# allenai/OLMoASR

Hardware: AMD Instinct MI355X
Metric: audio-seconds/sec/node (train step) (higher is better)
Workload: dtype bf16

## Files before the change

### include/oasr.h

```cpp
#ifndef OASR_H
#define OASR_H
#include <stddef.h>
#include <stdint.h>
#ifdef __cplusplus
extern "C" {
#endif

#define OASR_OK 0
#define OASR_EINVAL (-1)
#define OASR_EHIP (-2)
#define OASR_ESTATE (-3)
#define OASR_ERETRY (-4)

typedef struct oasr_ctx oasr_ctx;

typedef struct oasr_dims {
  int n_mels, n_audio_ctx, n_audio_state, n_audio_head, n_audio_layer;
  int n_vocab, n_text_ctx, n_text_state, n_text_head, n_text_layer;
} oasr_dims;

const char* oasr_last_error(void);
#define OASR_ABI_VERSION 216
int oasr_version(void);

// ... 64 lines not shown
  int32_t B;
  int32_t S;
  int32_t span_forward;
  int32_t accumulate_loss;
  float loss_scale, inv_accum;
} oasr_train_step_args;
size_t oasr_sizeof_train_step_args(void);
int oasr_train_step(oasr_ctx*, const oasr_train_step_args*, void* workspace, size_t workspace_bytes, void* stream);

int oasr_train_fwd(oasr_ctx*, const float* mel, const int64_t* tokens, const int32_t* text_len, int B, int S, float* logits_out,
                   void* workspace, size_t workspace_bytes, void* stream);
int oasr_train_bwd(oasr_ctx*, const int64_t* tokens, const int32_t* text_len, const float* dlogits, int B, int S, void** seg_events,
                   void* workspace, size_t workspace_bytes, void* stream);
int oasr_zero_grad(oasr_ctx*, void* stream);

int oasr_train_encode(oasr_ctx*, const float* mel, int B, void* xa_out, void* workspace, size_t workspace_bytes, void* stream);
int oasr_train_encode_bwd(oasr_ctx*, const void* dxa, int B, float* dmel_out, void* workspace, size_t workspace_bytes, void* stream);
int oasr_train_decode(oasr_ctx*, const int64_t* tokens, const void* xa, const int32_t* text_len, int B, int S, float* logits_out,
                      void* workspace, size_t workspace_bytes, void* stream);
int oasr_train_decode_bwd(oasr_ctx*, const int64_t* tokens, const int32_t* text_len, const float* dlogits, int B, int S, void* dxa_out,
                          void* workspace, size_t workspace_bytes, void* stream);

int oasr_set_trainable(oasr_ctx*, const uint8_t* mask, int n_params);

int oasr_optim_step(oasr_ctx*, float inv_loss_scale, float max_grad_norm, float lr, float beta1, float beta2, float eps,
                    float weight_decay, int64_t step, float* stats_out, void* scratch, void* stream);

int oasr_grad_sumsq_range(oasr_ctx*, int64_t off, int64_t numel, float* stats_out, void* scratch, void* stream);
int oasr_optim_step_range(oasr_ctx*, int64_t off, int64_t numel, float* exp_avg_shard, float* exp_avg_sq_shard, const float* stats,
                          float inv_loss_scale, float max_grad_norm, float lr, float beta1, float beta2, float eps, float weight_decay,
                          int64_t step, void* stream);

typedef struct oasr_operand {
  const void* ptr; int64_t ld; int rpb; int64_t bstride; int lead; int kvalid; int trail_from;
} oasr_operand;
typedef struct oasr_gemm_args {
  oasr_operand A, B; int M, N, K; int ta, tb; float alpha;
  const float* bias; int act; const float* pos; int pos_period;
  const void* dgelu_u; int64_t ldu; const void* resid; int64_t ldr;
  void* out; void* out_pre; int64_t ldc; float* out_f32; int64_t ldc32; float beta; float* colsum; int atomic; int split_k;
  int dgelu_deriv;
} oasr_gemm_args;
int oasr_gemm(const oasr_gemm_args*, void* stream);
int oasr_layernorm_fwd(const void* x, const float* gamma, const float* beta, void* y, float* mean, float* rstd, int64_t rows, int d, void* stream);
int oasr_layernorm_bwd(const void* dy, const void* x, const float* gamma, const float* mean, const float* rstd, const void* dres,
                       void* dx, float* dgamma, float* dbeta, int64_t rows, int d, void* stream);
typedef struct oasr_attn_args {
  const void *q, *k, *v; int64_t ldq, ldk, ldv, bsq, bsk, bsv; void* o; int64_t ldo, bso; float* lse; void* o_lo; const int32_t* kv_len;
  int B, H, Tq, Tk, causal; const void* d_o; float* delta; void *dq, *dk, *dv;
  float *dq_colsum, *dv_colsum;
  float* colsum_scratch;
  int32_t* qtile_flags;
  const int32_t *q_rows, *k_rows, *q_span;
} oasr_attn_args;
#define OASR_ROWTAB 16
size_t oasr_sizeof_attn_args(void);
int oasr_attention_fwd(const oasr_attn_args*, void* stream);
int oasr_attention_bwd(const oasr_attn_args*, void* stream);
int oasr_attention_scores(const oasr_attn_args*, int dtype, float* scores, void* stream);
#define OASR_ALIGN_MAX_LAYERS 32
typedef struct oasr_align_args {
  const float* qk[OASR_ALIGN_MAX_LAYERS];
  uint32_t head_mask[OASR_ALIGN_MAX_LAYERS];
  int32_t n_layers, H, n_tok, Tk, n_frames, medfilt_width;
  float qk_scale;
  int32_t reserved;
  float* out;
  int64_t ldo;
} oasr_align_args;
size_t oasr_sizeof_align_args(void);
size_t oasr_alignment_workspace_bytes(int n_selected_heads, int n_tok, int n_frames);
int oasr_alignment_matrix(const oasr_align_args*, void* workspace, size_t workspace_bytes, void* stream);
size_t oasr_dtw_workspace_bytes(int N, int M);
int oasr_dtw(const float* cost, int64_t ld, int N, int M, int negate, int32_t* text_indices, int32_t* time_indices, int32_t* path_len,
             void* workspace, size_t workspace_bytes, void* stream);
#define OASR_SPECAUG_MAX_MASKS 8
typedef struct oasr_specaug {
  int32_t freq_masks, freq_width, time_masks, time_width;
  float fill;
} oasr_specaug;
size_t oasr_sizeof_specaug(void);
int oasr_spec_augment(float* mel, int B, int n_mels, int T, const oasr_specaug* policy, uint64_t seed, uint64_t first_clip, void* stream);
int oasr_spec_augment_plan(const oasr_specaug* policy, uint64_t seed, uint64_t clip, int n_mels, int T, int32_t* freq_iv, int32_t* time_iv);
#define OASR_EDIT_MAX_LEN 1023
typedef struct oasr_edit_args {
  const int32_t *hyp, *ref, *hyp_len, *ref_len;
  int32_t* out;
  int64_t ld_hyp, ld_ref;
  int32_t B, Lh, Lr, reserved;
} oasr_edit_args;
size_t oasr_sizeof_edit_args(void);
int oasr_edit_counts(const oasr_edit_args*, void* stream);
int oasr_edit_counts_host(const oasr_edit_args*);
int oasr_cross_entropy(void* logits_bf16, int64_t ld, int V, const int64_t* targets, int64_t rows, int64_t ignore, float gscale,
                       int32_t* n_valid_dev, float* row_loss, float* loss_out, int write_grad, void* stream);
int oasr_cast_f32_bf16(const float* src, void* dst, int64_t n, void* stream);
int oasr_lora_merge_op(const float* w0, const float* A, const float* B, int rows, int cols, int rank, float scale, int out_dtype, void* out,
                       void* stream);
size_t oasr_lora_grad_scratch_bytes(int rows, int cols, int rank);
int oasr_lora_grad_op(const float* dW, const float* A, const float* B, int rows, int cols, int rank, float scale, float* dA, float* dB,
                      void* scratch, void* stream);
int oasr_pick_tokens(const float* logits, int64_t ld, int V, int64_t rows, const float* mask, const float* mask2, int64_t* tok,
                     float* logprob, void* stream);
int oasr_pick_tokens_ts(const float* logits, int64_t ld, int V, int64_t rows, const float* mask, const float* mask2,
                        const int64_t* history, int64_t history_ld, int n_history, int timestamp_begin, int eot, int no_timestamps,
                        int max_initial_index, int64_t* tok, float* logprob, void* stream);
// ... 12 lines not shown
```

### include/oasr_testing.h

```cpp
#ifndef OASR_TESTING_H
#define OASR_TESTING_H
#include "oasr.h"
#ifdef __cplusplus
extern "C" {
#endif

int oasr_profile_gemm(int enable);
int oasr_gemm_set_variant(int v);
int oasr_decode_set_ln_fold(int mode);
int oasr_span_set_side_streams(int mode);
int oasr_span_side_streams(void);
int oasr_xcd_plan_debug(int d, int H, int Te, int M, int L, int team, int wg, int* out, int max_blocks);
int oasr_wide_supports_debug(int d, int H, int Te, int S_max, int L, int M, int nwg);
int oasr_wide_plan_debug(int d, int nwg, int N, int K, int wg, int wave, int* out, int max_units);
int oasr_xcd_offsets_ok_debug(const int64_t* layer0, long long lstride, long long cache_lstride, int d, int Te, int L, int M);
int oasr_attention_set_pingpong(int on);
int oasr_gemm_set_stagger(int sleeps, int phases);
int oasr_gemm_force_general(int on);
int oasr_test_gemm(const oasr_gemm_args* a, float* colsum_scratch, int atomic_on_pp, int raster_gm, int stagger, int stagger_phases, void* stream);
int oasr_profile_gemm_records(char* buf, int cap);
int oasr_profile_gemm_collect(double* ms4, double* flops4, int64_t* count4, char* by_symbol , int cap);
int oasr_probe_lds_oob(const void* src_u16 , void* dst_u16 , void* stream);
int oasr_probe_tr16(const void* src_bf16 , void* dst_bf16 , void* stream);
int oasr_test_span_tables(const int32_t* span_host, int B, int S, const int64_t* targets, int32_t* rows_out, int32_t* span_out,
                          int64_t* targets_rows_out, int64_t* active_rows_out, void* stream);

int oasr_test_embedding_fwd(const int64_t* tok, const float* E, const float* pos, void* x, int dtype, int B, int S, int d, int64_t n_embed,
                            const int32_t* rows, void* stream);
int oasr_test_embedding_bwd(const int64_t* tok, const void* dx, int dtype, float* dE, float* dpos, int B, int S, int d, int64_t pad_id,
                            int64_t n_embed, const int32_t* rows, const int32_t* span, void* stream);
int oasr_test_colsum(const void* x, int dtype, int64_t ld, int64_t M, int ncols, float* out, void* stream);
int oasr_test_conv2_col2im_dgelu(const void* dA, const void* u1, void* dpre1, int dtype, int B, int T1, int d, void* stream);
int oasr_test_conv1_col2im_mel(const void* dcol, int dtype, float* dmel, int B, int T1, int n_mels, void* stream);
int oasr_test_mel_to_time_major(const float* mel, void* out, int dtype, int B, int n_mels, int T, const float* clip_max, void* stream);
int oasr_test_pack_conv_weight(const float* w, void* dst, int dtype, int co, int ci, int ldk, void* stream);
int oasr_test_unpack_conv_grad(const float* g, float* dw, int co, int ci, int ldk, void* stream);
int oasr_test_pack_embedding(const float* e, void* dst, int rows, int rows_pad, int d, void* stream);
int oasr_test_dgelu_mul(const void* dy, const void* u, void* out, int dtype, int64_t n, void* stream);
int oasr_test_dlogits_from_f32(const float* src, int V, int64_t rows, int64_t ld, void* dst, int dtype, void* stream);
int oasr_test_logits_to_f32(const void* logits, int dtype, int64_t ld, int64_t rows, int V, float* out, void* stream);
int oasr_test_layernorm_bwd(const void* dy, const void* x, const float* gamma, const float* mean, const float* rstd, const void* dres, void* dx,
                            float* dgamma, float* dbeta, float* dsum, int dtype, int64_t rows, int d, void* stream);

int oasr_test_dtw_host(const float* cost, int64_t ld, int N, int M, int negate, int32_t* text_indices, int32_t* time_indices, int32_t* path_len,
                       void* workspace);

int oasr_test_argmax_rows(const void* logits, int dtype, int64_t ld, int V, int64_t n_rows, const int32_t* rows, const int32_t* span, int B, int S,
                          int32_t* pred_out, void* stream);

#ifdef __cplusplus
}
#endif
#endif
```

### olmoasr_amd/_native.py

```python
import ctypes as C
import os

import torch

_HERE = os.path.dirname(os.path.abspath(__file__))
LIB_PATH = os.environ.get("OASR_LIB") or os.path.join(_HERE, "liboasr.so")
_lib = None


class NativeError(RuntimeError):
    pass


class Dims(C.Structure):
    _fields_ = [(n, C.c_int) for n in ("n_mels", "n_audio_ctx", "n_audio_state", "n_audio_head", "n_audio_layer",
                                       "n_vocab", "n_text_ctx", "n_text_state", "n_text_head", "n_text_layer")]


class Operand(C.Structure):
    _fields_ = [("ptr", C.c_void_p), ("ld", C.c_int64), ("rpb", C.c_int), ("bstride", C.c_int64), ("lead", C.c_int),
                ("kvalid", C.c_int), ("trail_from", C.c_int)]


class GemmArgs(C.Structure):
    _fields_ = [("A", Operand), ("B", Operand), ("M", C.c_int), ("N", C.c_int), ("K", C.c_int), ("ta", C.c_int),
                ("tb", C.c_int), ("alpha", C.c_float), ("bias", C.c_void_p), ("act", C.c_int), ("pos", C.c_void_p),
                ("pos_period", C.c_int), ("dgelu_u", C.c_void_p), ("ldu", C.c_int64), ("resid", C.c_void_p),
                ("ldr", C.c_int64), ("out", C.c_void_p), ("out_pre", C.c_void_p), ("ldc", C.c_int64),
                ("out_f32", C.c_void_p), ("ldc32", C.c_int64), ("beta", C.c_float), ("colsum", C.c_void_p), ("atomic", C.c_int),
                ("split_k", C.c_int), ("dgelu_deriv", C.c_int)]


class AttnArgs(C.Structure):
    _fields_ = [("q", C.c_void_p), ("k", C.c_void_p), ("v", C.c_void_p), ("ldq", C.c_int64), ("ldk", C.c_int64),
                ("ldv", C.c_int64), ("bsq", C.c_int64), ("bsk", C.c_int64), ("bsv", C.c_int64), ("o", C.c_void_p),
                ("ldo", C.c_int64), ("bso", C.c_int64), ("lse", C.c_void_p), ("o_lo", C.c_void_p), ("kv_len", C.c_void_p), ("B", C.c_int),
                ("H", C.c_int), ("Tq", C.c_int), ("Tk", C.c_int), ("causal", C.c_int), ("d_o", C.c_void_p),
                ("delta", C.c_void_p), ("dq", C.c_void_p), ("dk", C.c_void_p), ("dv", C.c_void_p), ("dq_colsum", C.c_void_p),
                ("dv_colsum", C.c_void_p), ("colsum_scratch", C.c_void_p), ("qtile_flags", C.c_void_p),
                ("q_rows", C.c_void_p), ("k_rows", C.c_void_p), ("q_span", C.c_void_p)]


class AlignArgs(C.Structure):
    MAX_LAYERS = 32
    _fields_ = [("qk", C.c_void_p * 32), ("head_mask", C.c_uint32 * 32), ("n_layers", C.c_int32), ("H", C.c_int32), ("n_tok", C.c_int32),
                ("Tk", C.c_int32), ("n_frames", C.c_int32), ("medfilt_width", C.c_int32), ("qk_scale", C.c_float), ("reserved", C.c_int32),
                ("out", C.c_void_p), ("ldo", C.c_int64)]


class SpecAug(C.Structure):
    MAX_MASKS = 8
    _fields_ = [("freq_masks", C.c_int32), ("freq_width", C.c_int32), ("time_masks", C.c_int32), ("time_width", C.c_int32), ("fill", C.c_float)]


class EditArgs(C.Structure):
    MAX_LEN = 1023
    _fields_ = [("hyp", C.c_void_p), ("ref", C.c_void_p), ("hyp_len", C.c_void_p), ("ref_len", C.c_void_p), ("out", C.c_void_p),
                ("ld_hyp", C.c_int64), ("ld_ref", C.c_int64), ("B", C.c_int32), ("Lh", C.c_int32), ("Lr", C.c_int32), ("reserved", C.c_int32)]


class TrainStepArgs(C.Structure):
    _fields_ = [(n, C.c_void_p) for n in ("mel", "xa", "tokens", "targets", "text_len", "span_host", "mel_clip_max", "loss_out", "logits_out",
                                          "pred_out", "seg_events")] + \
               [(n, C.c_int32) for n in ("B", "S", "span_forward", "accumulate_loss")] + [("loss_scale", C.c_float), ("inv_accum", C.c_float)]


DTW_MAX_N, DTW_MAX_M = 448, 1500
ABI_VERSION = 216
KV_TAIL_BYTES = 327680
MODE_INFER, MODE_TRAIN, MODE_TRAIN_ENC, MODE_TRAIN_DEC = 0, 1, 2, 3
ROWTAB = 16
LORA_MAX_RANK = 64


def _declare(lib):
    vp, i32, i64, f32, sz = C.c_void_p, C.c_int, C.c_int64, C.c_float, C.c_size_t
    sig = {
        "oasr_last_error": (C.c_char_p, []),
        "oasr_version": (i32, []),
        "oasr_log_mel_workspace_bytes": (sz, [i32]),
        "oasr_log_mel": (i32, [vp, i32, i32, i32, vp, vp, vp]),
        "oasr_mel_filterbank": (i32, [vp]),
        "oasr_create": (vp, [C.POINTER(Dims)]),
        "oasr_create_ex": (vp, [C.POINTER(Dims), i32]),
        "oasr_create_ex2": (vp, [C.POINTER(Dims), i32, i32]),
        "oasr_compute_dtype": (i32, [vp]),
        "oasr_create_ex3": (vp, [C.POINTER(Dims), i32, i32, vp, i32, i32, f32]),
        "oasr_lora_count": (i32, [vp]),
        "oasr_lora_merge": (i32, [vp, vp]),
        "oasr_lora_merge_op": (i32, [vp, vp, vp, i32, i32, i32, f32, i32, vp, vp]),
        "oasr_lora_grad_scratch_bytes": (sz, [i32, i32, i32]),
        "oasr_lora_grad_op": (i32, [vp, vp, vp, i32, i32, i32, f32, vp, vp, vp, vp]),
        "oasr_encode": (i32, [vp, vp, i32, vp, vp, sz, vp]),
        "oasr_kv_cache_bytes": (sz, [vp, i32]),
        "oasr_decode_step_workspace_bytes": (sz, [vp, i32]),
        "oasr_decode_begin": (i32, [vp, vp, i32, vp, vp]),
        "oasr_decode_step": (i32, [vp, vp, i32, i32, vp, vp, vp, sz, vp]),
        "oasr_decode_check": (i32, [vp, i32, vp, vp]),
        "oasr_decode_logits": (i32, [vp, vp, vp, vp, i32, i32, i32, vp, vp, sz, vp]),
        "oasr_destroy": (None, [vp]),
        "oasr_param_count": (i32, [vp]),
        "oasr_param_info": (i32, [vp, i32, C.c_char_p, i32, C.POINTER(i64), C.POINTER(i64), C.POINTER(i32), C.POINTER(i64)]),
        "oasr_param_numel": (i64, [vp]),
        "oasr_segment_count": (i32, [vp]),
        "oasr_segment_info": (i32, [vp, i32, C.POINTER(i64), C.POINTER(i64)]),
        "oasr_bind": (i32, [vp, vp, vp, vp, vp, vp]),
        "oasr_shadow_bytes": (sz, [vp]),
        "oasr_bind_shadow": (i32, [vp, vp]),
        "oasr_refresh_shadow": (i32, [vp, vp]),
        "oasr_workspace_bytes": (sz, [vp, i32, i32, i32]),
        "oasr_forward": (i32, [vp, vp, vp, vp, i32, i32, vp, vp, vp, sz, vp]),
        "oasr_sizeof_train_step_args": (sz, []),
        "oasr_train_step": (i32, [vp, C.POINTER(TrainStepArgs), vp, sz, vp]),
        "oasr_log_mel_raw": (i32, [vp, i32, i32, i32, vp, vp, vp, vp]),
        "oasr_sizeof_attn_args": (sz, []),
        "oasr_test_span_tables": (i32, [vp, i32, i32, vp, vp, vp, vp, vp, vp]),
        "oasr_test_embedding_fwd": (i32, [vp, vp, vp, vp, i32, i32, i32, i32, i64, vp, vp]),
        "oasr_test_embedding_bwd": (i32, [vp, vp, i32, vp, vp, i32, i32, i32, i64, i64, vp, vp, vp]),
        "oasr_test_colsum": (i32, [vp, i32, i64, i64, i32, vp, vp]),
        "oasr_test_conv2_col2im_dgelu": (i32, [vp, vp, vp, i32, i32, i32, i32, vp]),
        "oasr_test_conv1_col2im_mel": (i32, [vp, i32, vp, i32, i32, i32, vp]),
        "oasr_test_mel_to_time_major": (i32, [vp, vp, i32, i32, i32, i32, vp, vp]),
        "oasr_test_pack_conv_weight": (i32, [vp, vp, i32, i32, i32, i32, vp]),
        "oasr_test_unpack_conv_grad": (i32, [vp, vp, i32, i32, i32, vp]),
        "oasr_test_pack_embedding": (i32, [vp, vp, i32, i32, i32, vp]),
        "oasr_test_dgelu_mul": (i32, [vp, vp, vp, i32, i64, vp]),
        "oasr_test_dlogits_from_f32": (i32, [vp, i32, i64, i64, vp, i32, vp]),
        "oasr_test_logits_to_f32": (i32, [vp, i32, i64, i64, i32, vp, vp]),
        "oasr_test_layernorm_bwd": (i32, [vp, vp, vp, vp, vp, vp, vp, vp, vp, vp, i32, i64, i32, vp]),
        "oasr_train_fwd": (i32, [vp, vp, vp, vp, i32, i32, vp, vp, sz, vp]),
        "oasr_train_bwd": (i32, [vp, vp, vp, vp, i32, i32, vp, vp, sz, vp]),
        "oasr_zero_grad": (i32, [vp, vp]),
        "oasr_train_encode": (i32, [vp, vp, i32, vp, vp, sz, vp]),
        "oasr_train_encode_bwd": (i32, [vp, vp, i32, vp, vp, sz, vp]),
        "oasr_train_decode": (i32, [vp, vp, vp, vp, i32, i32, vp, vp, sz, vp]),
        "oasr_train_decode_bwd": (i32, [vp, vp, vp, vp, i32, i32, vp, vp, sz, vp]),
        "oasr_set_trainable": (i32, [vp, vp, i32]),
        "oasr_optim_step": (i32, [vp, f32, f32, f32, f32, f32, f32, f32, i64, vp, vp, vp]),
        "oasr_grad_sumsq_range": (i32, [vp, i64, i64, vp, vp, vp]),
        "oasr_optim_step_range": (i32, [vp, i64, i64, vp, vp, vp, f32, f32, f32, f32, f32, f32, f32, i64, vp]),
        "oasr_gemm": (i32, [C.POINTER(GemmArgs), vp]),
        "oasr_test_gemm": (i32, [C.POINTER(GemmArgs), vp, i32, i32, i32, i32, vp]),
        "oasr_profile_gemm_records": (i32, [C.c_char_p, i32]),
        "oasr_layernorm_fwd": (i32, [vp, vp, vp, vp, vp, vp, i64, i32, vp]),
        "oasr_layernorm_bwd": (i32, [vp, vp, vp, vp, vp, vp, vp, vp, vp, i64, i32, vp]),
        "oasr_attention_fwd": (i32, [C.POINTER(AttnArgs), vp]),
        "oasr_attention_bwd": (i32, [C.POINTER(AttnArgs), vp]),
        "oasr_attention_scores": (i32, [C.POINTER(AttnArgs), i32, vp, vp]),
        "oasr_sizeof_align_args": (sz, []),
        "oasr_alignment_workspace_bytes": (sz, [i32, i32, i32]),
        "oasr_alignment_matrix": (i32, [C.POINTER(AlignArgs), vp, sz, vp]),
        "oasr_dtw_workspace_bytes": (sz, [i32, i32]),
        "oasr_dtw": (i32, [vp, i64, i32, i32, i32, vp, vp, vp, vp, sz, vp]),
        "oasr_test_dtw_host": (i32, [vp, i64, i32, i32, i32, vp, vp, vp, vp]),
        "oasr_sizeof_specaug": (sz, []),
        "oasr_spec_augment": (i32, [vp, i32, i32, i32, C.POINTER(SpecAug), C.c_uint64, C.c_uint64, vp]),
        "oasr_spec_augment_plan": (i32, [C.POINTER(SpecAug), C.c_uint64, C.c_uint64, i32, i32, vp, vp]),
        "oasr_sizeof_edit_args": (sz, []),
        "oasr_edit_counts": (i32, [C.POINTER(EditArgs), vp]),
        "oasr_edit_counts_host": (i32, [C.POINTER(EditArgs)]),
        "oasr_test_argmax_rows": (i32, [vp, i32, i64, i32, i64, vp, vp, i32, i32, vp, vp]),
        "oasr_cross_entropy": (i32, [vp, i64, i32, vp, i64, i64, f32, vp, vp, vp, i32, vp]),
        "oasr_cast_f32_bf16": (i32, [vp, vp, i64, vp]),
        "oasr_pick_tokens": (i32, [vp, i64, i32, i64, vp, vp, vp, vp, vp]),
        "oasr_pick_tokens_ts": (i32, [vp, i64, i32, i64, vp, vp, vp, i64, i32, i32, i32, i32, i32, vp, vp, vp]),
        "oasr_topk_tokens": (i32, [vp, i64, i32, i64, vp, vp, vp, i64, i32, i32, i32, i32, i32, i32, vp, vp, vp]),
        "oasr_sample_tokens": (i32, [vp, i64, i32, i64, vp, vp, vp, i64, i32, i32, i32, i32, i32, f32, vp, vp, vp, vp]),
        "oasr_probe_tr16": (i32, [vp, vp, vp]),
        "oasr_probe_lds_oob": (i32, [vp, vp, vp]),
        "oasr_profile_gemm": (i32, [i32]),
        "oasr_gemm_force_general": (i32, [i32]),
        "oasr_gemm_set_stagger": (i32, [i32, i32]),
        "oasr_gemm_set_variant": (i32, [i32]),
        "oasr_decode_set_ln_fold": (i32, [i32]),
        "oasr_span_set_side_streams": (i32, [i32]),
        "oasr_span_side_streams": (i32, []),
        "oasr_xcd_plan_debug": (i32, [i32, i32, i32, i32, i32, i32, i32, vp, i32]),
        "oasr_xcd_offsets_ok_debug": (i32, [vp, C.c_longlong, C.c_longlong, i32, i32, i32, i32]),
        "oasr_wide_supports_debug": (i32, [i32, i32, i32, i32, i32, i32, i32]),
        "oasr_wide_plan_debug": (i32, [i32, i32, i32, i32, i32, i32, vp, i32]),
        "oasr_attention_set_pingpong": (i32, [i32]),
        "oasr_profile_gemm_collect": (i32, [vp, vp, vp, C.c_char_p, i32]),
    }
    for name, (res, args) in sig.items():
        fn = getattr(lib, name)
        fn.restype = res
        fn.argtypes = args
    return list(sig)


EXPORTS = None


def lib():
    global _lib, EXPORTS
    if _lib is None:
        if not os.path.isfile(LIB_PATH):
            raise NativeError(f"{LIB_PATH} not found: run `python -c 'import __graft_entry__ as g; g.build()'` "
                              "(hipcc --offload-arch=gfx950).  There is no CPU/PyTorch fallback for this path.")
        try:
            _lib = C.CDLL(LIB_PATH)
        except OSError as e:
            raise NativeError(f"cannot load {LIB_PATH}: {e}") from e
        handle, _lib = _lib, None
        vfn = getattr(handle, "oasr_version", None)
        ver = int(vfn()) if vfn is not None else None
        sfn = getattr(handle, "oasr_sizeof_attn_args", None)
        size = int(sfn()) if sfn is not None else None
        if ver != ABI_VERSION or size != C.sizeof(AttnArgs):
            raise NativeError(f"{LIB_PATH}: ABI version {ver} / oasr_attn_args of {size} bytes, this binding is written for version "
                              f"{ABI_VERSION} / {C.sizeof(AttnArgs)} bytes -- rebuild (__graft_entry__.build())")
        try:
            exports = _declare(handle)
        except AttributeError as e:
            raise NativeError(f"{LIB_PATH} (ABI {ver}) lacks an entry point this binding declares: {e} -- rebuild (__graft_entry__.build())") from e
        if int(handle.oasr_sizeof_align_args()) != C.sizeof(AlignArgs):
            raise NativeError(f"{LIB_PATH}: oasr_align_args of {int(handle.oasr_sizeof_align_args())} bytes, this binding passes "
                              f"{C.sizeof(AlignArgs)} -- rebuild (__graft_entry__.build())")
        if int(handle.oasr_sizeof_specaug()) != C.sizeof(SpecAug):
            raise NativeError(f"{LIB_PATH}: oasr_specaug of {int(handle.oasr_sizeof_specaug())} bytes, this binding passes "
                              f"{C.sizeof(SpecAug)} -- rebuild (__graft_entry__.build())")
        if int(handle.oasr_sizeof_edit_args()) != C.sizeof(EditArgs):
            raise NativeError(f"{LIB_PATH}: oasr_edit_args of {int(handle.oasr_sizeof_edit_args())} bytes, this binding passes "
                              f"{C.sizeof(EditArgs)} -- rebuild (__graft_entry__.build())")
        if int(handle.oasr_sizeof_train_step_args()) != C.sizeof(TrainStepArgs):
            raise NativeError(f"{LIB_PATH}: oasr_train_step_args of {int(handle.oasr_sizeof_train_step_args())} bytes, this binding passes "
                              f"{C.sizeof(TrainStepArgs)} -- rebuild (__graft_entry__.build())")
        _lib, EXPORTS = handle, exports
    return _lib


def enable_testing_hooks():
    os.environ["OASR_TESTING_HOOKS"] = "1"

# ... 24 lines not shown
```

### olmoasr_amd/csrc/api.hip

```cpp
#include <stdarg.h>

#include "../../include/oasr.h"
#include "kernels.h"

static thread_local char g_err[512] = "";

void oasr_set_error(const char* fmt, ...) {
  va_list ap;
  va_start(ap, fmt);
  vsnprintf(g_err, sizeof(g_err), fmt, ap);
  va_end(ap);
}

extern "C" const char* oasr_last_error(void) { return g_err; }
extern "C" int oasr_version(void) { return OASR_ABI_VERSION; }
extern "C" size_t oasr_sizeof_attn_args(void) { return sizeof(oasr_attn_args); }

static OperandView to_view(const oasr_operand& o) {
  return OperandView{(const bf16_t*)o.ptr, (long)o.ld, o.rpb, (long)o.bstride, o.lead, o.kvalid, o.trail_from};
}

static int to_gemm(const oasr_gemm_args* a, GemmArgs& g) {
  OASR_REQUIRE(a, "oasr_gemm: null args");
  g = gemm_defaults();
// ... 13 lines not shown
  g.ldu = a->ldu;
  g.resid = (const bf16_t*)a->resid;
  g.ldr = a->ldr;
  g.out = (bf16_t*)a->out;
  g.out_pre = (bf16_t*)a->out_pre;
  g.ldc = a->ldc;
  g.out_f32 = a->out_f32;
  g.ldc32 = a->ldc32;
  g.beta = a->beta;
  g.colsum = a->colsum;
  g.atomic = a->atomic;
  g.split_k = a->split_k < 1 ? 1 : a->split_k;
  g.dgelu_deriv = a->dgelu_deriv;
  OASR_REQUIRE(a->act >= 0 && a->act <= 2, "oasr_gemm: act must be 0 (none), 1 (GELU) or 2 (GELU, out_pre = GELU')");
  return OASR_OK;
}

extern "C" int oasr_gemm(const oasr_gemm_args* a, void* stream) {
  GemmArgs g;
  const int rc = to_gemm(a, g);
  return rc ? rc : launch_gemm(g, (hipStream_t)stream);
}

extern "C" int oasr_test_gemm(const oasr_gemm_args* a, float* colsum_scratch, int atomic_on_pp, int raster_gm, int stagger, int stagger_phases,
                              void* stream) {
  GemmArgs g;
  const int rc = to_gemm(a, g);
  if (rc) return rc;
  g.colsum_scratch = colsum_scratch;
  g.atomic_on_pp = atomic_on_pp;
  g.raster_gm = raster_gm;
  g.stagger = stagger;
  g.stagger_phases = stagger_phases;
  return launch_gemm(g, (hipStream_t)stream);
}

extern "C" int oasr_profile_gemm(int enable) {
  gemm_profile_enable(enable);
  return OASR_OK;
}
extern "C" int oasr_gemm_set_variant(int dma_in_mma) {
  OASR_HOOK_GATE("oasr_gemm_set_variant");
  gemm_set_variant(dma_in_mma);
  return OASR_OK;
}
extern "C" int oasr_gemm_set_stagger(int sleeps, int phases) {
  OASR_HOOK_GATE("oasr_gemm_set_stagger");
  gemm_set_stagger(sleeps, phases);
  return OASR_OK;
}
extern "C" int oasr_attention_set_pingpong(int on) {
  OASR_HOOK_GATE("oasr_attention_set_pingpong");
  attention_set_pingpong(on);
  return OASR_OK;
}
extern "C" int oasr_gemm_force_general(int on) {
  OASR_HOOK_GATE("oasr_gemm_force_general");
  gemm_force_general(on);
  return OASR_OK;
}
extern "C" int oasr_profile_gemm_records(char* buf, int cap) {
  const int n = gemm_profile_records(buf, cap);
  OASR_REQUIRE(n >= 0, "oasr_profile_gemm_records: %d bytes do not hold the launch records", cap);
  return n;
}
extern "C" int oasr_profile_gemm_collect(double* ms4, double* flops4, int64_t* count4, char* by_symbol, int cap) {
  OASR_REQUIRE(ms4 && flops4 && count4, "profile_collect: null");
  long c[4];
  int rc = gemm_profile_collect(ms4, flops4, c, by_symbol, cap);
  for (int i = 0; i < 4; ++i) count4[i] = c[i];
  return rc;
}

extern "C" int oasr_layernorm_fwd(const void* x, const float* gamma, const float* beta, void* y, float* mean, float* rstd, int64_t rows,
                                  int d, void* stream) {
  return launch_layernorm_fwd((const bf16_t*)x, gamma, beta, (bf16_t*)y, mean, rstd, rows, d, (hipStream_t)stream);
}
extern "C" int oasr_layernorm_bwd(const void* dy, const void* x, const float* gamma, const float* mean, const float* rstd,
                                  const void* dres, void* dx, float* dgamma, float* dbeta, int64_t rows, int d, void* stream) {
  return launch_layernorm_bwd((const bf16_t*)dy, (const bf16_t*)x, gamma, mean, rstd, (const bf16_t*)dres, (bf16_t*)dx, dgamma, dbeta,
                              nullptr, rows, d, (hipStream_t)stream);
}

static AttnArgs to_attn(const oasr_attn_args* a) {
  AttnArgs r;
  memset(&r, 0, sizeof(r));
  r.q = (const bf16_t*)a->q;
  r.k = (const bf16_t*)a->k;
  r.v = (const bf16_t*)a->v;
  r.ldq = a->ldq;
  r.ldk = a->ldk;
  r.ldv = a->ldv;
  r.bsq = a->bsq;
  r.bsk = a->bsk;
  r.bsv = a->bsv;
  r.o = (bf16_t*)a->o;
  r.ldo = a->ldo;
  r.bso = a->bso;
  r.lse = a->lse;
  r.o_lo = (bf16_t*)a->o_lo;
  r.kv_len = a->kv_len;
  r.B = a->B;
  r.H = a->H;
  r.Tq = a->Tq;
  r.Tk = a->Tk;
  r.causal = a->causal;
  r.d_o = (const bf16_t*)a->d_o;
  r.delta = a->delta;
  r.dq = (bf16_t*)a->dq;
  r.dk = (bf16_t*)a->dk;
  r.dv = (bf16_t*)a->dv;
  r.dq_colsum = a->dq_colsum;
  r.dv_colsum = a->dv_colsum;
  r.colsum_scratch = a->colsum_scratch;
  r.qtile_flags = a->qtile_flags;
  r.q_rows = a->q_rows;
  r.k_rows = a->k_rows;
  r.q_span = a->q_span;
  return r;
}
extern "C" int oasr_attention_fwd(const oasr_attn_args* a, void* stream) {
  OASR_REQUIRE(a, "oasr_attention_fwd: null args");
  return launch_attention_fwd(to_attn(a), (hipStream_t)stream);
}
extern "C" int oasr_attention_bwd(const oasr_attn_args* a, void* stream) {
  OASR_REQUIRE(a, "oasr_attention_bwd: null args");
  return launch_attention_bwd(to_attn(a), (hipStream_t)stream);
}
extern "C" int oasr_attention_scores(const oasr_attn_args* a, int dtype, float* scores, void* stream) {
  OASR_REQUIRE(a && scores, "oasr_attention_scores: null args");
  OASR_REQUIRE(dtype == OASR_DTYPE_BF16 || dtype == OASR_DTYPE_F32, "oasr_attention_scores: dtype %d (0 = bf16 operands, 1 = fp32 operands)", dtype);
  if (dtype == OASR_DTYPE_BF16) return launch_attention_scores(to_attn(a), scores, (hipStream_t)stream);
  AttnArgsF f;
  memset(&f, 0, sizeof(f));
  f.q = (const float*)a->q, f.k = (const float*)a->k;
  f.ldq = a->ldq, f.ldk = a->ldk, f.bsq = a->bsq, f.bsk = a->bsk;
  f.kv_len = a->kv_len;
  f.B = a->B, f.H = a->H, f.Tq = a->Tq, f.Tk = a->Tk, f.causal = a->causal;
  f.q_rows = a->q_rows, f.k_rows = a->k_rows;
  return launch_attention_scores(f, scores, (hipStream_t)stream);
}

extern "C" size_t oasr_sizeof_align_args(void) { return sizeof(oasr_align_args); }
extern "C" int oasr_alignment_matrix(const oasr_align_args* a, void* workspace, size_t workspace_bytes, void* stream) {
  return launch_alignment_matrix(a, workspace, workspace_bytes, (hipStream_t)stream);
}
extern "C" int oasr_dtw(const float* cost, int64_t ld, int N, int M, int negate, int32_t* text_indices, int32_t* time_indices, int32_t* path_len,
                        void* workspace, size_t workspace_bytes, void* stream) {
  return launch_dtw(cost, (long)ld, N, M, negate, text_indices, time_indices, path_len, workspace, workspace_bytes, (hipStream_t)stream);
}

extern "C" size_t oasr_sizeof_specaug(void) { return sizeof(oasr_specaug); }
extern "C" int oasr_spec_augment(float* mel, int B, int n_mels, int T, const oasr_specaug* policy, uint64_t seed, uint64_t first_clip,
                                 void* stream) {
  return launch_spec_augment(mel, B, n_mels, T, policy, seed, first_clip, (hipStream_t)stream);
}

extern "C" int oasr_edit_counts(const oasr_edit_args* a, void* stream) { return launch_edit_counts(a, (hipStream_t)stream); }

extern "C" int oasr_test_span_tables(const int32_t* span_host, int B, int S, const int64_t* targets, int32_t* rows_out, int32_t* span_out,
                                     int64_t* targets_rows_out, int64_t* active_rows_out, void* stream) {
  OASR_REQUIRE(active_rows_out, "oasr_test_span_tables: null");
  long act = 0;
  const int rc = launch_build_span_tables(span_host, B, S, targets, 51864, rows_out, span_out, targets_rows_out, &act, (hipStream_t)stream);
  *active_rows_out = act;
  return rc;
}

#define OASR_TEST_DTYPE(name) \
  OASR_REQUIRE(dtype == OASR_DTYPE_BF16 || dtype == OASR_DTYPE_F32, name ": dtype %d (0 = bf16, 1 = fp32 activations)", dtype)

extern "C" int oasr_test_embedding_fwd(const int64_t* tok, const float* E, const float* pos, void* x, int dtype, int B, int S, int d,
                                       int64_t n_embed, const int32_t* rows, void* stream) {
  OASR_TEST_DTYPE("oasr_test_embedding_fwd");
  if (dtype == OASR_DTYPE_BF16) return launch_embedding_fwd(tok, E, pos, (bf16_t*)x, B, S, d, (long)n_embed, (hipStream_t)stream, rows);
  return launch_embedding_fwd(tok, E, pos, (float*)x, B, S, d, (long)n_embed, (hipStream_t)stream, rows);
}
extern "C" int oasr_test_embedding_bwd(const int64_t* tok, const void* dx, int dtype, float* dE, float* dpos, int B, int S, int d, int64_t pad_id,
                                       int64_t n_embed, const int32_t* rows, const int32_t* span, void* stream) {
  OASR_TEST_DTYPE("oasr_test_embedding_bwd");
  OASR_REQUIRE(!span || rows, "oasr_test_embedding_bwd: span comes with a chunk-row table");
  if (dtype == OASR_DTYPE_BF16)
    return launch_embedding_bwd(tok, (const bf16_t*)dx, dE, dpos, B, S, d, (long)pad_id, (long)n_embed, (hipStream_t)stream, rows, span);
  return launch_embedding_bwd(tok, (const float*)dx, dE, dpos, B, S, d, (long)pad_id, (long)n_embed, (hipStream_t)stream, rows, span);
}
extern "C" int oasr_test_colsum(const void* x, int dtype, int64_t ld, int64_t M, int ncols, float* out, void* stream) {
  OASR_TEST_DTYPE("oasr_test_colsum");
  if (dtype == OASR_DTYPE_BF16) return launch_colsum_accum((const bf16_t*)x, (long)ld, (long)M, ncols, out, (hipStream_t)stream);
  return launch_colsum_accum((const float*)x, (long)ld, (long)M, ncols, out, (hipStream_t)stream);
}
extern "C" int oasr_test_conv2_col2im_dgelu(const void* dA, const void* u1, void* dpre1, int dtype, int B, int T1, int d, void* stream) {
  OASR_TEST_DTYPE("oasr_test_conv2_col2im_dgelu");
  OASR_REQUIRE(B > 0 && T1 > 0 && d > 0, "oasr_test_conv2_col2im_dgelu: bad shape (B=%d T1=%d d=%d)", B, T1, d);
  if (dtype == OASR_DTYPE_BF16) return launch_conv2_col2im_dgelu((const bf16_t*)dA, (const bf16_t*)u1, (bf16_t*)dpre1, B, T1, d, (hipStream_t)stream);
  return launch_conv2_col2im_dgelu((const float*)dA, (const float*)u1, (float*)dpre1, B, T1, d, (hipStream_t)stream);
}
extern "C" int oasr_test_conv1_col2im_mel(const void* dcol, int dtype, float* dmel, int B, int T1, int n_mels, void* stream) {
  OASR_TEST_DTYPE("oasr_test_conv1_col2im_mel");
  if (dtype == OASR_DTYPE_BF16) return launch_conv1_col2im_mel((const bf16_t*)dcol, dmel, B, T1, n_mels, (hipStream_t)stream);
  return launch_conv1_col2im_mel((const float*)dcol, dmel, B, T1, n_mels, (hipStream_t)stream);
}
extern "C" int oasr_test_mel_to_time_major(const float* mel, void* out, int dtype, int B, int n_mels, int T, const float* clip_max, void* stream) {
  OASR_TEST_DTYPE("oasr_test_mel_to_time_major");
  OASR_REQUIRE(B > 0 && n_mels > 0 && T > 0, "oasr_test_mel_to_time_major: bad shape (B=%d n_mels=%d T=%d)", B, n_mels, T);
  if (dtype == OASR_DTYPE_BF16) return launch_mel_to_time_major(mel, (bf16_t*)out, B, n_mels, T, (hipStream_t)stream, clip_max);
  return launch_mel_to_time_major(mel, (float*)out, B, n_mels, T, (hipStream_t)stream, clip_max);
}
extern "C" int oasr_test_pack_conv_weight(const float* w, void* dst, int dtype, int co, int ci, int ldk, void* stream) {
  OASR_TEST_DTYPE("oasr_test_pack_conv_weight");
  OASR_REQUIRE(co > 0 && ci > 0, "oasr_test_pack_conv_weight: bad shape (co=%d ci=%d)", co, ci);
  if (dtype == OASR_DTYPE_BF16) return launch_pack_conv_weight(w, (bf16_t*)dst, co, ci, ldk, (hipStream_t)stream);
  return launch_pack_conv_weight(w, (float*)dst, co, ci, ldk, (hipStream_t)stream);
}
extern "C" int oasr_test_unpack_conv_grad(const float* g, float* dw, int co, int ci, int ldk, void* stream) {
  OASR_REQUIRE(co > 0 && ci > 0, "oasr_test_unpack_conv_grad: bad shape (co=%d ci=%d)", co, ci);
  return launch_unpack_conv_grad(g, dw, co, ci, ldk, (hipStream_t)stream);
}
extern "C" int oasr_test_pack_embedding(const float* e, void* dst, int rows, int rows_pad, int d, void* stream) {
  OASR_REQUIRE(rows > 0 && d > 0, "oasr_test_pack_embedding: bad shape (rows=%d d=%d)", rows, d);
  return launch_pack_embedding(e, (bf16_t*)dst, rows, rows_pad, d, (hipStream_t)stream);
}
// ... 109 lines not shown
```

### olmoasr_amd/csrc/attention.hip

```cpp
#include "decode_shared.h"

namespace {

constexpr float LOG2E = 1.4426950408889634f;
constexpr float LN2 = 0.6931471805599453f;
constexpr float SCALE = 0.125f;
constexpr float NEG = -1.0e30f;
constexpr int TILE = 64 * 64 * 2;

typedef __attribute__((address_space(3))) s16x4_t* lds_s16x4_ptr;

__device__ __forceinline__ int tile_addr(int row, int c16) {
  const int x = (row >> 1) & 7;
  return row * 128 + ((c16 ^ x ^ ((x & 1) << 2)) << 4);
}

struct TileSrc {
  __amdgpu_buffer_rsrc_t rs;
  unsigned voff[2];
  unsigned row_bytes;
};
__device__ __forceinline__ TileSrc tile_src(const bf16_t* base, long ld, int rmax, int tid) {
  TileSrc t;
  t.rs = __builtin_amdgcn_make_buffer_rsrc(const_cast<bf16_t*>(base), 0, (int)(((long)(rmax - 1) * ld + 64) * 2), 0x00020000);
// ... 47 lines not shown
  }
  return v;
}

__device__ __forceinline__ void store_rows_bf16(char* stg, const f32x16_t (&T)[2], float scale, bf16_t* gbase, long ld, int rows_valid,
                                                int lane, float* wave_sums = nullptr) {
  const int row = lane & 31, hh = lane >> 5;
#pragma unroll
  for (int dt = 0; dt < 2; ++dt)
#pragma unroll
    for (int g4 = 0; g4 < 4; ++g4) {
      u32x2_t o;
      o[0] = pack_bf2(T[dt][4 * g4] * scale, T[dt][4 * g4 + 1] * scale);
      o[1] = pack_bf2(T[dt][4 * g4 + 2] * scale, T[dt][4 * g4 + 3] * scale);
      *(u32x2_t*)(stg + row * 128 + (((dt * 4 + g4) ^ (row & 7)) << 4) + hh * 8) = o;
    }
  __builtin_amdgcn_wave_barrier();
  float cs[8];
#pragma unroll
  for (int e = 0; e < 8; ++e) cs[e] = 0.f;
#pragma unroll
  for (int i = 0; i < 4; ++i) {
    const int r2 = i * 8 + (lane >> 3), ch = lane & 7;
    const u32x4_t v = *(const u32x4_t*)(stg + r2 * 128 + ((ch ^ (r2 & 7)) << 4));
    if (r2 < rows_valid) {
      *(u32x4_t*)(gbase + (long)r2 * ld + ch * 8) = v;
#pragma unroll
      for (int e = 0; e < 4; ++e) {
        cs[2 * e] += bf_lo(v[e]);
        cs[2 * e + 1] += bf_hi(v[e]);
      }
    }
  }
  if (wave_sums) {
#pragma unroll
    for (int e = 0; e < 8; ++e) {
      float t = cs[e];
      t += __shfl_xor(t, 8, 64);
      t += __shfl_xor(t, 16, 64);
      t += __shfl_xor(t, 32, 64);
      cs[e] = t;
    }
    if (lane < 8) {
#pragma unroll
      for (int e = 0; e < 8; ++e) wave_sums[lane * 8 + e] = cs[e];
    }
  }
  __builtin_amdgcn_wave_barrier();
}

#define MFMA(a, b, c) __builtin_amdgcn_mfma_f32_32x32x16_bf16((a), (b), (c), 0, 0, 0)

__device__ __forceinline__ int chunk_row(const int32_t* rows, int b, int t) { return rows[b * OASR_ROWTAB + (t >> 6)] + (t & 63); }

typedef float f32x2_t __attribute__((ext_vector_type(2)));
__device__ __forceinline__ f32x2_t pk_fma(f32x2_t a, f32x2_t b, f32x2_t c) { return __builtin_elementwise_fma(a, b, c); }
__device__ __forceinline__ f32x2_t pk_exp2(f32x2_t a) {
  f32x2_t r;
  r[0] = __builtin_amdgcn_exp2f(a[0]);
  r[1] = __builtin_amdgcn_exp2f(a[1]);
  return r;
}
constexpr float RESCALE_THR = 8.0f;

#define ATTN_FENCE() __builtin_amdgcn_sched_barrier(0)
constexpr int PNS = 4;
constexpr int PSTG = 2 * TILE;

__device__ __forceinline__ void glds16_asm(const u32x4_t rs, unsigned lds_addr, unsigned voff) {
  asm volatile("s_mov_b32 m0, %0\n\ts_nop 0\n\tbuffer_load_dwordx4 %1, %2, 0 offen lds" ::"s"(lds_addr), "v"(voff), "s"(rs) : "memory");
}
struct PipeSrc1 {
  u32x4_t rs;
  unsigned voff;
  unsigned tile_bytes;
};
__device__ __forceinline__ PipeSrc1 pipe_src1(const bf16_t* base, long ld, int rmax, int wave, int lane) {
  PipeSrc1 t;
  const unsigned long addr = (unsigned long)base;
  t.rs[0] = (unsigned)addr;
  t.rs[1] = (unsigned)(addr >> 32) & 0xffffu;
  t.rs[2] = (unsigned)(((long)(rmax - 1) * ld + 64) * 2);
  t.rs[3] = 0x00020000u;
  t.tile_bytes = (unsigned)(64 * ld * 2);
  const int row = wave * 8 + (lane >> 3);
  const int x = (row >> 1) & 7;
  const int c = (lane & 7) ^ x ^ ((x & 1) << 2);
  t.voff = (unsigned)(row * ld * 2 + c * 16);
  return t;
}
#define ATTN_BARRIER()                          \
  do {                                          \
    ATTN_FENCE();                               \
    asm volatile("s_barrier" ::: "memory");     \
    ATTN_FENCE();                               \
  } while (0)


template <bool CAUSAL, bool ROWS>
__global__ __launch_bounds__(256, 3) void attn_fwd_kernel(AttnArgs a) {
  __shared__ __attribute__((aligned(1024))) char smem[3 * 2 * TILE];
  const int tid = threadIdx.x, lane = tid & 63, wave = tid >> 6, hh = lane >> 5;
  const int nqb = (a.Tq + 127) >> 7;
  const int bid = xcd_remap(blockIdx.x, gridDim.x);
  const int bh = bid / nqb;
  const int b = bh / a.H, h = bh - b * a.H;
  const int q0 = (bid - bh * nqb) * 128;
  const int myq = q0 + wave * 32 + (lane & 31);
  const int myq_c = myq < a.Tq ? myq : a.Tq - 1;
  const bool krows = ROWS && a.k_rows != nullptr;
  const int q_lim = (ROWS && a.q_span) ? min(a.q_span[b], a.Tq) : a.Tq;
  if (ROWS && q0 >= q_lim) return;
  const bool w_act = !ROWS || q0 + wave * 32 < q_lim;

  const bf16_t* qp = ROWS ? a.q + (long)chunk_row(a.q_rows, b, myq_c) * a.ldq + h * 64 : a.q + (long)b * a.bsq + (long)myq_c * a.ldq + h * 64;
  bf16x8_t qf[4];
#pragma unroll
  for (int ds = 0; ds < 4; ++ds) qf[ds] = ld_frag_global(qp + ds * 16 + hh * 8);

  int kv_len = a.kv_len ? a.kv_len[b] : a.Tk;
  kv_len = kv_len < a.Tk ? kv_len : a.Tk;
  int kv_end = kv_len;
  if (CAUSAL) kv_end = kv_end < q0 + 128 ? kv_end : q0 + 128;
  const int ntiles = kv_end > 0 ? (kv_end + 63) >> 6 : 1;

  auto krow0 = [&](int t) { return krows ? __builtin_amdgcn_readfirstlane(a.k_rows[b * OASR_ROWTAB + t]) : t * 64; };
  const PipeSrc1 ksrc = krows ? pipe_src1(a.k + h * 64, a.ldk, a.B * a.Tk, wave, lane) : pipe_src1(a.k + (long)b * a.bsk + h * 64, a.ldk, a.Tk, wave, lane);
  const PipeSrc1 vsrc = krows ? pipe_src1(a.v + h * 64, a.ldv, a.B * a.Tk, wave, lane) : pipe_src1(a.v + (long)b * a.bsv + h * 64, a.ldv, a.Tk, wave, lane);
  const unsigned smem_a = (unsigned)(size_t)smem;
  const int wave_u = __builtin_amdgcn_readfirstlane(wave);
  const unsigned krb = (unsigned)(a.ldk * 2), vrb = (unsigned)(a.ldv * 2);
  auto dma_tile = [&](int t2, int stage) {
    unsigned ko = 0x7fffff00u, vo = 0x7fffff00u;
    if (t2 < ntiles) {
      const unsigned r0 = (unsigned)krow0(t2);
      ko = ksrc.voff + r0 * krb;
      vo = vsrc.voff + r0 * vrb;
    }
    const unsigned dst = smem_a + stage * 2 * TILE + wave_u * 1024;
    glds16_asm(ksrc.rs, dst, ko);
    glds16_asm(ksrc.rs, dst + 4096, ko + 32 * krb);
    glds16_asm(vsrc.rs, dst + TILE, vo);
    glds16_asm(vsrc.rs, dst + TILE + 4096, vo + 32 * vrb);
  };

  f32x16_t oT[2];
#pragma unroll
  for (int i = 0; i < 2; ++i)
#pragma unroll
    for (int r = 0; r < 16; ++r) oT[i][r] = 0.f;
  float m_run = NEG;
  f32x2_t l_run2 = {0.f, 0.f};

  asm volatile("" ::"v"(qf[0]), "v"(qf[1]), "v"(qf[2]), "v"(qf[3]));
  asm volatile("s_waitcnt vmcnt(0)" ::: "memory");
  dma_tile(0, 0);
  dma_tile(1, 1);
  int stg = 0;
  asm volatile("s_waitcnt vmcnt(4)" ::: "memory");
  ATTN_BARRIER();
// ... 65 lines not shown
          ps0 += p0;
          ps1 += p1;
        }
      l_run2[0] += ps0;
      l_run2[1] += ps1;
    }
    asm volatile("s_waitcnt vmcnt(0)" ::: "memory");
    ATTN_BARRIER();
    dma_tile(t + 2, stg == 2 ? 0 : stg + 1);
    if (t + 1 < ntiles) {
#pragma unroll
      for (int ds = 0; ds < 4; ++ds) kf0[ds] = frag_rows(smem + stg * 2 * TILE, 0, ds, lane);
    }
#pragma unroll
    for (int kt = 0; kt < 2; ++kt)
#pragma unroll
      for (int u = 0; u < 2; ++u) {
        const bf16x8_t pf = pack_half(sT[kt], u);
#pragma unroll
        for (int dt = 0; dt < 2; ++dt) oT[dt] = MFMA(frag_cols(vb, kt * 32 + 16 * u, dt * 32, lane), pf, oT[dt]);
      }
  }
  asm volatile("s_waitcnt vmcnt(0)" ::: "memory");
  __syncthreads();

  const float l_run = l_run2[0] + l_run2[1];
  const float l_tot = l_run + __shfl_xor(l_run, 32, 64);
  const float inv = l_tot > 0.f ? 1.0f / l_tot : 0.f;
  {
    char* stg = smem + wave * 4096;
    const int rows_valid = w_act ? a.Tq - (q0 + wave * 32) : 0;
    const long row0 = ROWS ? (long)chunk_row(a.q_rows, b, q0 + wave * 32) * a.ldo + h * 64 : (long)b * a.bso + (long)(q0 + wave * 32) * a.ldo + h * 64;
    store_rows_bf16(stg, oT, inv, a.o + row0, a.ldo, rows_valid, lane);
    if (a.o_lo) {
#pragma unroll
      for (int dt = 0; dt < 2; ++dt)
#pragma unroll
        for (int r = 0; r < 16; ++r) {
          const float v = oT[dt][r] * inv;
          oT[dt][r] = v - bf_round(v);
        }
      store_rows_bf16(stg, oT, 1.0f, a.o_lo + row0, a.ldo, rows_valid, lane);
    }
    if (myq < a.Tq && hh == 0 && a.lse && w_act) a.lse[((long)b * a.H + h) * a.Tq + myq] = (m_run + __builtin_amdgcn_logf(l_tot)) * LN2;
  }
}

template <bool CAUSAL, bool ROWS>
__global__ __launch_bounds__(256, 2) void attn_bwd_dq_kernel(AttnArgs a) {
  __shared__ __attribute__((aligned(16))) char smem[4 * TILE];
  const int tid = threadIdx.x, lane = tid & 63, wave = tid >> 6, hh = lane >> 5;
  const int nqb = (a.Tq + 127) >> 7;
  const int bid = xcd_remap(blockIdx.x, gridDim.x);
  const int bh = bid / nqb;
  const int b = bh / a.H, h = bh - b * a.H;
  const int q0 = (bid - bh * nqb) * 128;
  const int myq = q0 + wave * 32 + (lane & 31);
  const bool krows = ROWS && a.k_rows != nullptr;
  const int q_lim = (ROWS && a.q_span) ? min(a.q_span[b], a.Tq) : a.Tq;
  if (ROWS && q0 >= q_lim) {
    if (a.dq_colsum && tid < 64) a.colsum_scratch[((long)(b * nqb + (bid - bh * nqb)) * a.H + h) * 64 + tid] = 0.f;
    return;
  }
  const bool w_act = !ROWS || q0 + wave * 32 < q_lim;
  const int myq_c = !w_act ? q0 + (lane & 31) : (myq < a.Tq ? myq : a.Tq - 1);

  const long qrow = ROWS ? (long)chunk_row(a.q_rows, b, myq_c) : 0;
  const bf16_t* qp = ROWS ? a.q + qrow * a.ldq + h * 64 : a.q + (long)b * a.bsq + (long)myq_c * a.ldq + h * 64;
  const long orow_off = ROWS ? qrow * a.ldo + h * 64 : (long)b * a.bso + (long)myq_c * a.ldo + h * 64;
  const bf16_t* dop = a.d_o + orow_off;
  const bf16_t* op = a.o + orow_off;
  const bf16_t* olop = a.o_lo ? a.o_lo + orow_off : nullptr;
  bf16x8_t qf[4], dof[4];
  float dpart = 0.f;
#pragma unroll
  for (int ds = 0; ds < 4; ++ds) {
    qf[ds] = ld_frag_global(qp + ds * 16 + hh * 8);
    u32x4_t d4 = *(const u32x4_t*)(dop + ds * 16 + hh * 8);
    if (ROWS && !w_act) d4 = u32x4_t{0u, 0u, 0u, 0u};
    dof[ds] = __builtin_bit_cast(bf16x8_t, d4);
    const u32x4_t o4 = *(const u32x4_t*)(op + ds * 16 + hh * 8);
    if (olop) {
      const u32x4_t r4 = *(const u32x4_t*)(olop + ds * 16 + hh * 8);
#pragma unroll
      for (int i = 0; i < 4; ++i)
        dpart += bf_lo(d4[i]) * (bf_lo(o4[i]) + bf_lo(r4[i])) + bf_hi(d4[i]) * (bf_hi(o4[i]) + bf_hi(r4[i]));
    } else {
#pragma unroll
      for (int i = 0; i < 4; ++i) dpart += bf_lo(d4[i]) * bf_lo(o4[i]) + bf_hi(d4[i]) * bf_hi(o4[i]);
    }
  }
  const float delta = dpart + __shfl_xor(dpart, 32, 64);
  const long stat_idx = ((long)b * a.H + h) * a.Tq + myq_c;
  if (hh == 0 && myq < a.Tq && w_act) a.delta[stat_idx] = delta;
  const float lse2 = a.lse[stat_idx] * LOG2E;

  int kv_len = a.kv_len ? a.kv_len[b] : a.Tk;
  kv_len = kv_len < a.Tk ? kv_len : a.Tk;
  int kv_end = kv_len;
  if (CAUSAL) kv_end = kv_end < q0 + 128 ? kv_end : q0 + 128;
  int ntiles = kv_end > 0 ? (kv_end + 63) >> 6 : 1;
  if (a.qtile_flags) {
    __shared__ int nzs[4];
    bool nz = false;
#pragma unroll
    for (int ds = 0; ds < 4; ++ds) {
      const u32x4_t d4 = __builtin_bit_cast(u32x4_t, dof[ds]);
      nz = nz || ((d4[0] | d4[1] | d4[2] | d4[3]) & 0x7fff7fffu) != 0u;
    }
    const bool wnz = __any(nz);
    if (lane == 0) nzs[wave] = wnz ? 1 : 0;
    __syncthreads();
    const int t0nz = nzs[0] | nzs[1], t1nz = nzs[2] | nzs[3];
    if (tid == 0) {
// ... 34 lines not shown
      f32x16_t sT, dpT;
#pragma unroll
      for (int r = 0; r < 16; ++r) {
        sT[r] = 0.f;
        dpT[r] = 0.f;
      }
#pragma unroll
      for (int ds = 0; ds < 4; ++ds) {
        sT = MFMA(frag_rows(kb, kt * 32, ds, lane), qf[ds], sT);
        dpT = MFMA(frag_rows(vb, kt * 32, ds, lane), dof[ds], dpT);
      }
      const bool full = (t * 64 + kt * 32 + 32 <= kv_len) && (!CAUSAL || (t * 64 + kt * 32 + 31 <= q0 + wave * 32));
      if (full) {
        const f32x2_t c2 = {SCALE * LOG2E, SCALE * LOG2E}, nl2 = {-lse2, -lse2}, nd2 = {-delta, -delta};
#pragma unroll
        for (int r = 0; r < 16; r += 2) {
          const f32x2_t s2 = {sT[r], sT[r + 1]}, dp2 = {dpT[r], dpT[r + 1]};
          const f32x2_t ds2 = pk_exp2(pk_fma(s2, c2, nl2)) * (dp2 + nd2);
          sT[r] = ds2[0];
          sT[r + 1] = ds2[1];
        }
      } else {
#pragma unroll
        for (int r = 0; r < 16; ++r) {
          const int key = t * 64 + kt * 32 + acc_row(r, hh);
          const bool ok = (key < kv_len) && (!CAUSAL || key <= myq);
          const float p = ok ? __builtin_amdgcn_exp2f(fmaf(sT[r], SCALE * LOG2E, -lse2)) : 0.f;
          sT[r] = p * (dpT[r] - delta);
        }
      }
#pragma unroll
      for (int u = 0; u < 2; ++u) {
        const bf16x8_t dsf = pack_half(sT, u);
#pragma unroll
        for (int dt = 0; dt < 2; ++dt) dqT[dt] = MFMA(frag_cols(kb, kt * 32 + 16 * u, dt * 32, lane), dsf, dqT[dt]);
      }
    }
    if (more) {
      char* nb = smem + ((t + 1) & 1) * 2 * TILE;
      tile_commit(nb, tid, rk);
      tile_commit(nb + TILE, tid, rv);
    }
    __syncthreads();
  }
  float* wsum = (float*)(smem + 16384);
  {
    const long drow0 = ROWS ? (long)chunk_row(a.q_rows, b, q0 + wave * 32) * a.ldq + h * 64 : (long)b * a.bsq + (long)(q0 + wave * 32) * a.ldq + h * 64;
    store_rows_bf16(smem + wave * 4096, dqT, SCALE, a.dq + drow0, a.ldq, w_act ? a.Tq - (q0 + wave * 32) : 0, lane,
                    a.dq_colsum ? wsum + wave * 64 : nullptr);
  }
  if (a.dq_colsum) {
    __syncthreads();
    if (tid < 64)
      a.colsum_scratch[((long)(b * nqb + (bid - bh * nqb)) * a.H + h) * 64 + tid] =
          (wsum[tid] + wsum[64 + tid]) + (wsum[128 + tid] + wsum[192 + tid]);
  }
}

template <bool ROWS>
__global__ __launch_bounds__(512, 1) void attn_bwd_dq_pp_kernel(AttnArgs a) {
  __shared__ __attribute__((aligned(1024))) char smem[PNS * PSTG];
  const int tid = threadIdx.x, lane = tid & 63, wave = __builtin_amdgcn_readfirstlane(tid >> 6), hh = lane >> 5;
  const int grp = wave >> 2;
  const unsigned smem_a = (unsigned)(size_t)smem;
  const int nqb = (a.Tq + 255) >> 8;
  const int bid = xcd_remap(blockIdx.x, gridDim.x);
  const int bh = bid / nqb;
  const int b = bh / a.H, h = bh - b * a.H;
  const int q0 = (bid - bh * nqb) * 256;
  const int myq = q0 + wave * 32 + (lane & 31);
  const int q_lim = (ROWS && a.q_span) ? min(a.q_span[b], a.Tq) : a.Tq;
  if (ROWS && q0 >= q_lim) {
    if (a.dq_colsum && tid < 128) {
      const int nqb128 = (a.Tq + 127) >> 7, blk128 = (bid - bh * nqb) * 2 + (tid >> 6);
      if (blk128 < nqb128) a.colsum_scratch[((long)(b * nqb128 + blk128) * a.H + h) * 64 + (tid & 63)] = 0.f;
    }
    return;
  }
  const bool w_act = !ROWS || q0 + wave * 32 < q_lim;
  const int myq_c = !w_act ? q0 + (lane & 31) : (myq < a.Tq ? myq : a.Tq - 1);

  const long qrow = ROWS ? (long)chunk_row(a.q_rows, b, myq_c) : 0;
  const bf16_t* qp = ROWS ? a.q + qrow * a.ldq + h * 64 : a.q + (long)b * a.bsq + (long)myq_c * a.ldq + h * 64;
  const long orow_off = ROWS ? qrow * a.ldo + h * 64 : (long)b * a.bso + (long)myq_c * a.ldo + h * 64;
  const bf16_t* dop = a.d_o + orow_off;
  const bf16_t* op = a.o + orow_off;
  const bf16_t* olop = a.o_lo ? a.o_lo + orow_off : nullptr;
  bf16x8_t qf[4], dof[4];
  float dpart = 0.f;
#pragma unroll
  for (int ds = 0; ds < 4; ++ds) {
    qf[ds] = ld_frag_global(qp + ds * 16 + hh * 8);
    u32x4_t d4 = *(const u32x4_t*)(dop + ds * 16 + hh * 8);
    if (ROWS && !w_act) d4 = u32x4_t{0u, 0u, 0u, 0u};
    dof[ds] = __builtin_bit_cast(bf16x8_t, d4);
    const u32x4_t o4 = *(const u32x4_t*)(op + ds * 16 + hh * 8);
    if (olop) {
      const u32x4_t r4 = *(const u32x4_t*)(olop + ds * 16 + hh * 8);
#pragma unroll
      for (int i = 0; i < 4; ++i)
        dpart += bf_lo(d4[i]) * (bf_lo(o4[i]) + bf_lo(r4[i])) + bf_hi(d4[i]) * (bf_hi(o4[i]) + bf_hi(r4[i]));
    } else {
#pragma unroll
      for (int i = 0; i < 4; ++i) dpart += bf_lo(d4[i]) * bf_lo(o4[i]) + bf_hi(d4[i]) * bf_hi(o4[i]);
    }
  }
  const float delta = dpart + __shfl_xor(dpart, 32, 64);
  const long stat_idx = ((long)b * a.H + h) * a.Tq + myq_c;
  if (hh == 0 && myq < a.Tq && w_act) a.delta[stat_idx] = delta;
  const float lse2 = a.lse[stat_idx] * LOG2E;
  asm volatile("" ::"v"(lse2), "v"(delta), "v"(qf[3]), "v"(dof[3]));
  asm volatile("s_waitcnt vmcnt(0)" ::: "memory");
  bool blk_nz = true;
  if (a.qtile_flags) {
    int* nzs = (int*)smem;
    bool nz = false;
#pragma unroll
    for (int ds = 0; ds < 4; ++ds) {
      const u32x4_t d4 = __builtin_bit_cast(u32x4_t, dof[ds]);
      nz = nz || ((d4[0] | d4[1] | d4[2] | d4[3]) & 0x7fff7fffu) != 0u;
    }
    const bool wnz = __any(nz);
    if (lane == 0) nzs[wave] = wnz ? 1 : 0;
    __syncthreads();
    if (tid < 4) {
      const int ntq = (a.Tq + 63) >> 6, tq = (q0 >> 6) + tid;
      if (tq < ntq) a.qtile_flags[((long)b * a.H + h) * ntq + tq] = nzs[2 * tid] | nzs[2 * tid + 1];
// ... 128 lines not shown
    S[0] = MFMA(Ak[ds], qf[ds], S[0]);
    dP[0] = MFMA(Av[ds], dof[ds], dP[0]);
  }
  ATTN_FENCE();
  load_seg(0, 0, 0);
#pragma unroll
  for (int u = 0; u < 2; ++u) {
    w[1][u] = u32x4_t{0u, 0u, 0u, 0u};
#pragma unroll
    for (int dt = 0; dt < 2; ++dt) {
      kc[u][dt][0] = s16x4_t{0, 0, 0, 0};
      kc[u][dt][1] = s16x4_t{0, 0, 0, 0};
    }
  }
  ATTN_BARRIER();
  if (grp == 1) ATTN_BARRIER();

  for (int g = 0; g < ngroups; ++g) {
#pragma unroll
    for (int st = 0; st < PNS; ++st) {
      const int t = g * PNS + st;
      if (w_act) compute_seg(0);
      ATTN_BARRIER();
      load_seg(t, st, 1);
      ATTN_BARRIER();
      if (w_act) compute_seg(1);
      ATTN_BARRIER();
      load_seg(t + 1, (st + 1) & 3, 0);
      ATTN_BARRIER();
    }
  }
#pragma unroll
  for (int u = 0; u < 2; ++u)
#pragma unroll
    for (int dt = 0; dt < 2; ++dt) {
      const s16x8_t kv8 = __builtin_shufflevector(kc[u][dt][0], kc[u][dt][1], 0, 1, 2, 3, 4, 5, 6, 7);
      dqT[dt] = MFMA(__builtin_bit_cast(bf16x8_t, kv8), __builtin_bit_cast(bf16x8_t, w[1][u]), dqT[dt]);
    }
  if (grp == 0) ATTN_BARRIER();
  asm volatile("s_waitcnt vmcnt(0)" ::: "memory");
  }
  __syncthreads();
  float* wsum = (float*)(smem + 32768);
  {
    const long drow0 = ROWS ? (long)chunk_row(a.q_rows, b, q0 + wave * 32) * a.ldq + h * 64 : (long)b * a.bsq + (long)(q0 + wave * 32) * a.ldq + h * 64;
    store_rows_bf16(smem + wave * 4096, dqT, SCALE, a.dq + drow0, a.ldq, w_act ? a.Tq - (q0 + wave * 32) : 0, lane,
                    a.dq_colsum ? wsum + wave * 64 : nullptr);
  }
  if (a.dq_colsum) {
    __syncthreads();
    if (tid < 128) {
      const int half = tid >> 6, c = tid & 63;
      const int nqb128 = (a.Tq + 127) >> 7;
      const int blk128 = (bid - bh * nqb) * 2 + half;
      if (blk128 < nqb128)
        a.colsum_scratch[((long)(b * nqb128 + blk128) * a.H + h) * 64 + c] =
            (wsum[half * 256 + c] + wsum[half * 256 + 64 + c]) + (wsum[half * 256 + 128 + c] + wsum[half * 256 + 192 + c]);
    }
  }
}

__device__ __forceinline__ int last_nonzero_qtile(const int32_t* flags, int n, int lane) {
  int last = -1;
  for (int i = lane; i < n; i += 64)
    if (flags[i] != 0) last = i;
  return __builtin_amdgcn_readfirstlane(wave_max_i(last));
}

template <bool CAUSAL, bool ROWS>
__global__ __launch_bounds__(256, 2) void attn_bwd_dkdv_kernel(AttnArgs a) {
  constexpr int STAGE = 2 * TILE + 512;
  __shared__ __attribute__((aligned(16))) char smem[2 * STAGE];
  const int tid = threadIdx.x, lane = tid & 63, wave = tid >> 6, hh = lane >> 5;
  const int nkb = (a.Tk + 127) >> 7;
  const int bid = xcd_remap(blockIdx.x, gridDim.x);
  const int bh = bid / nkb;
  const int b = bh / a.H, h = bh - b * a.H;
  const int k0 = (bid - bh * nkb) * 128;
  const int mykey = k0 + wave * 32 + (lane & 31);
  const bool krows = ROWS && a.k_rows != nullptr;
  const int q_lim = (ROWS && a.q_span) ? min(a.q_span[b], a.Tq) : a.Tq;
  const long dv_scratch_off0 = (long)a.B * ((a.Tq + 127) >> 7) * a.H * 64;
  if (krows && a.q_span && k0 >= q_lim) {
    if (a.dv_colsum && tid < 64) a.colsum_scratch[dv_scratch_off0 + ((long)(b * nkb + (bid - bh * nkb)) * a.H + h) * 64 + tid] = 0.f;
    return;
  }
  const bool w_store = !(krows && a.q_span) || k0 + wave * 32 < q_lim;
  const int mykey_c = !w_store ? k0 + (lane & 31) : (mykey < a.Tk ? mykey : a.Tk - 1);

  int kv_len = a.kv_len ? a.kv_len[b] : a.Tk;
  kv_len = kv_len < a.Tk ? kv_len : a.Tk;

  const bf16_t* kp = krows ? a.k + (long)chunk_row(a.k_rows, b, mykey_c) * a.ldk + h * 64 : a.k + (long)b * a.bsk + (long)mykey_c * a.ldk + h * 64;
  const bf16_t* vp = krows ? a.v + (long)chunk_row(a.k_rows, b, mykey_c) * a.ldv + h * 64 : a.v + (long)b * a.bsv + (long)mykey_c * a.ldv + h * 64;
  bf16x8_t kf[4], vf[4];
#pragma unroll
  for (int ds = 0; ds < 4; ++ds) {
    kf[ds] = ld_frag_global(kp + ds * 16 + hh * 8);
    vf[ds] = ld_frag_global(vp + ds * 16 + hh * 8);
  }
  f32x16_t dkT[2], dvT[2];
#pragma unroll
  for (int i = 0; i < 2; ++i)
#pragma unroll
    for (int r = 0; r < 16; ++r) {
      dkT[i][r] = 0.f;
      dvT[i][r] = 0.f;
    }

  const TileSrc qsrc = ROWS ? tile_src(a.q + h * 64, a.ldq, a.B * a.Tq, tid) : tile_src(a.q + (long)b * a.bsq + h * 64, a.ldq, a.Tq, tid);
  const TileSrc dosrc = ROWS ? tile_src(a.d_o + h * 64, a.ldo, a.B * a.Tq, tid) : tile_src(a.d_o + (long)b * a.bso + h * 64, a.ldo, a.Tq, tid);
  const float* lse_b = a.lse + ((long)b * a.H + h) * a.Tq;
  const float* delta_b = a.delta + ((long)b * a.H + h) * a.Tq;

  int nqt = (a.Tq + 63) >> 6;
  if (a.qtile_flags) nqt = last_nonzero_qtile(a.qtile_flags + ((long)b * a.H + h) * nqt, nqt, lane) + 1;
  if (ROWS && (q_lim >> 6) < nqt) nqt = q_lim >> 6;
  const int t_begin = (CAUSAL && k0 < kv_len) ? (k0 >> 6) : 0;
  const bool any = k0 < kv_len && t_begin < nqt;

  u32x4_t rq[2], rd[2];
  float rstat = 0.f;
  auto issue = [&](int t) {
    const int qr0 = ROWS ? __builtin_amdgcn_readfirstlane(a.q_rows[b * OASR_ROWTAB + t]) : t * 64;
    tile_issue(qsrc, qr0, rq);
    tile_issue(dosrc, qr0, rd);
    if (tid < 128) {
      int qi = t * 64 + (tid & 63);
      qi = qi < a.Tq ? qi : a.Tq - 1;
      rstat = tid < 64 ? lse_b[qi] * LOG2E : delta_b[qi];
    }
  };
  auto commit = [&](char* st) {
    tile_commit(st, tid, rq);
    tile_commit(st + TILE, tid, rd);
    if (tid < 128) ((float*)(st + 2 * TILE))[tid] = rstat;
  };
  const long dv_scratch_off = dv_scratch_off0;
  if (!any) {
    if (a.dv_colsum && tid < 64) a.colsum_scratch[dv_scratch_off + ((long)(b * nkb + (bid - bh * nkb)) * a.H + h) * 64 + tid] = 0.f;
    if (mykey < a.Tk && w_store) {
      bf16_t* dkp0 = krows ? a.dk + (long)chunk_row(a.k_rows, b, mykey) * a.ldk + h * 64 : a.dk + (long)b * a.bsk + (long)mykey * a.ldk + h * 64;
      bf16_t* dvp0 = krows ? a.dv + (long)chunk_row(a.k_rows, b, mykey) * a.ldv + h * 64 : a.dv + (long)b * a.bsv + (long)mykey * a.ldv + h * 64;
      const u32x4_t z = {0u, 0u, 0u, 0u};
#pragma unroll
      for (int i = 0; i < 4; ++i) {
        *(u32x4_t*)(dkp0 + hh * 32 + i * 8) = z;
        *(u32x4_t*)(dvp0 + hh * 32 + i * 8) = z;
      }
    }
    return;
  }
  issue(t_begin);
  commit(smem);
  __syncthreads();
  for (int t = t_begin; t < nqt; ++t) {
    const int cur = (t - t_begin) & 1;
    const char* st = smem + cur * STAGE;
    const char* qb = st;
    const char* dob = st + TILE;
    const float* stat = (const float*)(st + 2 * TILE);
    const bool more = t + 1 < nqt;
    if (more) issue(t + 1);
#pragma unroll
    for (int qt = 0; qt < 2; ++qt) {
      f32x16_t s, dp;
#pragma unroll
      for (int r = 0; r < 16; ++r) {
        s[r] = 0.f;
        dp[r] = 0.f;
      }
#pragma unroll
      for (int ds = 0; ds < 4; ++ds) {
        s = MFMA(frag_rows(qb, qt * 32, ds, lane), kf[ds], s);
        dp = MFMA(frag_rows(dob, qt * 32, ds, lane), vf[ds], dp);
      }
      const int key_hi = k0 + wave * 32 + 31;
      const bool full = (t * 64 + qt * 32 + 32 <= a.Tq) && (key_hi < kv_len) && (!CAUSAL || key_hi <= t * 64 + qt * 32);
      if (full) {
        const f32x2_t c2 = {SCALE * LOG2E, SCALE * LOG2E};
#pragma unroll
        for (int g4 = 0; g4 < 4; ++g4) {
          const int ql = qt * 32 + 8 * g4 + 4 * hh;
          const f32x4_t l4 = *(const f32x4_t*)(stat + ql);
          const f32x4_t d4 = *(const f32x4_t*)(stat + 64 + ql);
#pragma unroll
          for (int i = 0; i < 4; i += 2) {
            const int r = 4 * g4 + i;
            const f32x2_t s2 = {s[r], s[r + 1]}, dp2 = {dp[r], dp[r + 1]}, nl2 = {-l4[i], -l4[i + 1]}, nd2 = {-d4[i], -d4[i + 1]};
            const f32x2_t p2 = pk_exp2(pk_fma(s2, c2, nl2));
            const f32x2_t ds2 = p2 * (dp2 + nd2);
            s[r] = p2[0];
            s[r + 1] = p2[1];
            dp[r] = ds2[0];
            dp[r + 1] = ds2[1];
          }
        }
      } else {
#pragma unroll
        for (int g4 = 0; g4 < 4; ++g4) {
          const int ql = qt * 32 + 8 * g4 + 4 * hh;
          const f32x4_t l4 = *(const f32x4_t*)(stat + ql);
          const f32x4_t d4 = *(const f32x4_t*)(stat + 64 + ql);
#pragma unroll
          for (int i = 0; i < 4; ++i) {
            const int r = 4 * g4 + i;
            const int qg = t * 64 + ql + i;
            const bool ok = (qg < a.Tq) && (mykey < kv_len) && (!CAUSAL || mykey <= qg);
            const float p = ok ? __builtin_amdgcn_exp2f(fmaf(s[r], SCALE * LOG2E, -l4[i])) : 0.f;
            s[r] = p;
            dp[r] = p * (dp[r] - d4[i]);
          }
        }
      }
#pragma unroll
      for (int u = 0; u < 2; ++u) {
        const bf16x8_t pf = pack_half(s, u);
        const bf16x8_t dsf = pack_half(dp, u);
#pragma unroll
        for (int dt = 0; dt < 2; ++dt) {
          dvT[dt] = MFMA(frag_cols(dob, qt * 32 + 16 * u, dt * 32, lane), pf, dvT[dt]);
          dkT[dt] = MFMA(frag_cols(qb, qt * 32 + 16 * u, dt * 32, lane), dsf, dkT[dt]);
        }
      }
    }
    if (more) commit(smem + (cur ^ 1) * STAGE);
    __syncthreads();
  }
  {
    char* stg = smem + wave * 4096;
    const int rows_valid = w_store ? a.Tk - (k0 + wave * 32) : 0;
    const long krow0 = krows ? (long)chunk_row(a.k_rows, b, k0 + wave * 32) : 0;
    store_rows_bf16(stg, dkT, SCALE, krows ? a.dk + krow0 * a.ldk + h * 64 : a.dk + (long)b * a.bsk + (long)(k0 + wave * 32) * a.ldk + h * 64,
                    a.ldk, rows_valid, lane);
    float* wsum = (float*)(smem + 16384);
    store_rows_bf16(stg, dvT, 1.0f, krows ? a.dv + krow0 * a.ldv + h * 64 : a.dv + (long)b * a.bsv + (long)(k0 + wave * 32) * a.ldv + h * 64,
                    a.ldv, rows_valid, lane, a.dv_colsum ? wsum + wave * 64 : nullptr);
    if (a.dv_colsum) {
      __syncthreads();
      if (tid < 64)
        a.colsum_scratch[dv_scratch_off + ((long)(b * nkb + (bid - bh * nkb)) * a.H + h) * 64 + tid] =
            (wsum[tid] + wsum[64 + tid]) + (wsum[128 + tid] + wsum[192 + tid]);
    }
  }
}

constexpr int KSTAT = 2048;
constexpr int KLDS = KSTAT + PNS * PSTG;

__device__ __forceinline__ void glds4_asm(const u32x4_t rs, unsigned lds_addr, unsigned voff) {
  asm volatile("s_mov_b32 m0, %0\n\ts_nop 0\n\tbuffer_load_dword %1, %2, 0 offen lds" ::"s"(lds_addr), "v"(voff), "s"(rs) : "memory");
}

template <bool ROWS>
__global__ __launch_bounds__(512, 1) void attn_bwd_dkdv_pp_kernel(AttnArgs a) {
  extern __shared__ __attribute__((aligned(1024))) char smem[];
  const int tid = threadIdx.x, lane = tid & 63, wave = __builtin_amdgcn_readfirstlane(tid >> 6), hh = lane >> 5;
  const int grp = wave >> 2;
  const unsigned smem_a = (unsigned)(size_t)smem;
  const int nkb = (a.Tk + 255) >> 8;
  const int bid = xcd_remap(blockIdx.x, gridDim.x);
  const int bh = bid / nkb;
  const int b = bh / a.H, h = bh - b * a.H;
  const int k0 = (bid - bh * nkb) * 256;
  const int mykey = k0 + wave * 32 + (lane & 31);
  const int mykey_c = mykey < a.Tk ? mykey : a.Tk - 1;

  const bf16_t* kp = a.k + (long)b * a.bsk + (long)mykey_c * a.ldk + h * 64;
  const bf16_t* vp = a.v + (long)b * a.bsv + (long)mykey_c * a.ldv + h * 64;
  bf16x8_t kf[4], vf[4];
#pragma unroll
  for (int ds = 0; ds < 4; ++ds) {
    const u32x4_t k4 = *(const u32x4_t*)(kp + ds * 16 + hh * 8);
    const u32x4_t v4 = *(const u32x4_t*)(vp + ds * 16 + hh * 8);
    u32x4_t kn, vn;
#pragma unroll
    for (int i = 0; i < 4; ++i) {
      kn[i] = pack_bf2(bf_lo(k4[i]) * -0.125f, bf_hi(k4[i]) * -0.125f);
      vn[i] = v4[i] ^ 0x80008000u;
    }
    kf[ds] = __builtin_bit_cast(bf16x8_t, kn);
    vf[ds] = __builtin_bit_cast(bf16x8_t, vn);
  }
  asm volatile("" ::"v"(kf[3]), "v"(vf[3]));
  asm volatile("s_waitcnt vmcnt(0)" ::: "memory");

  int ntiles = (a.Tq + 63) >> 6;
  if (a.qtile_flags) ntiles = last_nonzero_qtile(a.qtile_flags + ((long)b * a.H + h) * ntiles, ntiles, lane) + 1;
  if (ROWS && a.q_span) ntiles = min(ntiles, min(a.q_span[b], a.Tq) >> 6);
  const int ngroups = (ntiles + PNS - 1) / PNS;
  const PipeSrc1 qsrc = ROWS ? pipe_src1(a.q + h * 64, a.ldq, a.B * a.Tq, wave, lane) : pipe_src1(a.q + (long)b * a.bsq + h * 64, a.ldq, a.Tq, wave, lane);
  const PipeSrc1 dosrc = ROWS ? pipe_src1(a.d_o + h * 64, a.ldo, a.B * a.Tq, wave, lane) : pipe_src1(a.d_o + (long)b * a.bso + h * 64, a.ldo, a.Tq, wave, lane);
  int qrow[8];
  if (ROWS) {
// ... 232 lines not shown
        const int t = t0 + 32 * u;
        k4[u] = *(const u32x4_t*)(kp + (long)(k0 + (t < n ? t : n - 1)) * a.ldk);
      }
#pragma unroll
      for (int u = 0; u < 8; ++u) {
        const int t = t0 + 32 * u;
        const float s2 = dec::score8(qv, k4[u]);
        if (t < n) {
          if (l8 == 0) sc[t] = s2;
          mx = fmaxf(mx, s2);
        }
      }
    }
    mx = wave_max(mx);
    if (lane == 0) wmax[wave] = mx;
    __syncthreads();
    const float m = fmaxf(fmaxf(wmax[0], wmax[1]), fmaxf(wmax[2], wmax[3]));
    float l = 0.f, o[8];
#pragma unroll
    for (int j = 0; j < 8; ++j) o[j] = 0.f;
    for (int t0 = grp; t0 < n; t0 += 32 * 8) {
      u32x4_t v4[8];
#pragma unroll
      for (int u = 0; u < 8; ++u) {
        const int t = t0 + 32 * u;
        v4[u] = *(const u32x4_t*)(vp + (long)(k0 + (t < n ? t : n - 1)) * a.ldv);
      }
#pragma unroll
      for (int u = 0; u < 8; ++u) {
        const int t = t0 + 32 * u;
        dec::accum_pv(t < n ? __builtin_amdgcn_exp2f(sc[t] - m) : 0.f, v4[u], l, o);
      }
    }
#pragma unroll
    for (int j = 0; j < 8; ++j) red[grp][l8 * 8 + j] = o[j];
    if (l8 == 0) lsum[grp] = l;
    __syncthreads();
    if (tid < 64) {
      dec::reduce_groups(red, lsum, tid, o_s[sg], l_s[sg]);
      m_s[sg] = m;
    }
    __syncthreads();
  }
  if (tid < 64) {
    float m, lt;
    const float val = dec::merge_segments(m_s, l_s, o_s, ns, m, lt);
    const float nb = __shfl_xor(val, 1, 64);
    if ((tid & 1) == 0) *(uint32_t*)(a.o + (long)b * a.bso + h * 64 + tid) = pack_bf2(val, nb);
    if (tid == 0 && a.lse) a.lse[(long)b * a.H + h] = lt > 0.f ? (m + __builtin_amdgcn_logf(lt)) * LN2 : NEG;
  }
}

int g_attn_pingpong = 1;

int check_args(const AttnArgs& a, bool bwd) {
  OASR_REQUIRE(a.q && a.k && a.v && a.o, "attention: null pointer");
  OASR_REQUIRE(a.B > 0 && a.H > 0 && a.Tq > 0 && a.Tk > 0, "attention: bad shape");
  OASR_REQUIRE((a.ldq % 8) == 0 && (a.ldk % 8) == 0 && (a.ldv % 8) == 0 && (a.ldo % 8) == 0, "attention: strides must be multiples of 8");
  OASR_REQUIRE(!a.causal || a.Tq == a.Tk, "attention: causal needs Tq == Tk");
  if (bwd) OASR_REQUIRE(a.d_o && a.lse && a.delta && a.dq && a.dk && a.dv, "attention_bwd: null pointer");
  if (bwd) OASR_REQUIRE((!a.dq_colsum && !a.dv_colsum) || a.colsum_scratch, "attention_bwd: fused bias gradients need colsum_scratch");
  OASR_REQUIRE(!a.k_rows || a.q_rows, "attention: k_rows needs q_rows");
  OASR_REQUIRE(!a.q_span || a.q_rows, "attention: q_span needs q_rows");
  OASR_REQUIRE(!a.q_rows || ((a.Tq % 64) == 0 && a.Tq <= 64 * OASR_ROWTAB), "attention: chunked query rows need Tq %% 64 == 0 and Tq <= %d", 64 * OASR_ROWTAB);
  OASR_REQUIRE(!a.k_rows || ((a.Tk % 64) == 0 && a.Tk <= 64 * OASR_ROWTAB), "attention: chunked key rows need Tk %% 64 == 0 and Tk <= %d", 64 * OASR_ROWTAB);
  return OASR_OK;
}

}

void attention_set_pingpong(int on) { g_attn_pingpong = on; }

int launch_attention_fwd(const AttnArgs& a, hipStream_t s) {
  int rc = check_args(a, false);
  if (rc) return rc;
  if (a.Tq == 1 && a.Tk <= 1536 && !a.o_lo && !a.q_rows) {
    hipLaunchKernelGGL(attn_decode_kernel, dim3(a.B * a.H), dim3(256), 0, s, a);
    OASR_LAUNCH_CHECK();
    return OASR_OK;
  }
  dim3 grid(cdiv(a.Tq, 128) * a.B * a.H);
  if (a.q_rows) {
    if (a.causal)
      hipLaunchKernelGGL((attn_fwd_kernel<true, true>), grid, dim3(256), 0, s, a);
    else
      hipLaunchKernelGGL((attn_fwd_kernel<false, true>), grid, dim3(256), 0, s, a);
  } else if (a.causal) {
    hipLaunchKernelGGL((attn_fwd_kernel<true, false>), grid, dim3(256), 0, s, a);
  } else {
    hipLaunchKernelGGL((attn_fwd_kernel<false, false>), grid, dim3(256), 0, s, a);
  }
  OASR_LAUNCH_CHECK();
  return OASR_OK;
}

int launch_attention_bwd(const AttnArgs& a, hipStream_t s) {
  int rc = check_args(a, true);
  if (rc) return rc;
  dim3 gq(cdiv(a.Tq, 128) * a.B * a.H), gk(cdiv(a.Tk, 128) * a.B * a.H);
  const bool rows = a.q_rows != nullptr;
  if (a.causal) {
    if (rows) {
      hipLaunchKernelGGL((attn_bwd_dq_kernel<true, true>), gq, dim3(256), 0, s, a);
      hipLaunchKernelGGL((attn_bwd_dkdv_kernel<true, true>), gk, dim3(256), 0, s, a);
    } else {
      hipLaunchKernelGGL((attn_bwd_dq_kernel<true, false>), gq, dim3(256), 0, s, a);
      hipLaunchKernelGGL((attn_bwd_dkdv_kernel<true, false>), gk, dim3(256), 0, s, a);
    }
  } else {
    const bool pp = !a.kv_len && g_attn_pingpong && (!rows || (!a.k_rows && a.Tq <= 512));
    if (pp) {
      if (rows) hipLaunchKernelGGL(attn_bwd_dq_pp_kernel<true>, dim3(cdiv(a.Tq, 256) * a.B * a.H), dim3(512), 0, s, a);
      else hipLaunchKernelGGL(attn_bwd_dq_pp_kernel<false>, dim3(cdiv(a.Tq, 256) * a.B * a.H), dim3(512), 0, s, a);
      static LdsAttrOnce attr_rows, attr_plain;
      rc = rows ? ensure_dynamic_lds(attr_rows, (const void*)attn_bwd_dkdv_pp_kernel<true>, KLDS)
                : ensure_dynamic_lds(attr_plain, (const void*)attn_bwd_dkdv_pp_kernel<false>, KLDS);
      if (rc) return rc;
      if (rows) hipLaunchKernelGGL(attn_bwd_dkdv_pp_kernel<true>, dim3(cdiv(a.Tk, 256) * a.B * a.H), dim3(512), KLDS, s, a);
      else hipLaunchKernelGGL(attn_bwd_dkdv_pp_kernel<false>, dim3(cdiv(a.Tk, 256) * a.B * a.H), dim3(512), KLDS, s, a);
    } else if (rows) {
      hipLaunchKernelGGL((attn_bwd_dq_kernel<false, true>), gq, dim3(256), 0, s, a);
      hipLaunchKernelGGL((attn_bwd_dkdv_kernel<false, true>), gk, dim3(256), 0, s, a);
    } else {
      hipLaunchKernelGGL((attn_bwd_dq_kernel<false, false>), gq, dim3(256), 0, s, a);
      hipLaunchKernelGGL((attn_bwd_dkdv_kernel<false, false>), gk, dim3(256), 0, s, a);
    }
  }
  OASR_LAUNCH_CHECK();
  const int d = a.H * 64;
  const long rq = (long)a.B * cdiv(a.Tq, 128), rk = (long)a.B * cdiv(a.Tk, 128);
  if (a.dq_colsum) {
    int rc2 = launch_colsum_accum(a.colsum_scratch, d, rq, d, a.dq_colsum, s);
    if (rc2) return rc2;
  }
  if (a.dv_colsum) {
    int rc2 = launch_colsum_accum(a.colsum_scratch + rq * d, d, rk, d, a.dv_colsum, s);
    if (rc2) return rc2;
  }
  return OASR_OK;
}
```

### olmoasr_amd/csrc/elementwise.hip

```cpp
#include "kernels.h"

namespace {

inline unsigned grid_for(long work_items, int per_block = 256, int cap = 2048) {
  long b = (work_items + per_block - 1) / per_block;
  if (b < 1) b = 1;
  if (b > cap) b = cap;
  return (unsigned)b;
}

__global__ __launch_bounds__(256) void cast_kernel(const float* __restrict__ src, bf16_t* __restrict__ dst, long n) {
  const long n8 = n >> 3;
  for (long i = blockIdx.x * 256L + threadIdx.x; i < n8; i += (long)gridDim.x * 256) {
    const f32x4_t a = ((const f32x4_t*)src)[2 * i], b = ((const f32x4_t*)src)[2 * i + 1];
    u32x4_t o;
    o[0] = pack_bf2(a[0], a[1]);
    o[1] = pack_bf2(a[2], a[3]);
    o[2] = pack_bf2(b[0], b[1]);
    o[3] = pack_bf2(b[2], b[3]);
    ((u32x4_t*)dst)[i] = o;
  }
  if (blockIdx.x == 0)
    for (long i = (n8 << 3) + threadIdx.x; i < n; i += 256) dst[i] = f2bf_dev(src[i]);
}
// ... 214 lines not shown
  hipLaunchKernelGGL(cast_kernel, dim3(grid_for(n / 8 + 1)), dim3(256), 0, s, src, dst, n);
  OASR_LAUNCH_CHECK();
  return OASR_OK;
}
int launch_pack_conv_weight(const float* w, bf16_t* dst, int co, int ci, int ldk, hipStream_t s) {
  OASR_REQUIRE(w && dst && ldk >= 3 * ci, "pack_conv_weight: bad args");
  hipLaunchKernelGGL(pack_conv_kernel, dim3(grid_for((long)co * ldk)), dim3(256), 0, s, w, dst, co, ci, ldk);
  OASR_LAUNCH_CHECK();
  return OASR_OK;
}
int launch_unpack_conv_grad(const float* g, float* dw, int co, int ci, int ldk, hipStream_t s) {
  OASR_REQUIRE(g && dw && ldk >= 3 * ci, "unpack_conv_grad: bad args");
  hipLaunchKernelGGL(unpack_conv_grad_kernel, dim3(grid_for((long)co * ci * 3)), dim3(256), 0, s, g, dw, co, ci, ldk);
  OASR_LAUNCH_CHECK();
  return OASR_OK;
}
int launch_pack_embedding(const float* e, bf16_t* dst, int rows, int rows_pad, int d, hipStream_t s) {
  OASR_REQUIRE(e && dst && rows_pad >= rows && d % 8 == 0, "pack_embedding: bad args");
  hipLaunchKernelGGL(pack_embedding_kernel, dim3(grid_for((long)rows_pad * d / 8)), dim3(256), 0, s, e, dst, (long)rows * d,
                     (long)rows_pad * d);
  OASR_LAUNCH_CHECK();
  return OASR_OK;
}
int launch_mel_to_time_major(const float* mel, bf16_t* out, int B, int n_mels, int T, hipStream_t s, const float* clip_max) {
  OASR_REQUIRE(mel && out && n_mels <= 128, "mel_to_time_major: bad args");
  hipLaunchKernelGGL(mel_tm_kernel, dim3(cdiv(T, 32), B), dim3(256), 0, s, mel, out, n_mels, T, clip_max);
  OASR_LAUNCH_CHECK();
  return OASR_OK;
}
int launch_embedding_fwd(const int64_t* tok, const float* E, const float* pos, bf16_t* x, int B, int S, int d, long n_embed,
                         hipStream_t s, const int32_t* rows_tab) {
  OASR_REQUIRE(tok && E && pos && x && d % 8 == 0, "embedding_fwd: bad args");
  OASR_REQUIRE(!rows_tab || (S % 64 == 0 && S <= 64 * OASR_ROWTAB), "embedding_fwd: chunk rows need S %% 64 == 0");
  const long rows = (long)B * S;
  hipLaunchKernelGGL(embedding_fwd_kernel, dim3(grid_for(rows * (d / 8))), dim3(256), 0, s, tok, E, pos, x, S, d, rows, n_embed, rows_tab);
  OASR_LAUNCH_CHECK();
  return OASR_OK;
}
int launch_embedding_bwd(const int64_t* tok, const bf16_t* dx, float* dE, float* dpos, int B, int S, int d, long pad_id, long n_embed,
                         hipStream_t s, const int32_t* rows_tab, const int32_t* span) {
  OASR_REQUIRE(tok && dx && (dE || dpos), "embedding_bwd: bad args");
  OASR_REQUIRE(!rows_tab || (S % 64 == 0 && S <= 64 * OASR_ROWTAB), "embedding_bwd: chunk rows need S %% 64 == 0");
  hipLaunchKernelGGL(embedding_bwd_kernel, dim3(S), dim3(256), 0, s, tok, dx, dE, dpos, B, S, d, pad_id, n_embed, rows_tab, span);
  OASR_LAUNCH_CHECK();
  return OASR_OK;
}

namespace {
struct SpanArg {
  uint16_t span[512];
};
__global__ __launch_bounds__(1024) void build_span_tables_kernel(SpanArg sp, int B, int S, const int64_t* __restrict__ targets, long ignore,
                                                                 int32_t* __restrict__ rows, int32_t* __restrict__ span_dev,
                                                                 int64_t* __restrict__ targets_phys) {
  __shared__ int cnt_act[OASR_ROWTAB + 1];
  __shared__ int rows_s[512 * OASR_ROWTAB];
  const int nch = S >> 6, tid = threadIdx.x;
  if (tid <= OASR_ROWTAB) cnt_act[tid] = 0;
  __syncthreads();
  if (tid < nch) {
    int n = 0;
    for (int b = 0; b < B; ++b) n += (64 * tid < (int)sp.span[b]) ? 1 : 0;
    for (int c = tid + 1; c <= nch; ++c) atomicAdd(&cnt_act[c], n);
  }
  __syncthreads();
  const int total_act = cnt_act[nch];
  for (int i = tid; i < B * OASR_ROWTAB; i += 1024) {
    const int b = i / OASR_ROWTAB, c = i - b * OASR_ROWTAB;
    int row = 0x3fffffff;
    if (c < nch) {
      const bool act = 64 * c < (int)sp.span[b];
      int before = 0;
      for (int bb = 0; bb < b; ++bb) before += ((64 * c < (int)sp.span[bb]) == act) ? 1 : 0;
      const int blk_before = act ? cnt_act[c] : c * B - cnt_act[c];
      row = 64 * ((act ? 0 : total_act) + blk_before + before);
    }
    rows[i] = row;
    rows_s[i] = row;
  }
  for (int b = tid; b < B; b += 1024) span_dev[b] = ((int)sp.span[b] + 63) & ~63;
  __syncthreads();
  for (long i = tid; i < (long)B * S; i += 1024) {
    const int b = (int)(i / S), s = (int)(i - (long)b * S);
    if (s < (((int)sp.span[b] + 63) & ~63)) targets_phys[(long)rows_s[b * OASR_ROWTAB + (s >> 6)] + (s & 63)] = targets[i];
  }
  (void)ignore;
}
}
int launch_build_span_tables(const int32_t* span_host, int B, int S, const int64_t* targets, long ignore, int32_t* rows, int32_t* span_dev,
                             int64_t* targets_phys, long* active_rows, hipStream_t s) {
  OASR_REQUIRE(span_host && targets && rows && span_dev && targets_phys && active_rows, "build_span_tables: null pointer");
  OASR_REQUIRE(B > 0 && B <= 512 && S > 0 && S % 64 == 0 && S <= 64 * OASR_ROWTAB, "build_span_tables: need B <= 512, S %% 64 == 0, S <= %d (B=%d S=%d)",
               64 * OASR_ROWTAB, B, S);
  SpanArg sp;
  long act = 0;
  for (int b = 0; b < B; ++b) {
    OASR_REQUIRE(span_host[b] >= 0 && span_host[b] <= S, "build_span_tables: span[%d] = %d outside [0, %d]", b, span_host[b], S);
    sp.span[b] = (uint16_t)span_host[b];
    act += (span_host[b] + 63) / 64 * 64;
  }
  for (int b = B; b < 512; ++b) sp.span[b] = 0;
  *active_rows = act;
  hipLaunchKernelGGL(build_span_tables_kernel, dim3(1), dim3(1024), 0, s, sp, B, S, targets, ignore, rows, span_dev, targets_phys);
  OASR_LAUNCH_CHECK();
  return OASR_OK;
}
int launch_colsum_accum(const bf16_t* x, long ld, long M, int ncols, float* out, hipStream_t s) {
  OASR_REQUIRE(x && out && ncols > 0 && ncols % 8 == 0 && ld % 8 == 0, "colsum: bad args");
  if (M <= 0) return OASR_OK;
  const int gx = cdiv(ncols, 512);
  long gy = 2048 / gx;
  if (gy < 1) gy = 1;
  if (gy > (M + 3) / 4) gy = (M + 3) / 4;
  hipLaunchKernelGGL(colsum_kernel, dim3(gx, (unsigned)gy), dim3(256), 0, s, x, ld, M, ncols, out);
  OASR_LAUNCH_CHECK();
  return OASR_OK;
}
int launch_conv2_col2im_dgelu(const bf16_t* dA, const bf16_t* u1, bf16_t* dpre1, int B, int T1, int d, hipStream_t s) {
  OASR_REQUIRE(dA && u1 && dpre1 && d % 8 == 0 && T1 % 2 == 0, "col2im: bad args");
  const long total8 = (long)B * T1 * (d / 8);
  hipLaunchKernelGGL(col2im_dgelu_kernel, dim3(grid_for(total8)), dim3(256), 0, s, dA, u1, dpre1, T1, d, total8);
  OASR_LAUNCH_CHECK();
  return OASR_OK;
}
int launch_axpy_f32(const float* src, float* dst, long n, float a, hipStream_t s) {
  if (n <= 0) return OASR_OK;
  hipLaunchKernelGGL(axpy_kernel, dim3(grid_for(n)), dim3(256), 0, s, src, dst, n, a);
  OASR_LAUNCH_CHECK();
  return OASR_OK;
}
int launch_dgelu_mul(const bf16_t* dy, const bf16_t* u, bf16_t* out, long n, hipStream_t s) {
  OASR_REQUIRE(dy && u && out && n % 8 == 0, "dgelu_mul: bad args");
  hipLaunchKernelGGL(dgelu_mul_kernel, dim3(grid_for(n / 8)), dim3(256), 0, s, dy, u, out, n / 8);
  OASR_LAUNCH_CHECK();
  return OASR_OK;
}
int launch_dlogits_from_f32(const float* src, int V, long rows, long ld, bf16_t* dst, hipStream_t s) {
  OASR_REQUIRE(src && dst && V <= ld, "dlogits_from_f32: bad args");
  const long total = rows * ld;
  hipLaunchKernelGGL(dlogits_from_f32_kernel, dim3(grid_for(total, 256, 4096)), dim3(256), 0, s, src, V, ld, dst, total);
  OASR_LAUNCH_CHECK();
  return OASR_OK;
}
int launch_logits_to_f32(const bf16_t* logits, long ld, long rows, int V, float* out, hipStream_t s) {
  const long total = rows * V;
  hipLaunchKernelGGL(logits_to_f32_kernel, dim3(grid_for(total, 256, 4096)), dim3(256), 0, s, logits, ld, V, out, total);
  OASR_LAUNCH_CHECK();
  return OASR_OK;
}
```

### olmoasr_amd/csrc/engine_run.h

```cpp
#pragma once
#include "engine_ctx.h"

namespace {

struct LaneScope {
  const int entry = gemm_profile_lane(-1);
  ~LaneScope() { gemm_profile_lane(entry); }
};

template <typename T>
struct Engine {
  typedef OperandViewT<T> View;
  typedef GemmArgsT<T> Gemm;
  typedef AttnArgsT<T> Attn;

struct AttnSave {
  T *ln, *qkv, *o;
  T* kv;
  float *mean, *rstd, *lse;
  T* o_lo;
};
struct BlockSave {
  T* x_in;
  AttnSave sa, ca;
  T *x_mid, *x_mid2, *ln2, *u, *hg, *x_out;
  float *mean2, *rstd2;
};

struct Plan {
  T *mel_tm, *u1, *h1, *u2, *x0, *xa;
  float *mean_p, *rstd_p;
  std::vector<BlockSave> enc, dec;
  T *dx0, *lnf, *logits;
  float *mean_f, *rstd_f, *row_loss;
  int32_t* n_valid;
  T *ga, *gb, *gc, *gln, *gqkv, *go, *gu, *gxa, *gkv, *gq, *gA2;
  float *delta, *tmp_w1p, *tmp_w2p, *cs_scratch, *gemm_cs_scratch;
  int32_t* qtile_flags;
  int32_t *rows, *span_dev;
  int64_t* targets_phys;
  float *lora_dw, *lora_part;
};

static void plan_attn(Arena& A, AttnSave& s, long M, long Mkv, int d, int B, int H, long Tq, bool cross, bool train) {
  s.ln = A.template act<T>(M * d);
  s.qkv = A.template act<T>(M * (cross ? d : 3 * d));
  s.kv = cross ? A.template act<T>(Mkv * 2 * d) : nullptr;
  s.o = A.template act<T>(M * d);
  s.mean = A.f32(M);
  s.rstd = A.f32(M);
  s.lse = A.f32((long)B * H * Tq);
  s.o_lo = train ? A.template act<T>(M * d) : nullptr;
}

static void make_plan(const oasr_ctx* c, Arena& A, Plan& p, int B, int S, bool train, int stage = STAGE_ALL) {
  const int d = c->d;
  const long Me = (long)B * c->Te, M1 = (long)B * c->T1, Md = (long)B * S;
  const bool enc = stage != STAGE_DEC, dec = stage != STAGE_ENC;
  p = Plan();
  if (enc) {
    p.mel_tm = A.template act<T>(M1 * c->dims.n_mels + 2 * 256) + 256;
    p.u1 = A.template act<T>(M1 * d);
    p.h1 = A.template act<T>(M1 * d + d) + d;
    p.u2 = A.template act<T>(Me * d);
    p.x0 = A.template act<T>(Me * d);
  }
  auto plan_block = [&](BlockSave& s, long M, long Tq, bool cross) {
    plan_attn(A, s.sa, M, 0, d, B, c->H, Tq, false, train);
    s.x_mid = A.template act<T>(M * d);
    if (cross) {
      plan_attn(A, s.ca, M, Me, d, B, c->H, Tq, true, train);
      s.x_mid2 = A.template act<T>(M * d);
    } else {
      s.x_mid2 = nullptr;
    }
    s.ln2 = A.template act<T>(M * d);
    s.u = A.template act<T>(M * 4 * d);
    s.hg = A.template act<T>(M * 4 * d);
    s.mean2 = A.f32(M);
    s.rstd2 = A.f32(M);
    s.x_out = A.template act<T>(M * d);
  };
  p.enc.resize(c->L_enc);
  p.dec.resize(c->L_dec);
  if (!enc) {
  } else if (train) {
    for (auto& s : p.enc) plan_block(s, Me, c->Te, false);
  } else {
    BlockSave s0, s1;
    plan_block(s0, Me, c->Te, false);
    s1 = s0;
    s1.x_out = A.template act<T>(Me * d);
    for (int i = 0; i < c->L_enc; ++i) p.enc[i] = (i & 1) ? s1 : s0;
  }
  p.xa = A.template act<T>(Me * d);
  if (enc) {
    p.mean_p = A.f32(Me);
    p.rstd_p = A.f32(Me);
  }
  if (dec) {
    p.dx0 = A.template act<T>(Md * d);
    if (train) {
      for (auto& s : p.dec) plan_block(s, Md, S, true);
    } else {
      BlockSave s0, s1;
      plan_block(s0, Md, S, true);
      s1 = s0;
      s1.x_out = A.template act<T>(Md * d);
      for (int i = 0; i < c->L_dec; ++i) p.dec[i] = (i & 1) ? s1 : s0;
    }
    p.lnf = A.template act<T>(Md * d);
    p.mean_f = A.f32(Md);
    p.rstd_f = A.f32(Md);
    p.logits = A.template act<T>(Md * c->Vp);
    p.row_loss = A.f32(Md);
    p.n_valid = (int32_t*)A.raw(256);
  }
  if (train) {
    if (dec) {
      p.rows = (int32_t*)A.raw((size_t)B * OASR_ROWTAB * 4);
      p.span_dev = (int32_t*)A.raw((size_t)B * 4);
      p.targets_phys = (int64_t*)A.raw((size_t)Md * 8);
    }
    const long Mmax = stage == STAGE_ENC ? Me : stage == STAGE_DEC ? Md : (Me > Md ? Me : Md);
    p.ga = A.template act<T>(Mmax * d);
    p.gb = A.template act<T>(Mmax * d);
    p.gc = A.template act<T>(Mmax * d);
    p.gln = A.template act<T>(Mmax * d);
    p.gqkv = A.template act<T>(Mmax * 3 * d);
    p.go = A.template act<T>(Mmax * d);
    p.gu = A.template act<T>(enc && M1 * d > Mmax * 4 * d ? M1 * d : Mmax * 4 * d);
    if (dec) {
      p.gxa = A.template act<T>(Me * d);
      p.gkv = A.template act<T>(Me * 2 * d);
      p.gq = A.template act<T>(Md * d);
    }
    if (enc)
      p.gA2 = A.template act<T>(stage == STAGE_ENC && M1 * 256 > Me * 3 * d ? M1 * 256 : Me * 3 * d);
    p.delta = A.f32((long)B * c->H * (stage == STAGE_DEC ? S : c->Te));
    p.cs_scratch = A.f32(stage == STAGE_DEC ? attn_colsum_scratch_floats(B, c->H, S, S > c->Te ? S : c->Te)
                                            : attn_colsum_scratch_floats(B, c->H, c->Te, c->Te));
    if (dec) p.qtile_flags = (int32_t*)A.f32((size_t)B * c->H * ((S + 63) / 64) + 16);
    p.gemm_cs_scratch = A.f32((size_t)2 * cdiv(Mmax, 256) * 4 * d + 64);
    if (enc) {
      p.tmp_w1p = A.f32((long)d * 256);
      p.tmp_w2p = A.f32((long)d * 3 * d);
    }
    if (!c->lora.empty()) {
      p.lora_dw = A.f32(c->lora_dw_floats);
      p.lora_part = A.f32(c->lora_part_floats);
    }
    if (enc)
      for (int i = 0; i < c->L_enc; ++i) p.enc[i].x_in = i ? p.enc[i - 1].x_out : p.x0;
    if (dec)
      for (int i = 0; i < c->L_dec; ++i) p.dec[i].x_in = i ? p.dec[i - 1].x_out : p.dx0;
  }
}

struct Runner {
  const oasr_ctx* c;
  hipStream_t st;
  int B, S;
  const int32_t* text_len;
  bool train = false;
  float* cs_scratch = nullptr;
  const int32_t* dec_rows = nullptr;
  const int32_t* dec_span = nullptr;
  long dec_rows_bwd = 0;
  long dec_rows_fwd = 0;
  const float* mel_clip_max = nullptr;
  float* lora_dw = nullptr;
  float* Gw(int64_t off) const {
    const int j = c->lora_at(off);
    return j >= 0 ? lora_dw + c->lora[j].dw : c->G(off);
  }

  int linear(const T* x, long M, int K, const T* W, int N, const float* bias, int act, const T* resid, T* out,
             T* out_pre) {
    Gemm g = gemm_defaults_t<T>();
    g.A = plain_view(x, K);
    g.B = plain_view(W, K);
    g.M = (int)M;
    g.N = N;
    g.K = K;
    g.bias = bias;
    g.act = act;
    g.resid = resid;
    g.ldr = N;
    g.out = out;
    g.out_pre = out_pre;
    g.ldc = N;
    return launch_gemm(g, st);
  }
  int dgrad(const T* dy, long M, int N, const T* W, int K, const T* dgelu_u, const T* resid, T* dx,
            float* colsum = nullptr, bool u_is_deriv = false) {
    Gemm g = gemm_defaults_t<T>();
    g.A = plain_view(dy, N);
    g.B = plain_view(W, K);
    g.tb = 1;
    g.M = (int)M;
    g.N = K;
    g.K = N;
    g.dgelu_u = dgelu_u;
    g.dgelu_deriv = u_is_deriv ? 1 : 0;
    g.ldu = K;
    g.resid = resid;
    g.ldr = K;
    g.out = dx;
    g.ldc = K;
    g.colsum = colsum;
    g.colsum_scratch = colsum ? cs_scratch : nullptr;
    return launch_gemm(g, st);
  }
  int wgrad(const T* dy, long ldy, long M, int N, const View& x, int K, float* dW, long ldw) {
    Gemm g = gemm_defaults_t<T>();
    g.A = plain_view(dy, ldy);
    g.ta = 1;
    g.B = x;
    g.tb = 1;
    g.M = N;
    g.N = K;
// ... 91 lines not shown
    return OASR_OK;
  }
  int wgrad_side(const T* dy, long ldy, long M, int N, const View& x, int K, float* dW, long ldw) {
    if (!(side_mode & 1)) return wgrad(dy, ldy, M, N, x, K, dW, ldw);
    RC(fork_to(c->side.stream));
    OnStream on(st, c->side.stream);
    side_pending = true;
    return wgrad(dy, ldy, M, N, x, K, dW, ldw);
  }
  int join_side() {
    if (!side_pending) return OASR_OK;
    side_pending = false;
    return join_from(c->side.stream);
  }
  int join_big() {
    if (!big_pending) return OASR_OK;
    big_pending = false;
    return join_from(c->side.big);
  }

  int attn_args(Attn& a, const AttnSave& s, bool cross, long Tq, long Tk, bool causal) {
    const int d = c->d;
    memset(&a, 0, sizeof(a));
    if (!cross) {
      a.q = s.qkv;
      a.k = s.qkv + d;
      a.v = s.qkv + 2 * d;
      a.ldq = a.ldk = a.ldv = 3 * d;
      a.bsq = a.bsk = a.bsv = Tq * 3 * d;
    } else {
      a.q = s.qkv;
      a.ldq = d;
      a.bsq = Tq * d;
      a.k = s.kv;
      a.v = s.kv + d;
      a.ldk = a.ldv = 2 * d;
      a.bsk = a.bsv = Tk * 2 * d;
    }
    a.o = s.o;
    a.ldo = d;
    a.bso = Tq * d;
    a.lse = s.lse;
    a.o_lo = s.o_lo;
    a.kv_len = causal ? text_len : nullptr;
    a.B = B;
    a.H = c->H;
    a.Tq = (int)Tq;
    a.Tk = (int)Tk;
    a.causal = causal ? 1 : 0;
    if (dec_rows && (causal || cross)) {
      a.q_rows = dec_rows;
      a.k_rows = cross ? nullptr : dec_rows;
      if (dec_rows_fwd) a.q_span = dec_span;
    }
    return OASR_OK;
  }

  int kv_proj(const BlockP& bp, BlockSave& s, const T* xa) {
    const int d = c->d;
    return linear(xa, (long)B * c->Te, d, c->template Wt<T>(bp.cattn.kw), 2 * d, c->aux(bp.cattn.fused_bias) + d, 0, nullptr, s.ca.kv, nullptr);
  }
  int block_fwd(const BlockP& bp, BlockSave& s, const T* x_in, long M, long Tq, const T* xa, bool causal, hipEvent_t kv_ready = nullptr) {
    const int d = c->d;
    s.x_in = const_cast<T*>(x_in);
    RC(launch_layernorm_fwd(x_in, c->P(bp.attn_ln_w), c->P(bp.attn_ln_b), s.sa.ln, s.sa.mean, s.sa.rstd, M, d, st));
    RC(linear(s.sa.ln, M, d, c->template Wt<T>(bp.attn.qw), 3 * d, c->aux(bp.attn.fused_bias), 0, nullptr, s.sa.qkv, nullptr));
    Attn a;
    attn_args(a, s.sa, false, Tq, Tq, causal);
    RC(launch_attention_fwd(a, st));
    RC(linear(s.sa.o, M, d, c->template Wt<T>(bp.attn.ow), d, c->P(bp.attn.ob), 0, x_in, s.x_mid, nullptr));
    const T* xm = s.x_mid;
    if (bp.cross) {
      RC(launch_layernorm_fwd(xm, c->P(bp.cln_w), c->P(bp.cln_b), s.ca.ln, s.ca.mean, s.ca.rstd, M, d, st));
      RC(linear(s.ca.ln, M, d, c->template Wt<T>(bp.cattn.qw), d, c->P(bp.cattn.qb), 0, nullptr, s.ca.qkv, nullptr));
      if (kv_ready)
        OASR_CHECK_HIP(hipStreamWaitEvent(st, kv_ready, 0));
      else
        RC(kv_proj(bp, s, xa));
      attn_args(a, s.ca, true, Tq, c->Te, false);
      RC(launch_attention_fwd(a, st));
      RC(linear(s.ca.o, M, d, c->template Wt<T>(bp.cattn.ow), d, c->P(bp.cattn.ob), 0, xm, s.x_mid2, nullptr));
      xm = s.x_mid2;
    }
    RC(launch_layernorm_fwd(xm, c->P(bp.mlp_ln_w), c->P(bp.mlp_ln_b), s.ln2, s.mean2, s.rstd2, M, d, st));
    RC(linear(s.ln2, M, d, c->template Wt<T>(bp.w1), 4 * d, c->P(bp.b1), train ? 2 : 1, nullptr, s.hg, train ? s.u : nullptr));
    RC(linear(s.hg, M, 4 * d, c->template Wt<T>(bp.w2), d, c->P(bp.b2), 0, xm, s.x_out, nullptr));
    return OASR_OK;
  }

  View conv1_view(const T* mel_tm) const {
    const int nm = c->dims.n_mels;
    return View{mel_tm, nm, c->T1, (long)c->T1 * nm, nm, 3 * nm, 2 * nm};
  }
  View conv2_view(const T* h1) const {
    const int d = c->d;
    return View{h1, 2L * d, c->Te, (long)c->T1 * d, d, 3 * d, 3 * d};
  }

  int encoder_fwd(Plan& p, const float* mel) {
    const int d = c->d;
    const long M1 = (long)B * c->T1, Me = (long)B * c->Te;
    RC(launch_mel_to_time_major(mel, p.mel_tm, B, c->dims.n_mels, c->T1, st, mel_clip_max));
    const int nm = c->dims.n_mels;
    OASR_CHECK_HIP(hipMemsetAsync(p.mel_tm - 256, 0, 256 * sizeof(T), st));
    OASR_CHECK_HIP(hipMemsetAsync(p.mel_tm + M1 * nm, 0, 256 * sizeof(T), st));
    OASR_CHECK_HIP(hipMemsetAsync(p.h1 - d, 0, (size_t)d * sizeof(T), st));
// ... 420 lines not shown
```

### olmoasr_amd/csrc/engine_step.hip

```cpp
#include "engine_run.h"

constexpr int SIDE_STREAMS_DEFAULT = 7;

template <typename T>
static size_t plan_bytes(const oasr_ctx* c, int B, int S, bool train, int stage) {
  return Step<T>(c, nullptr, 0, nullptr, B, S, nullptr, train, stage).A.cur;
}
extern "C" size_t oasr_workspace_bytes(const oasr_ctx* c, int B, int S, int mode) {
  if (!c || B <= 0 || S <= 0 || mode < OASR_MODE_INFER || mode > OASR_MODE_TRAIN_DEC) return 0;
  const bool train = mode != OASR_MODE_INFER;
  const int stage = mode == OASR_MODE_TRAIN_ENC ? STAGE_ENC : mode == OASR_MODE_TRAIN_DEC ? STAGE_DEC : STAGE_ALL;
  return OASR_BY_DTYPE(c, plan_bytes, c, B, S, train, stage) + 4096;
}

template <typename T>
static int oasr_forward_impl(oasr_ctx* c, const float* mel, const int64_t* tokens, const int32_t* text_len, int B, int S,
                            float* logits_out, void* xa_out, void* workspace, size_t workspace_bytes, void* stream) {
  RC(check_bound(c, false));
  OASR_REQUIRE(mel && tokens && workspace && B > 0 && S > 0 && S <= c->S_max, "oasr_forward: bad args (B=%d S=%d)", B, S);
  OASR_REQUIRE(workspace_bytes >= oasr_workspace_bytes(c, B, S, OASR_MODE_INFER), "oasr_forward: workspace too small");
  Step<T> s(c, workspace, workspace_bytes, stream, B, S, text_len, false);
  RC(s.r.encoder_fwd(s.p, mel));
  RC(s.r.decoder_fwd(s.p, tokens));
  if (xa_out) RC(copy_xa<T>(c, xa_out, s.p.xa, B, s.r.st));
// ... 45 lines not shown
    return e ? atoi(e) : -1;
  }();
  return env >= 0 ? (env & 15) : SIDE_STREAMS_DEFAULT;
}
extern "C" int oasr_span_side_streams(void) { return span_side_streams(); }
extern "C" int oasr_span_set_side_streams(int mode) {
  OASR_HOOK_GATE("oasr_span_set_side_streams");
  g_side_streams = mode < 0 ? -1 : (mode & 15);
  return OASR_OK;
}

static bool span_chunkable(const oasr_ctx* c, int B) { return (c->S_max % 64) == 0 && c->S_max <= 64 * OASR_ROWTAB && B <= 512; }

static int train_step_check(const oasr_ctx* c, const oasr_train_step_args* a, const void* workspace, size_t workspace_bytes) {
  RC(check_bound(c, true));
  OASR_REQUIRE(a, "oasr_train_step: null args");
  OASR_REQUIRE(!a->mel != !a->xa, "oasr_train_step: exactly one of mel and xa is required (mel: the whole step; xa: the decoder alone on given features)");
  OASR_REQUIRE(a->tokens && a->targets && a->text_len && a->loss_out && workspace,
               "oasr_train_step: bad args (tokens, targets, text_len, loss_out and workspace are required)");
  OASR_REQUIRE(a->B > 0 && a->S > 0 && a->S <= c->S_max, "oasr_train_step: B=%d must be positive and S=%d inside (0, n_text_ctx=%d]", a->B, a->S, c->S_max);
  if (a->span_host) {
    OASR_REQUIRE(a->S == c->S_max, "oasr_train_step: a span step covers the whole context (S = %d, n_text_ctx = %d)", a->S, c->S_max);
    OASR_REQUIRE(a->span_forward == OASR_SPAN_FORWARD_ALL || a->span_forward == OASR_SPAN_FORWARD_ACTIVE, "oasr_train_step: span_forward");
    OASR_REQUIRE(!a->logits_out, "oasr_train_step: logits_out belongs to the plain step (the span step keeps no fp32 logits)");
  } else {
    OASR_REQUIRE(!a->pred_out, "oasr_train_step: pred_out comes with span_host (the predictions cover the span's rows)");
    OASR_REQUIRE(!a->mel_clip_max, "oasr_train_step: mel_clip_max comes with span_host (the un-finalized log-mel is consumed by the span step only)");
  }
  OASR_REQUIRE(!a->xa || (!a->mel_clip_max && !a->logits_out), "oasr_train_step: mel_clip_max / logits_out do not apply to the step from a given xa");
  OASR_REQUIRE(!a->pred_out || span_chunkable(c, a->B),
               "pred_out needs the chunk-row table: n_text_ctx = %d must be a multiple of 64 (<= %d) and B = %d <= 512", c->S_max, 64 * OASR_ROWTAB, a->B);
  OASR_REQUIRE(workspace_bytes >= oasr_workspace_bytes(c, a->B, a->S, a->xa ? OASR_MODE_TRAIN_DEC : OASR_MODE_TRAIN), "oasr_train_step: workspace too small");
  if (a->xa && c->pr.enc_any) {
    oasr_set_error("oasr_train_step: an encoder tensor is trainable -- the step from a given xa has no encoder backward (freeze the "
                   "encoder, or pass mel)");
    return OASR_ESTATE;
  }
  return OASR_OK;
}

template <typename T>
static int train_step_impl(oasr_ctx* c, const oasr_train_step_args& a, bool chunked, void* workspace, size_t workspace_bytes, void* stream) {
  const int B = a.B, S = a.S;
  const long Md = (long)B * S;
  Step<T> s(c, workspace, workspace_bytes, stream, B, S, a.text_len, true, a.xa ? STAGE_DEC : STAGE_ALL);
  auto& p = s.p;
  auto& r = s.r;
  hipStream_t st = r.st;
  r.mel_clip_max = a.mel_clip_max;
  const int64_t* ce_targets = a.targets;
  long ce_rows = Md;
  if (chunked) {
    long R = 0;
    RC(launch_build_span_tables(a.span_host, B, S, a.targets, PAD_ID, p.rows, p.span_dev, p.targets_phys, &R, st));
    OASR_REQUIRE(R > 0, "oasr_train_step: no position of the micro-batch carries gradient (every span is 0)");
    r.dec_rows = p.rows;
    r.dec_span = p.span_dev;
    r.dec_rows_bwd = R;
    r.dec_rows_fwd = a.span_forward == OASR_SPAN_FORWARD_ACTIVE ? R : 0;
    if (const int mode = span_side_streams()) RC(r.side_begin(mode));
    ce_targets = p.targets_phys;
    ce_rows = R;
  }
  if (a.xa) RC(copy_xa<T>(c, p.xa, a.xa, B, st));
  else RC(r.encoder_fwd(p, a.mel));
  RC(r.decoder_fwd(p, a.tokens));
  if (a.logits_out) RC(launch_logits_to_f32(p.logits, c->Vp, Md, c->V, a.logits_out, st));
  if (a.pred_out) RC(launch_argmax_rows(p.logits, c->Vp, c->V, Md, p.rows, p.span_dev, B, S, a.pred_out, st));
  RC(launch_count_valid(a.targets, Md, PAD_ID, c->V, p.n_valid, st));
  RC(launch_cross_entropy(p.logits, c->Vp, c->V, ce_targets, ce_rows, PAD_ID, a.loss_scale * a.inv_accum, p.n_valid, p.row_loss, 1, st));
  RC(launch_loss_reduce(p.row_loss, ce_rows, p.n_valid, a.inv_accum, a.loss_out, a.accumulate_loss, st));
  return train_backward<T>(c, r, p, a.tokens, B, S, a.seg_events);
}
extern "C" size_t oasr_sizeof_train_step_args(void) { return sizeof(oasr_train_step_args); }
extern "C" int oasr_train_step(oasr_ctx* c, const oasr_train_step_args* a, void* workspace, size_t workspace_bytes, void* stream) {
  RC(train_step_check(c, a, workspace, workspace_bytes));
  return OASR_BY_DTYPE(c, train_step_impl, c, *a, a->span_host && span_chunkable(c, a->B), workspace, workspace_bytes, stream);
}

template <typename T>
static int oasr_train_fwd_impl(oasr_ctx* c, const float* mel, const int64_t* tokens, const int32_t* text_len, int B, int S,
                               float* logits_out, void* workspace, size_t workspace_bytes, void* stream) {
  Step<T> s(c, workspace, workspace_bytes, stream, B, S, text_len, true);
  RC(s.r.encoder_fwd(s.p, mel));
  RC(s.r.decoder_fwd(s.p, tokens));
  return launch_logits_to_f32(s.p.logits, c->Vp, (long)B * S, c->V, logits_out, s.r.st);
}
template <typename T>
static int oasr_train_bwd_impl(oasr_ctx* c, const int64_t* tokens, const int32_t* text_len, const float* dlogits, int B, int S, void** ev,
                               void* workspace, size_t workspace_bytes, void* stream) {
  Step<T> s(c, workspace, workspace_bytes, stream, B, S, text_len, true);
  RC(launch_dlogits_from_f32(dlogits, c->V, (long)B * S, c->Vp, s.p.logits, s.r.st));
  return train_backward<T>(c, s.r, s.p, tokens, B, S, ev);
}
extern "C" int oasr_train_fwd(oasr_ctx* c, const float* mel, const int64_t* tokens, const int32_t* text_len, int B, int S, float* logits_out,
                              void* workspace, size_t workspace_bytes, void* stream) {
  RC(check_bound(c, true));
  OASR_REQUIRE(S > 0 && S <= c->S_max, "oasr_train_fwd: S=%d outside (0, n_text_ctx=%d]", S, c->S_max);
  OASR_REQUIRE(mel && tokens && text_len && logits_out && workspace && B > 0, "oasr_train_fwd: bad args");
  OASR_REQUIRE(workspace_bytes >= oasr_workspace_bytes(c, B, S, OASR_MODE_TRAIN), "oasr_train_fwd: workspace too small");
  return OASR_BY_DTYPE(c, oasr_train_fwd_impl, c, mel, tokens, text_len, B, S, logits_out, workspace, workspace_bytes, stream);
}
extern "C" int oasr_train_bwd(oasr_ctx* c, const int64_t* tokens, const int32_t* text_len, const float* dlogits, int B, int S, void** ev,
                              void* workspace, size_t workspace_bytes, void* stream) {
  RC(check_bound(c, true));
  OASR_REQUIRE(S > 0 && S <= c->S_max, "oasr_train_bwd: S=%d outside (0, n_text_ctx=%d]", S, c->S_max);
  OASR_REQUIRE(tokens && text_len && dlogits && workspace && B > 0, "oasr_train_bwd: bad args");
  OASR_REQUIRE(workspace_bytes >= oasr_workspace_bytes(c, B, S, OASR_MODE_TRAIN), "oasr_train_bwd: workspace too small");
  return OASR_BY_DTYPE(c, oasr_train_bwd_impl, c, tokens, text_len, dlogits, B, S, ev, workspace, workspace_bytes, stream);
}
// ... 68 lines not shown
```

### olmoasr_amd/csrc/fp32ref.hip

```cpp
#include <math.h>

#include "kernels.h"

namespace {

inline unsigned grid_for(long work_items, int per_block = 256, int cap = 4096) {
  long b = (work_items + per_block - 1) / per_block;
  if (b < 1) b = 1;
  if (b > cap) b = cap;
  return (unsigned)b;
}

__device__ __forceinline__ float gelu_exact(float x) { return 0.5f * x * (1.0f + erff(x * 0.70710678118654752f)); }
__device__ __forceinline__ float dgelu_exact(float x) {
  const float z = x * 0.70710678118654752f;
  const float cdf = x < 0.f ? 0.5f * erfcf(-z) : 0.5f * (1.0f + erff(z));
  return cdf + x * expf(-0.5f * x * x) * 0.3989422804014327f;
}

__device__ __forceinline__ float view_elem(const OperandViewF& v, long i, long j) {
  if (v.rpb) {
    const long b = i / v.rpb, t = i - b * v.rpb;
    if (j >= v.kvalid || (t == 0 && j < v.lead) || (t == v.rpb - 1 && j >= v.trail_from)) return 0.f;
    return v.ptr[b * v.bstride + t * v.ld - v.lead + j];
// ... 456 lines not shown
  if (rows <= 0) return OASR_OK;
  hipLaunchKernelGGL(ln_fwd_f32_kernel, dim3((unsigned)((rows + 3) / 4)), dim3(256), 0, s, x, gamma, beta, y, mean, rstd, rows, d);
  OASR_LAUNCH_CHECK();
  return OASR_OK;
}
int launch_layernorm_bwd(const float* dy, const float* x, const float* gamma, const float* mean, const float* rstd, const float* dres,
                         float* dx, float* dgamma, float* dbeta, float* dsum, long rows, int d, hipStream_t s) {
  OASR_REQUIRE(dy && x && gamma && mean && rstd && dx && d > 0 && d <= 64 * LN_MAXC, "layernorm_bwd(f32): bad args");
  if (rows <= 0) return OASR_OK;
  long nb = (rows + 3) / 4;
  if (nb > 512) nb = 512;
  const dim3 g((unsigned)nb);
  switch ((dgamma ? 1 : 0) | (dbeta ? 2 : 0)) {
    case 3: hipLaunchKernelGGL(ln_bwd_f32_kernel<3>, g, dim3(256), 0, s, dy, x, gamma, mean, rstd, dres, dx, dgamma, dbeta, dsum, rows, d); break;
    case 2: hipLaunchKernelGGL(ln_bwd_f32_kernel<2>, g, dim3(256), 0, s, dy, x, gamma, mean, rstd, dres, dx, dgamma, dbeta, dsum, rows, d); break;
    case 1: hipLaunchKernelGGL(ln_bwd_f32_kernel<1>, g, dim3(256), 0, s, dy, x, gamma, mean, rstd, dres, dx, dgamma, dbeta, dsum, rows, d); break;
    default: hipLaunchKernelGGL(ln_bwd_f32_kernel<0>, g, dim3(256), 0, s, dy, x, gamma, mean, rstd, dres, dx, dgamma, dbeta, dsum, rows, d); break;
  }
  OASR_LAUNCH_CHECK();
  return OASR_OK;
}

int launch_pack_conv_weight(const float* w, float* dst, int co, int ci, int ldk, hipStream_t s) {
  OASR_REQUIRE(w && dst && ldk >= 3 * ci, "pack_conv_weight(f32): bad args");
  hipLaunchKernelGGL(pack_conv_f32_kernel, dim3(grid_for((long)co * ldk)), dim3(256), 0, s, w, dst, co, ci, ldk);
  OASR_LAUNCH_CHECK();
  return OASR_OK;
}
int launch_mel_to_time_major(const float* mel, float* out, int B, int n_mels, int T, hipStream_t s, const float* clip_max) {
  OASR_REQUIRE(mel && out, "mel_to_time_major(f32): bad args");
  const long total = (long)B * T * n_mels;
  hipLaunchKernelGGL(mel_tm_f32_kernel, dim3(grid_for(total)), dim3(256), 0, s, mel, out, n_mels, T, total, clip_max);
  OASR_LAUNCH_CHECK();
  return OASR_OK;
}
int launch_embedding_fwd(const int64_t* tok, const float* E, const float* pos, float* x, int B, int S, int d, long n_embed, hipStream_t s,
                         const int32_t* rows_tab) {
  OASR_REQUIRE(tok && E && pos && x, "embedding_fwd(f32): bad args");
  const long total = (long)B * S * d;
  hipLaunchKernelGGL(embedding_fwd_f32_kernel, dim3(grid_for(total)), dim3(256), 0, s, tok, E, pos, x, S, d, total, n_embed, rows_tab);
  OASR_LAUNCH_CHECK();
  return OASR_OK;
}
int launch_embedding_bwd(const int64_t* tok, const float* dx, float* dE, float* dpos, int B, int S, int d, long pad_id, long n_embed,
                         hipStream_t s, const int32_t* rows_tab, const int32_t* span) {
  OASR_REQUIRE(tok && dx && (dE || dpos), "embedding_bwd(f32): bad args");
  hipLaunchKernelGGL(embedding_bwd_f32_kernel, dim3(S), dim3(256), 0, s, tok, dx, dE, dpos, B, S, d, pad_id, n_embed, rows_tab, span);
  OASR_LAUNCH_CHECK();
  return OASR_OK;
}
int launch_colsum_accum(const float* x, long ld, long M, int ncols, float* out, hipStream_t s) {
  OASR_REQUIRE(x && out && ncols > 0, "colsum(f32): bad args");
  if (M <= 0) return OASR_OK;
  long gy = M < 256 ? M : 256;
  hipLaunchKernelGGL(colsum_f32_kernel, dim3(cdiv(ncols, 256), (unsigned)gy), dim3(256), 0, s, x, ld, M, ncols, out);
  OASR_LAUNCH_CHECK();
  return OASR_OK;
}
int launch_conv2_col2im_dgelu(const float* dA, const float* u1, float* dpre1, int B, int T1, int d, hipStream_t s) {
  OASR_REQUIRE(dA && u1 && dpre1 && T1 % 2 == 0, "col2im(f32): bad args");
  const long total = (long)B * T1 * d;
  hipLaunchKernelGGL(col2im_dgelu_f32_kernel, dim3(grid_for(total)), dim3(256), 0, s, dA, u1, dpre1, T1, d, total);
  OASR_LAUNCH_CHECK();
  return OASR_OK;
}
int launch_dgelu_mul(const float* dy, const float* u, float* out, long n, hipStream_t s) {
  OASR_REQUIRE(dy && u && out, "dgelu_mul(f32): bad args");
  hipLaunchKernelGGL(dgelu_mul_f32_kernel, dim3(grid_for(n)), dim3(256), 0, s, dy, u, out, n);
  OASR_LAUNCH_CHECK();
  return OASR_OK;
}
int launch_dlogits_from_f32(const float* src, int V, long rows, long ld, float* dst, hipStream_t s) {
  OASR_REQUIRE(src && dst && V <= ld, "dlogits_from_f32(f32): bad args");
  const long total = rows * ld;
  hipLaunchKernelGGL(dlogits_copy_f32_kernel, dim3(grid_for(total)), dim3(256), 0, s, src, V, ld, dst, total);
  OASR_LAUNCH_CHECK();
  return OASR_OK;
}
int launch_logits_to_f32(const float* logits, long ld, long rows, int V, float* out, hipStream_t s) {
  const long total = rows * V;
  hipLaunchKernelGGL(logits_copy_f32_kernel, dim3(grid_for(total)), dim3(256), 0, s, logits, ld, V, out, total);
  OASR_LAUNCH_CHECK();
  return OASR_OK;
}
int launch_cross_entropy(float* logits, long ld, int V, const int64_t* targets, long rows, long ignore, float gscale,
                         const int32_t* n_valid_dev, float* row_loss, int write_grad, hipStream_t s) {
  OASR_REQUIRE(logits && targets && n_valid_dev && row_loss && V <= ld, "cross_entropy(f32): bad args");
  if (rows <= 0) return OASR_OK;
  hipLaunchKernelGGL(ce_f32_kernel, dim3((unsigned)rows), dim3(256), 0, s, logits, ld, V, targets, ignore, gscale, n_valid_dev, row_loss,
                     write_grad);
  OASR_LAUNCH_CHECK();
  return OASR_OK;
}
```

### olmoasr_amd/csrc/kernels.h

```cpp
#pragma once
#include "common.h"

template <typename T>
struct OperandViewT {
  const T* ptr;
  long ld;
  int rpb;
  long bstride;
  int lead;
  int kvalid;
  int trail_from;
};
typedef OperandViewT<bf16_t> OperandView;
typedef OperandViewT<float> OperandViewF;
template <typename T>
static inline OperandViewT<T> plain_view(const T* p, long ld) {
  return OperandViewT<T>{p, ld, 0, 0, 0, 0, 0};
}

template <typename T>
struct GemmArgsT {
  OperandViewT<T> A, B;
  int M, N, K;
  int ta, tb;
// ... 22 lines not shown
  int vgrid;
  int epi_flags;
  float* colsum_scratch;
};
typedef GemmArgsT<bf16_t> GemmArgs;
typedef GemmArgsT<float> GemmArgsF;
int launch_gemm(const GemmArgs& a, hipStream_t stream);
int launch_gemm(const GemmArgsF& a, hipStream_t stream);
void gemm_profile_enable(int on);
int gemm_profile_lane(int lane);
void gemm_force_general(int on);
void gemm_set_variant(int dma_in_mma);
void gemm_set_stagger(int sleeps, int phases);
int gemm_profile_collect(double ms[4], double flops[4], long count[4], char* by_symbol, int cap);
int gemm_profile_records(char* buf, int cap);
template <typename T>
static inline GemmArgsT<T> gemm_defaults_t() {
  GemmArgsT<T> g;
  memset(&g, 0, sizeof(g));
  g.alpha = 1.0f;
  g.split_k = 1;
  return g;
}
static inline GemmArgs gemm_defaults() { return gemm_defaults_t<bf16_t>(); }

int launch_layernorm_fwd(const bf16_t* x, const float* gamma, const float* beta, bf16_t* y, float* mean, float* rstd,
                         long rows, int d, hipStream_t s);
int launch_layernorm_bwd(const bf16_t* dy, const bf16_t* x, const float* gamma, const float* mean, const float* rstd,
                         const bf16_t* dres, bf16_t* dx, float* dgamma, float* dbeta, float* dsum, long rows, int d, hipStream_t s);
int launch_layernorm_fwd(const float* x, const float* gamma, const float* beta, float* y, float* mean, float* rstd, long rows, int d,
                         hipStream_t s);
int launch_layernorm_bwd(const float* dy, const float* x, const float* gamma, const float* mean, const float* rstd, const float* dres,
                         float* dx, float* dgamma, float* dbeta, float* dsum, long rows, int d, hipStream_t s);

template <typename T>
struct AttnArgsT {
  const T *q, *k, *v;
  long ldq, ldk, ldv;
  long bsq, bsk, bsv;
  T* o;
  long ldo, bso;
  float* lse;
  T* o_lo;
  const int32_t* kv_len;
  int B, H, Tq, Tk, causal;
  const T* d_o;
  float* delta;
  T *dq, *dk, *dv;
  float *dq_colsum, *dv_colsum;
  float* colsum_scratch;
  int32_t* qtile_flags;
  const int32_t *q_rows, *k_rows;
  const int32_t* q_span;
};
#ifndef OASR_ROWTAB
#define OASR_ROWTAB 16
#endif
static inline size_t attn_colsum_scratch_floats(int B, int H, int Tq, int Tk) {
  return (size_t)B * ((size_t)(Tq + 127) / 128 + (size_t)(Tk + 127) / 128) * H * 64;
}
typedef AttnArgsT<bf16_t> AttnArgs;
typedef AttnArgsT<float> AttnArgsF;
int launch_attention_fwd(const AttnArgs& a, hipStream_t s);
int launch_attention_bwd(const AttnArgs& a, hipStream_t s);
int launch_attention_scores(const AttnArgs& a, float* out, hipStream_t s);
void attention_set_pingpong(int on);
int launch_attention_fwd(const AttnArgsF& a, hipStream_t s);
int launch_attention_bwd(const AttnArgsF& a, hipStream_t s);
int launch_attention_scores(const AttnArgsF& a, float* out, hipStream_t s);

int launch_decode_proj(const bf16_t* x, int M, int K, const bf16_t* W, int N, const float* ln_g, const float* ln_b, const float* bias,
                       int gelu, const bf16_t* resid, long ldr, bf16_t* out, long ldc, float* out_f32, long ldf, hipStream_t s);

struct DecodeXcdArgs {
  const bf16_t* wflat;
  const float* params;
  const float* aux;
  bf16_t* cache;
  long cache_lstride;
  bf16_t *x, *x2, *x3, *q, *o, *hg;
  float* part;
  unsigned* ctrl;
  int d, H, Te, S_max, L, M, pos;
  int flags;
  void* stamps;
  int team, stride;
  const bf16_t* w_logits = nullptr;
  const float *lnf_g = nullptr, *lnf_b = nullptr;
  float* logits_out = nullptr;
  int V = 0;
  const int64_t* layer_offsets;
  long lstride, astride;
};
int launch_decode_xcd(const DecodeXcdArgs& a, hipStream_t s);
bool decode_xcd_supports(int d, int H, int Te, int S_max, int L, int M);
bool decode_xcd_offsets_ok(const int64_t* layer0, long lstride, long cache_lstride, int d, int Te, int L, int M);
size_t decode_xcd_part_floats(int M, int H, int Te);
int launch_decode_wide(const DecodeXcdArgs& a, hipStream_t s);
bool decode_wide_supports(int d, int H, int Te, int S_max, int L, int M, int nwg);
size_t decode_wide_part_floats(int H);

int launch_cast_f32_bf16(const float* src, bf16_t* dst, long n, hipStream_t s);
int launch_pack_conv_weight(const float* w, bf16_t* dst, int co, int ci, int ldk, hipStream_t s);
int launch_unpack_conv_grad(const float* g, float* dw, int co, int ci, int ldk, hipStream_t s);
int launch_pack_embedding(const float* e, bf16_t* dst, int rows, int rows_pad, int d, hipStream_t s);
int launch_mel_to_time_major(const float* mel, bf16_t* out, int B, int n_mels, int T, hipStream_t s, const float* clip_max = nullptr);
int launch_embedding_fwd(const int64_t* tok, const float* E, const float* pos, bf16_t* x, int B, int S, int d, long n_embed,
                         hipStream_t s, const int32_t* rows = nullptr);
int launch_embedding_bwd(const int64_t* tok, const bf16_t* dx, float* dE, float* dpos, int B, int S, int d, long pad_id, long n_embed,
                         hipStream_t s, const int32_t* rows = nullptr, const int32_t* span = nullptr);
int launch_build_span_tables(const int32_t* span_host, int B, int S, const int64_t* targets, long ignore, int32_t* rows, int32_t* span_dev,
                             int64_t* targets_phys, long* active_rows, hipStream_t s);
int launch_colsum_accum(const bf16_t* x, long ld, long M, int ncols, float* out, hipStream_t s);
int launch_conv2_col2im_dgelu(const bf16_t* dA , const bf16_t* u1 , bf16_t* dpre1, int B, int T1,
                              int d, hipStream_t s);
int launch_conv1_col2im_mel(const bf16_t* dcol, float* dmel, int B, int T1, int n_mels, hipStream_t s);
int launch_conv1_col2im_mel(const float* dcol, float* dmel, int B, int T1, int n_mels, hipStream_t s);
int launch_axpy_f32(const float* src, float* dst, long n, float a, hipStream_t s);
int launch_pack_conv_weight(const float* w, float* dst, int co, int ci, int ldk, hipStream_t s);
int launch_mel_to_time_major(const float* mel, float* out, int B, int n_mels, int T, hipStream_t s, const float* clip_max = nullptr);
int launch_embedding_fwd(const int64_t* tok, const float* E, const float* pos, float* x, int B, int S, int d, long n_embed, hipStream_t s,
                         const int32_t* rows = nullptr);
int launch_embedding_bwd(const int64_t* tok, const float* dx, float* dE, float* dpos, int B, int S, int d, long pad_id, long n_embed,
                         hipStream_t s, const int32_t* rows = nullptr, const int32_t* span = nullptr);
int launch_colsum_accum(const float* x, long ld, long M, int ncols, float* out, hipStream_t s);
int launch_conv2_col2im_dgelu(const float* dA, const float* u1, float* dpre1, int B, int T1, int d, hipStream_t s);
int launch_dgelu_mul(const bf16_t* dy, const bf16_t* u, bf16_t* out, long n, hipStream_t s);
int launch_dgelu_mul(const float* dy, const float* u, float* out, long n, hipStream_t s);
int launch_logits_to_f32(const bf16_t* logits, long ld, long rows, int V, float* out, hipStream_t s);
int launch_logits_to_f32(const float* logits, long ld, long rows, int V, float* out, hipStream_t s);
int launch_dlogits_from_f32(const float* src, int V, long rows, long ld, bf16_t* dst, hipStream_t s);
int launch_dlogits_from_f32(const float* src, int V, long rows, long ld, float* dst, hipStream_t s);

int launch_count_valid(const int64_t* targets, long rows, long ignore, int V, int32_t* n_valid_dev, hipStream_t s);
int launch_cross_entropy(bf16_t* logits, long ld, int V, const int64_t* targets, long rows, long ignore, float gscale,
                         const int32_t* n_valid_dev, float* row_loss, int write_grad, hipStream_t s);
int launch_cross_entropy(float* logits, long ld, int V, const int64_t* targets, long rows, long ignore, float gscale,
                         const int32_t* n_valid_dev, float* row_loss, int write_grad, hipStream_t s);
int launch_loss_reduce(const float* row_loss, long rows, const int32_t* n_valid_dev, float mul, float* loss_out, int accumulate,
                       hipStream_t s);

int launch_pick_tokens(const float* logits, long ld, int V, long rows, const float* mask, const float* mask2, int64_t* tok, float* logprob,
                       hipStream_t s);
int launch_pick_tokens_ts(const float* logits, long ld, int V, long rows, const float* mask, const float* mask2, const int64_t* hist,
                          long hist_ld, int n_hist, int ts_begin, int eot, int no_ts, int max_initial_index, int64_t* tok, float* logprob,
                          hipStream_t s);

int launch_topk_tokens_ts(const float* logits, long ld, int V, long rows, const float* mask, const float* mask2, const int64_t* hist,
                          long hist_ld, int n_hist, int ts_begin, int eot, int no_ts, int max_initial_index, int K, int64_t* tok,
                          float* logprob, hipStream_t s);
int launch_sample_tokens_ts(const float* logits, long ld, int V, long rows, const float* mask, const float* mask2, const int64_t* hist,
                            long hist_ld, int n_hist, int ts_begin, int eot, int no_ts, int max_initial_index, float temperature,
                            const float* u, int64_t* tok, float* logprob, hipStream_t s);

struct oasr_align_args;
int launch_alignment_matrix(const oasr_align_args* a, void* workspace, size_t workspace_bytes, hipStream_t s);
int launch_dtw(const float* cost, long ld, int N, int M, int negate, int32_t* text_indices, int32_t* time_indices, int32_t* path_len,
               void* workspace, size_t workspace_bytes, hipStream_t s);

struct oasr_edit_args;
int launch_edit_counts(const oasr_edit_args* a, hipStream_t s);

int launch_argmax_rows(const bf16_t* logits, long ld, int V, long n_rows, const int32_t* rows, const int32_t* span, int B, int S, int32_t* pred,
                       hipStream_t s);
int launch_argmax_rows(const float* logits, long ld, int V, long n_rows, const int32_t* rows, const int32_t* span, int B, int S, int32_t* pred,
// ... 18 lines not shown
```

### olmoasr_amd/ops.py

```python
import ctypes as C

import torch

from . import _native as N

BF = torch.bfloat16


def _op(t, ld=None, rpb=0, bstride=0, lead=0, kvalid=0, trail_from=0):
    return N.Operand(t.data_ptr(), ld if ld is not None else t.stride(0), rpb, bstride, lead, kvalid, trail_from)


def gemm(A, B, M, N_, K, *, ta=False, tb=False, a_view=None, b_view=None, bias=None, act=0, pos=None, pos_period=0,
         dgelu_u=None, resid=None, out=None, out_pre=None, ldc=None, out_f32=None, beta=0.0, atomic=False, split_k=1,
         alpha=1.0, colsum=None, dgelu_deriv=False, ldc32=None, colsum_scratch=None, atomic_on_pp=None, raster_gm=None, stagger=None,
         stagger_phases=None):
    g = N.GemmArgs()
    g.A = a_view if a_view is not None else _op(A)
    g.B = b_view if b_view is not None else _op(B)
    g.M, g.N, g.K, g.ta, g.tb, g.alpha = M, N_, K, int(ta), int(tb), alpha
    g.bias = bias.data_ptr() if bias is not None else None
    g.act = act
    g.pos = pos.data_ptr() if pos is not None else None
    g.pos_period = pos_period
# ... 88 lines not shown
    a.kv_len = kv_len.data_ptr() if kv_len is not None else None
    a.B, a.H, a.Tq, a.Tk, a.causal = B, H, Tq, Tk, int(causal)
    N.check(N.lib().oasr_attention_scores(C.byref(a), 0 if q.dtype == BF else 1, N.ptr(out), N.stream_ptr()), "attention_scores")
    return out


def attention_bwd(q, k, v, o, lse, d_o, kv_len=None, causal=False, o_lo=None, dq_colsum=None, dv_colsum=None, qtile_flags=None):
    B, Tq, H, _ = q.shape
    dq, dk, dv = (torch.empty_strided(t.shape, t.stride(), device=t.device, dtype=t.dtype) for t in (q, k, v))
    delta = torch.empty(B, H, Tq, device=q.device, dtype=torch.float32)
    a = _attn_args(q, k, v, o.view(B, Tq, H, 64), lse, kv_len, causal)
    a.d_o, a.delta = d_o.data_ptr(), delta.data_ptr()
    a.o_lo = o_lo.data_ptr() if o_lo is not None else None
    a.dq, a.dk, a.dv = dq.data_ptr(), dk.data_ptr(), dv.data_ptr()
    a.dq_colsum = dq_colsum.data_ptr() if dq_colsum is not None else None
    a.dv_colsum = dv_colsum.data_ptr() if dv_colsum is not None else None
    a.qtile_flags = qtile_flags.data_ptr() if qtile_flags is not None else None
    scratch = None
    if dq_colsum is not None or dv_colsum is not None:
        Tk = k.shape[1]
        scratch = torch.empty(B * ((Tq + 127) // 128 + (Tk + 127) // 128) * H * 64, device=q.device, dtype=torch.float32)
        a.colsum_scratch = scratch.data_ptr()
    N.check(N.lib().oasr_attention_bwd(C.byref(a), N.stream_ptr()), "attention_bwd")
    return dq, dk, dv


def chunk_rows_table(order, B, n_chunks):
    tab = torch.full((B, N.ROWTAB), 0x3FFFFFFF, dtype=torch.int32)
    for i, (b, c) in enumerate(order):
        tab[b, c] = 64 * i
    assert int((tab[:, :n_chunks] == 0x3FFFFFFF).sum()) == 0, "every (b, chunk) needs a place"
    return tab


def to_chunked(x, tab):
    B, T = x.shape[:2]
    out = torch.empty((B * T,) + tuple(x.shape[2:]), device=x.device, dtype=x.dtype)
    for b in range(B):
        for c in range(T // 64):
            r = int(tab[b, c])
            out[r:r + 64] = x[b, 64 * c:64 * c + 64]
    return out


def from_chunked(xc, tab, B, T):
    out = torch.empty((B, T) + tuple(xc.shape[1:]), device=xc.device, dtype=xc.dtype)
    for b in range(B):
        for c in range(T // 64):
            r = int(tab[b, c])
            out[b, 64 * c:64 * c + 64] = xc[r:r + 64]
    return out


def _attn_args_rows(qc, kc, vc, oc, lse, B, H, Tq, Tk, q_rows, k_rows, kv_len, causal):
    a = N.AttnArgs()
    a.q, a.k, a.v, a.o = qc.data_ptr(), kc.data_ptr(), vc.data_ptr(), oc.data_ptr()
    a.ldq, a.ldo = qc.stride(0), oc.stride(0)
    if k_rows is not None:
        a.ldk, a.ldv = kc.stride(0), vc.stride(0)
        a.k_rows = k_rows.data_ptr()
    else:
        a.ldk, a.ldv, a.bsk, a.bsv = kc.stride(1), vc.stride(1), kc.stride(0), vc.stride(0)
    a.lse = lse.data_ptr()
    a.kv_len = kv_len.data_ptr() if kv_len is not None else None
    a.B, a.H, a.Tq, a.Tk, a.causal = B, H, Tq, Tk, int(causal)
    a.q_rows = q_rows.data_ptr()
    return a


def attention_fwd_rows(qc, kc, vc, B, H, Tq, Tk, q_rows, k_rows=None, kv_len=None, causal=False, want_o_lo=False):
    oc = torch.empty(B * Tq, H * 64, device=qc.device, dtype=BF)
    lse = torch.empty(B, H, Tq, device=qc.device, dtype=torch.float32)
    a = _attn_args_rows(qc, kc, vc, oc.view(B * Tq, H, 64), lse, B, H, Tq, Tk, q_rows, k_rows, kv_len, causal)
    o_lo = torch.empty_like(oc) if want_o_lo else None
    a.o_lo = o_lo.data_ptr() if want_o_lo else None
    N.check(N.lib().oasr_attention_fwd(C.byref(a), N.stream_ptr()), "attention_fwd(rows)")
    return (oc, lse, o_lo) if want_o_lo else (oc, lse)


def attention_bwd_rows(qc, kc, vc, oc, lse, doc, B, H, Tq, Tk, q_rows, k_rows=None, q_span=None, kv_len=None, causal=False, o_lo=None,
                       dq_colsum=None, dv_colsum=None, fill=None):
    def like(t):
        g = torch.empty_strided(t.shape, t.stride(), device=t.device, dtype=t.dtype)
        if fill is not None:
            g.fill_(fill)
        return g
    dq, dk, dv = like(qc), like(kc), like(vc)
    delta = torch.zeros(B, H, Tq, device=qc.device, dtype=torch.float32)
    a = _attn_args_rows(qc, kc, vc, oc.view(B * Tq, H, 64), lse, B, H, Tq, Tk, q_rows, k_rows, kv_len, causal)
    a.d_o, a.delta = doc.data_ptr(), delta.data_ptr()
    a.o_lo = o_lo.data_ptr() if o_lo is not None else None
    a.dq, a.dk, a.dv = dq.data_ptr(), dk.data_ptr(), dv.data_ptr()
    a.q_span = q_span.data_ptr() if q_span is not None else None
    a.dq_colsum = dq_colsum.data_ptr() if dq_colsum is not None else None
    a.dv_colsum = dv_colsum.data_ptr() if dv_colsum is not None else None
    scratch = None
    if dq_colsum is not None or dv_colsum is not None:
        scratch = torch.empty(B * ((Tq + 127) // 128 + (Tk + 127) // 128) * H * 64, device=qc.device, dtype=torch.float32)
        a.colsum_scratch = scratch.data_ptr()
    N.check(N.lib().oasr_attention_bwd(C.byref(a), N.stream_ptr()), "attention_bwd(rows)")
    return dq, dk, dv


_ws_cache = {}


def _workspace(kind, device, need):
    key = (kind, torch.device(device).index if torch.device(device).index is not None else torch.cuda.current_device())
    ws = _ws_cache.get(key)
    if ws is None or ws.numel() < need:
        _ws_cache[key] = None
        ws = _ws_cache[key] = torch.empty(max(int(need), 16), dtype=torch.uint8, device=device)
    return ws


MEDFILT_WIDTHS = (1, 3, 5, 7, 9, 11, 13, 15)


def alignment_matrix(qk_layers, heads_per_layer, n_frames, medfilt_width=7, qk_scale=1.0, out=None):
    qk_layers, heads_per_layer = list(qk_layers), [[int(h) for h in hs] for hs in heads_per_layer]
    if any(len(set(hs)) != len(hs) for hs in heads_per_layer):
        raise ValueError("alignment_matrix: a head index is repeated within a layer")
    if not qk_layers or len(qk_layers) != len(heads_per_layer) or len(qk_layers) > N.AlignArgs.MAX_LAYERS:
        raise ValueError(f"alignment_matrix: {len(qk_layers)} score tensors for {len(heads_per_layer)} head lists (1 .. {N.AlignArgs.MAX_LAYERS}, one list each)")
    shape = tuple(qk_layers[0].shape)
    for t in qk_layers:
        if not (isinstance(t, torch.Tensor) and t.dim() == 3 and tuple(t.shape) == shape and t.dtype == torch.float32 and t.is_contiguous()):
            raise ValueError("alignment_matrix: every score tensor is a contiguous fp32 [H, n_tok, Tk] of the same shape")
    H, n_tok, Tk = shape
    if not (1 <= H <= 32 and 1 <= n_tok <= 65535 and Tk >= 1):
        raise ValueError(f"alignment_matrix: H = {H} (1 .. 32), n_tok = {n_tok} (1 .. 65535), Tk = {Tk}")
    if any(h < 0 or h >= H for hs in heads_per_layer for h in hs) or not any(heads_per_layer):
        raise ValueError(f"alignment_matrix: head indices must lie in [0, {H}) and at least one head must be selected")
    n_frames, medfilt_width = int(n_frames), int(medfilt_width)
    if not 1 <= n_frames <= Tk:
        raise ValueError(f"alignment_matrix: n_frames = {n_frames} outside [1, Tk = {Tk}]")
    if medfilt_width not in MEDFILT_WIDTHS:
        raise ValueError(f"alignment_matrix: medfilt_width = {medfilt_width}: an odd width from 1 to 15")
    dev = qk_layers[0].device
    for t in qk_layers:
        N.require_gpu(t, "alignment_matrix: score tensor")
        if t.device != dev:
            raise ValueError("alignment_matrix: score tensors on different devices")
    if out is None:
        out = torch.empty(n_tok, n_frames, device=dev, dtype=torch.float32)
    elif not (out.dtype == torch.float32 and tuple(out.shape) == (n_tok, n_frames) and out.device == dev and (out.stride(1) == 1 or n_frames == 1)
              and out.stride(0) >= n_frames):
        raise ValueError("alignment_matrix: out must be fp32 [n_tok, n_frames] on the scores' device with unit column stride")
    a = N.AlignArgs()
    for l, (t, hs) in enumerate(zip(qk_layers, heads_per_layer)):
        a.qk[l] = t.data_ptr()
        a.head_mask[l] = sum(1 << h for h in hs)
# ... 335 lines not shown
```

Measured before the change: 5976.

## Launch decoder attention only over active span blocks via compact block tables

Builds compact (b, h, block) tables of the 128- and 256-query blocks that fall inside each sample's active span while the span tables are built. The decoder attention forward and backward kernels then launch grids sized to those active blocks instead of the full B*H*Tq grid. Inactive blocks used to launch and exit early. The colsum scratch is now zeroed with a memset so the skipped blocks leave no stale partial sums. Small colsum reductions also use a single row of workgroups. The cost is an extra memset and table build per step, plus added bookkeeping that reuses the qtile_flags buffer to hold the tables.

```diff
diff --git a/include/oasr.h b/include/oasr.h
--- a/include/oasr.h
+++ b/include/oasr.h
@@ -140,6 +140,8 @@
   float* colsum_scratch;
   int32_t* qtile_flags;
   const int32_t *q_rows, *k_rows, *q_span;
+  const int32_t *qblk128, *qblk256;
+  int n128, n256;
 } oasr_attn_args;
 #define OASR_ROWTAB 16
 size_t oasr_sizeof_attn_args(void);
diff --git a/include/oasr_testing.h b/include/oasr_testing.h
--- a/include/oasr_testing.h
+++ b/include/oasr_testing.h
@@ -15,6 +15,7 @@
 int oasr_wide_plan_debug(int d, int nwg, int N, int K, int wg, int wave, int* out, int max_units);
 int oasr_xcd_offsets_ok_debug(const int64_t* layer0, long long lstride, long long cache_lstride, int d, int Te, int L, int M);
 int oasr_attention_set_pingpong(int on);
+int oasr_attention_set_span_grid(int on);
 int oasr_gemm_set_stagger(int sleeps, int phases);
 int oasr_gemm_force_general(int on);
 int oasr_test_gemm(const oasr_gemm_args* a, float* colsum_scratch, int atomic_on_pp, int raster_gm, int stagger, int stagger_phases, void* stream);
@@ -24,6 +25,8 @@
 int oasr_probe_tr16(const void* src_bf16 , void* dst_bf16 , void* stream);
 int oasr_test_span_tables(const int32_t* span_host, int B, int S, const int64_t* targets, int32_t* rows_out, int32_t* span_out,
                           int64_t* targets_rows_out, int64_t* active_rows_out, void* stream);
+int oasr_test_span_block_tables(const int32_t* span_host, int B, int S, int H, const int64_t* targets, int32_t* rows_out, int32_t* span_out,
+                                int64_t* targets_rows_out, int32_t* blk128_out, int32_t* blk256_out, int32_t* counts_out, void* stream);
 
 int oasr_test_embedding_fwd(const int64_t* tok, const float* E, const float* pos, void* x, int dtype, int B, int S, int d, int64_t n_embed,
                             const int32_t* rows, void* stream);
diff --git a/olmoasr_amd/_native.py b/olmoasr_amd/_native.py
--- a/olmoasr_amd/_native.py
+++ b/olmoasr_amd/_native.py
@@ -38,7 +38,8 @@
                 ("H", C.c_int), ("Tq", C.c_int), ("Tk", C.c_int), ("causal", C.c_int), ("d_o", C.c_void_p),
                 ("delta", C.c_void_p), ("dq", C.c_void_p), ("dk", C.c_void_p), ("dv", C.c_void_p), ("dq_colsum", C.c_void_p),
                 ("dv_colsum", C.c_void_p), ("colsum_scratch", C.c_void_p), ("qtile_flags", C.c_void_p),
-                ("q_rows", C.c_void_p), ("k_rows", C.c_void_p), ("q_span", C.c_void_p)]
+                ("q_rows", C.c_void_p), ("k_rows", C.c_void_p), ("q_span", C.c_void_p),
+                ("qblk128", C.c_void_p), ("qblk256", C.c_void_p), ("n128", C.c_int), ("n256", C.c_int)]
 
 
 class AlignArgs(C.Structure):
@@ -115,6 +116,7 @@
         "oasr_log_mel_raw": (i32, [vp, i32, i32, i32, vp, vp, vp, vp]),
         "oasr_sizeof_attn_args": (sz, []),
         "oasr_test_span_tables": (i32, [vp, i32, i32, vp, vp, vp, vp, vp, vp]),
+        "oasr_test_span_block_tables": (i32, [vp, i32, i32, i32, vp, vp, vp, vp, vp, vp, vp, vp]),
         "oasr_test_embedding_fwd": (i32, [vp, vp, vp, vp, i32, i32, i32, i32, i64, vp, vp]),
         "oasr_test_embedding_bwd": (i32, [vp, vp, i32, vp, vp, i32, i32, i32, i64, i64, vp, vp, vp]),
         "oasr_test_colsum": (i32, [vp, i32, i64, i64, i32, vp, vp]),
@@ -180,6 +182,7 @@
         "oasr_wide_supports_debug": (i32, [i32, i32, i32, i32, i32, i32, i32]),
         "oasr_wide_plan_debug": (i32, [i32, i32, i32, i32, i32, i32, vp, i32]),
         "oasr_attention_set_pingpong": (i32, [i32]),
+        "oasr_attention_set_span_grid": (i32, [i32]),
         "oasr_profile_gemm_collect": (i32, [vp, vp, vp, C.c_char_p, i32]),
     }
     for name, (res, args) in sig.items():
diff --git a/olmoasr_amd/csrc/api.hip b/olmoasr_amd/csrc/api.hip
--- a/olmoasr_amd/csrc/api.hip
+++ b/olmoasr_amd/csrc/api.hip
@@ -89,6 +89,11 @@
 extern "C" int oasr_attention_set_pingpong(int on) {
   OASR_HOOK_GATE("oasr_attention_set_pingpong");
   attention_set_pingpong(on);
+  return OASR_OK;
+}
+extern "C" int oasr_attention_set_span_grid(int on) {
+  OASR_HOOK_GATE("oasr_attention_set_span_grid");
+  attention_set_span_grid(on);
   return OASR_OK;
 }
 extern "C" int oasr_gemm_force_general(int on) {
@@ -154,6 +159,10 @@
   r.q_rows = a->q_rows;
   r.k_rows = a->k_rows;
   r.q_span = a->q_span;
+  r.qblk128 = a->qblk128;
+  r.qblk256 = a->qblk256;
+  r.n128 = a->n128;
+  r.n256 = a->n256;
   return r;
 }
 extern "C" int oasr_attention_fwd(const oasr_attn_args* a, void* stream) {
@@ -204,6 +213,18 @@
   return rc;
 }
 
+extern "C" int oasr_test_span_block_tables(const int32_t* span_host, int B, int S, int H, const int64_t* targets, int32_t* rows_out,
+                                           int32_t* span_out, int64_t* targets_rows_out, int32_t* blk128_out, int32_t* blk256_out,
+                                           int32_t* counts_out, void* stream) {
+  OASR_REQUIRE(counts_out, "oasr_test_span_block_tables: null");
+  long act = 0;
+  SpanBlockTables blk{H, blk128_out, blk256_out, 0, 0};
+  const int rc = launch_build_span_tables(span_host, B, S, targets, 51864, rows_out, span_out, targets_rows_out, &act, (hipStream_t)stream, &blk);
+  counts_out[0] = blk.n128;
+  counts_out[1] = blk.n256;
+  return rc;
+}
+
 #define OASR_TEST_DTYPE(name) \
   OASR_REQUIRE(dtype == OASR_DTYPE_BF16 || dtype == OASR_DTYPE_F32, name ": dtype %d (0 = bf16, 1 = fp32 activations)", dtype)
 
diff --git a/olmoasr_amd/csrc/attention.hip b/olmoasr_amd/csrc/attention.hip
--- a/olmoasr_amd/csrc/attention.hip
+++ b/olmoasr_amd/csrc/attention.hip
@@ -123,6 +123,26 @@
 #define MFMA(a, b, c) __builtin_amdgcn_mfma_f32_32x32x16_bf16((a), (b), (c), 0, 0, 0)
 
 __device__ __forceinline__ int chunk_row(const int32_t* rows, int b, int t) { return rows[b * OASR_ROWTAB + (t >> 6)] + (t & 63); }
+
+struct BlockId {
+  int b, h, blk;
+};
+template <bool ROWS>
+__device__ __forceinline__ BlockId block_id(const int32_t* tab, int bid, int nblk, int H) {
+  BlockId r;
+  if (ROWS && tab) {
+    const int e = tab[bid];
+    r.b = e >> 16;
+    r.h = (e >> 4) & 0xfff;
+    r.blk = e & 15;
+  } else {
+    const int bh = bid / nblk;
+    r.b = bh / H;
+    r.h = bh - r.b * H;
+    r.blk = bid - bh * nblk;
+  }
+  return r;
+}
 
 typedef float f32x2_t __attribute__((ext_vector_type(2)));
 __device__ __forceinline__ f32x2_t pk_fma(f32x2_t a, f32x2_t b, f32x2_t c) { return __builtin_elementwise_fma(a, b, c); }
@@ -174,9 +194,9 @@
   const int tid = threadIdx.x, lane = tid & 63, wave = tid >> 6, hh = lane >> 5;
   const int nqb = (a.Tq + 127) >> 7;
   const int bid = xcd_remap(blockIdx.x, gridDim.x);
-  const int bh = bid / nqb;
-  const int b = bh / a.H, h = bh - b * a.H;
-  const int q0 = (bid - bh * nqb) * 128;
+  const BlockId id = block_id<ROWS>(a.qblk128, bid, nqb, a.H);
+  const int b = id.b, h = id.h, qblk = id.blk;
+  const int q0 = qblk * 128;
   const int myq = q0 + wave * 32 + (lane & 31);
   const int myq_c = myq < a.Tq ? myq : a.Tq - 1;
   const bool krows = ROWS && a.k_rows != nullptr;
@@ -348,14 +368,14 @@
   const int tid = threadIdx.x, lane = tid & 63, wave = tid >> 6, hh = lane >> 5;
   const int nqb = (a.Tq + 127) >> 7;
   const int bid = xcd_remap(blockIdx.x, gridDim.x);
-  const int bh = bid / nqb;
-  const int b = bh / a.H, h = bh - b * a.H;
-  const int q0 = (bid - bh * nqb) * 128;
+  const BlockId id = block_id<ROWS>(a.qblk128, bid, nqb, a.H);
+  const int b = id.b, h = id.h, qblk = id.blk;
+  const int q0 = qblk * 128;
   const int myq = q0 + wave * 32 + (lane & 31);
   const bool krows = ROWS && a.k_rows != nullptr;
   const int q_lim = (ROWS && a.q_span) ? min(a.q_span[b], a.Tq) : a.Tq;
   if (ROWS && q0 >= q_lim) {
-    if (a.dq_colsum && tid < 64) a.colsum_scratch[((long)(b * nqb + (bid - bh * nqb)) * a.H + h) * 64 + tid] = 0.f;
+    if (a.dq_colsum && tid < 64) a.colsum_scratch[((long)(b * nqb + qblk) * a.H + h) * 64 + tid] = 0.f;
     return;
   }
   const bool w_act = !ROWS || q0 + wave * 32 < q_lim;
@@ -496,7 +516,7 @@
   if (a.dq_colsum) {
     __syncthreads();
     if (tid < 64)
-      a.colsum_scratch[((long)(b * nqb + (bid - bh * nqb)) * a.H + h) * 64 + tid] =
+      a.colsum_scratch[((long)(b * nqb + qblk) * a.H + h) * 64 + tid] =
           (wsum[tid] + wsum[64 + tid]) + (wsum[128 + tid] + wsum[192 + tid]);
   }
 }
@@ -509,14 +529,14 @@
   const unsigned smem_a = (unsigned)(size_t)smem;
   const int nqb = (a.Tq + 255) >> 8;
   const int bid = xcd_remap(blockIdx.x, gridDim.x);
-  const int bh = bid / nqb;
-  const int b = bh / a.H, h = bh - b * a.H;
-  const int q0 = (bid - bh * nqb) * 256;
+  const BlockId id = block_id<ROWS>(a.qblk256, bid, nqb, a.H);
+  const int b = id.b, h = id.h, qblk = id.blk;
+  const int q0 = qblk * 256;
   const int myq = q0 + wave * 32 + (lane & 31);
   const int q_lim = (ROWS && a.q_span) ? min(a.q_span[b], a.Tq) : a.Tq;
   if (ROWS && q0 >= q_lim) {
     if (a.dq_colsum && tid < 128) {
-      const int nqb128 = (a.Tq + 127) >> 7, blk128 = (bid - bh * nqb) * 2 + (tid >> 6);
+      const int nqb128 = (a.Tq + 127) >> 7, blk128 = qblk * 2 + (tid >> 6);
       if (blk128 < nqb128) a.colsum_scratch[((long)(b * nqb128 + blk128) * a.H + h) * 64 + (tid & 63)] = 0.f;
     }
     return;
@@ -751,7 +771,7 @@
     if (tid < 128) {
       const int half = tid >> 6, c = tid & 63;
       const int nqb128 = (a.Tq + 127) >> 7;
-      const int blk128 = (bid - bh * nqb) * 2 + half;
+      const int blk128 = qblk * 2 + half;
       if (blk128 < nqb128)
         a.colsum_scratch[((long)(b * nqb128 + blk128) * a.H + h) * 64 + c] =
             (wsum[half * 256 + c] + wsum[half * 256 + 64 + c]) + (wsum[half * 256 + 128 + c] + wsum[half * 256 + 192 + c]);
@@ -773,15 +793,15 @@
   const int tid = threadIdx.x, lane = tid & 63, wave = tid >> 6, hh = lane >> 5;
   const int nkb = (a.Tk + 127) >> 7;
   const int bid = xcd_remap(blockIdx.x, gridDim.x);
-  const int bh = bid / nkb;
-  const int b = bh / a.H, h = bh - b * a.H;
-  const int k0 = (bid - bh * nkb) * 128;
+  const BlockId id = block_id<ROWS>(a.qblk128, bid, nkb, a.H);
+  const int b = id.b, h = id.h, kblk = id.blk;
+  const int k0 = kblk * 128;
   const int mykey = k0 + wave * 32 + (lane & 31);
   const bool krows = ROWS && a.k_rows != nullptr;
   const int q_lim = (ROWS && a.q_span) ? min(a.q_span[b], a.Tq) : a.Tq;
   const long dv_scratch_off0 = (long)a.B * ((a.Tq + 127) >> 7) * a.H * 64;
   if (krows && a.q_span && k0 >= q_lim) {
-    if (a.dv_colsum && tid < 64) a.colsum_scratch[dv_scratch_off0 + ((long)(b * nkb + (bid - bh * nkb)) * a.H + h) * 64 + tid] = 0.f;
+    if (a.dv_colsum && tid < 64) a.colsum_scratch[dv_scratch_off0 + ((long)(b * nkb + kblk) * a.H + h) * 64 + tid] = 0.f;
     return;
   }
   const bool w_store = !(krows && a.q_span) || k0 + wave * 32 < q_lim;
@@ -837,7 +857,7 @@
   };
   const long dv_scratch_off = dv_scratch_off0;
   if (!any) {
-    if (a.dv_colsum && tid < 64) a.colsum_scratch[dv_scratch_off + ((long)(b * nkb + (bid - bh * nkb)) * a.H + h) * 64 + tid] = 0.f;
+    if (a.dv_colsum && tid < 64) a.colsum_scratch[dv_scratch_off + ((long)(b * nkb + kblk) * a.H + h) * 64 + tid] = 0.f;
     if (mykey < a.Tk && w_store) {
       bf16_t* dkp0 = krows ? a.dk + (long)chunk_row(a.k_rows, b, mykey) * a.ldk + h * 64 : a.dk + (long)b * a.bsk + (long)mykey * a.ldk + h * 64;
       bf16_t* dvp0 = krows ? a.dv + (long)chunk_row(a.k_rows, b, mykey) * a.ldv + h * 64 : a.dv + (long)b * a.bsv + (long)mykey * a.ldv + h * 64;
@@ -938,7 +958,7 @@
     if (a.dv_colsum) {
       __syncthreads();
       if (tid < 64)
-        a.colsum_scratch[dv_scratch_off + ((long)(b * nkb + (bid - bh * nkb)) * a.H + h) * 64 + tid] =
+        a.colsum_scratch[dv_scratch_off + ((long)(b * nkb + kblk) * a.H + h) * 64 + tid] =
             (wsum[tid] + wsum[64 + tid]) + (wsum[128 + tid] + wsum[192 + tid]);
     }
   }
@@ -1277,6 +1297,9 @@
 }
 
 int g_attn_pingpong = 1;
+int g_attn_span_grid = 1;
+
+bool span_grid(const AttnArgs& a) { return g_attn_span_grid && a.q_rows && a.q_span && a.qblk128 && a.qblk256; }
 
 int check_args(const AttnArgs& a, bool bwd) {
   OASR_REQUIRE(a.q && a.k && a.v && a.o, "attention: null pointer");
@@ -1289,12 +1312,17 @@
   OASR_REQUIRE(!a.q_span || a.q_rows, "attention: q_span needs q_rows");
   OASR_REQUIRE(!a.q_rows || ((a.Tq % 64) == 0 && a.Tq <= 64 * OASR_ROWTAB), "attention: chunked query rows need Tq %% 64 == 0 and Tq <= %d", 64 * OASR_ROWTAB);
   OASR_REQUIRE(!a.k_rows || ((a.Tk % 64) == 0 && a.Tk <= 64 * OASR_ROWTAB), "attention: chunked key rows need Tk %% 64 == 0 and Tk <= %d", 64 * OASR_ROWTAB);
+  OASR_REQUIRE(!a.qblk128 == !a.qblk256, "attention: the 128- and the 256-query block tables come together");
+  OASR_REQUIRE(!a.qblk128 || (a.n128 >= 0 && a.n128 <= a.B * cdiv(a.Tq, 128) && a.n256 >= 0 && a.n256 <= a.B * cdiv(a.Tq, 256) && a.n256 <= a.n128 &&
+                              a.n128 <= 2 * a.n256),
+               "attention: block counts n128 = %d, n256 = %d do not fit B = %d, Tq = %d", a.n128, a.n256, a.B, a.Tq);
   return OASR_OK;
 }
 
 }
 
 void attention_set_pingpong(int on) { g_attn_pingpong = on; }
+void attention_set_span_grid(int on) { g_attn_span_grid = on; }
 
 int launch_attention_fwd(const AttnArgs& a, hipStream_t s) {
   int rc = check_args(a, false);
@@ -1306,10 +1334,17 @@
   }
   dim3 grid(cdiv(a.Tq, 128) * a.B * a.H);
   if (a.q_rows) {
+    AttnArgs r = a;
+    if (span_grid(a)) {
+      if (a.n128 == 0) return OASR_OK;
+      grid = dim3(a.n128 * a.H);
+    } else {
+      r.qblk128 = r.qblk256 = nullptr;
+    }
     if (a.causal)
-      hipLaunchKernelGGL((attn_fwd_kernel<true, true>), grid, dim3(256), 0, s, a);
+      hipLaunchKernelGGL((attn_fwd_kernel<true, true>), grid, dim3(256), 0, s, r);
     else
-      hipLaunchKernelGGL((attn_fwd_kernel<false, true>), grid, dim3(256), 0, s, a);
+      hipLaunchKernelGGL((attn_fwd_kernel<false, true>), grid, dim3(256), 0, s, r);
   } else if (a.causal) {
     hipLaunchKernelGGL((attn_fwd_kernel<true, false>), grid, dim3(256), 0, s, a);
   } else {
@@ -1322,12 +1357,27 @@
 int launch_attention_bwd(const AttnArgs& a, hipStream_t s) {
   int rc = check_args(a, true);
   if (rc) return rc;
-  dim3 gq(cdiv(a.Tq, 128) * a.B * a.H), gk(cdiv(a.Tk, 128) * a.B * a.H);
+  dim3 gq(cdiv(a.Tq, 128) * a.B * a.H), gk(cdiv(a.Tk, 128) * a.B * a.H), gq256(cdiv(a.Tq, 256) * a.B * a.H);
   const bool rows = a.q_rows != nullptr;
+  const int d = a.H * 64;
+  const long rq = (long)a.B * cdiv(a.Tq, 128), rk = (long)a.B * cdiv(a.Tk, 128);
+  AttnArgs aq = a, ak = a;
+  const bool cq = rows && span_grid(a), ck = cq && a.k_rows != nullptr && a.Tk == a.Tq;
+  if (!cq) aq.qblk128 = aq.qblk256 = nullptr;
+  if (!ck) ak.qblk128 = ak.qblk256 = nullptr;
+  if (cq) {
+    if (a.n128 == 0) return OASR_OK;
+    gq = dim3(a.n128 * a.H);
+    gq256 = dim3(a.n256 * a.H);
+    if (ck) gk = gq;
+    const long zrows = (a.dq_colsum ? rq : 0) + (ck && a.dv_colsum ? rk : 0);
+    float* z0 = a.dq_colsum ? a.colsum_scratch : a.colsum_scratch + rq * d;
+    if (zrows) OASR_CHECK_HIP(hipMemsetAsync(z0, 0, (size_t)zrows * d * sizeof(float), s));
+  }
   if (a.causal) {
     if (rows) {
-      hipLaunchKernelGGL((attn_bwd_dq_kernel<true, true>), gq, dim3(256), 0, s, a);
-      hipLaunchKernelGGL((attn_bwd_dkdv_kernel<true, true>), gk, dim3(256), 0, s, a);
+      hipLaunchKernelGGL((attn_bwd_dq_kernel<true, true>), gq, dim3(256), 0, s, aq);
+      hipLaunchKernelGGL((attn_bwd_dkdv_kernel<true, true>), gk, dim3(256), 0, s, ak);
     } else {
       hipLaunchKernelGGL((attn_bwd_dq_kernel<true, false>), gq, dim3(256), 0, s, a);
       hipLaunchKernelGGL((attn_bwd_dkdv_kernel<true, false>), gk, dim3(256), 0, s, a);
@@ -1335,7 +1385,7 @@
   } else {
     const bool pp = !a.kv_len && g_attn_pingpong && (!rows || (!a.k_rows && a.Tq <= 512));
     if (pp) {
-      if (rows) hipLaunchKernelGGL(attn_bwd_dq_pp_kernel<true>, dim3(cdiv(a.Tq, 256) * a.B * a.H), dim3(512), 0, s, a);
+      if (rows) hipLaunchKernelGGL(attn_bwd_dq_pp_kernel<true>, gq256, dim3(512), 0, s, aq);
       else hipLaunchKernelGGL(attn_bwd_dq_pp_kernel<false>, dim3(cdiv(a.Tq, 256) * a.B * a.H), dim3(512), 0, s, a);
       static LdsAttrOnce attr_rows, attr_plain;
       rc = rows ? ensure_dynamic_lds(attr_rows, (const void*)attn_bwd_dkdv_pp_kernel<true>, KLDS)
@@ -1344,16 +1394,14 @@
       if (rows) hipLaunchKernelGGL(attn_bwd_dkdv_pp_kernel<true>, dim3(cdiv(a.Tk, 256) * a.B * a.H), dim3(512), KLDS, s, a);
       else hipLaunchKernelGGL(attn_bwd_dkdv_pp_kernel<false>, dim3(cdiv(a.Tk, 256) * a.B * a.H), dim3(512), KLDS, s, a);
     } else if (rows) {
-      hipLaunchKernelGGL((attn_bwd_dq_kernel<false, true>), gq, dim3(256), 0, s, a);
-      hipLaunchKernelGGL((attn_bwd_dkdv_kernel<false, true>), gk, dim3(256), 0, s, a);
+      hipLaunchKernelGGL((attn_bwd_dq_kernel<false, true>), gq, dim3(256), 0, s, aq);
+      hipLaunchKernelGGL((attn_bwd_dkdv_kernel<false, true>), gk, dim3(256), 0, s, ak);
     } else {
       hipLaunchKernelGGL((attn_bwd_dq_kernel<false, false>), gq, dim3(256), 0, s, a);
       hipLaunchKernelGGL((attn_bwd_dkdv_kernel<false, false>), gk, dim3(256), 0, s, a);
     }
   }
   OASR_LAUNCH_CHECK();
-  const int d = a.H * 64;
-  const long rq = (long)a.B * cdiv(a.Tq, 128), rk = (long)a.B * cdiv(a.Tk, 128);
   if (a.dq_colsum) {
     int rc2 = launch_colsum_accum(a.colsum_scratch, d, rq, d, a.dq_colsum, s);
     if (rc2) return rc2;
diff --git a/olmoasr_amd/csrc/elementwise.hip b/olmoasr_amd/csrc/elementwise.hip
--- a/olmoasr_amd/csrc/elementwise.hip
+++ b/olmoasr_amd/csrc/elementwise.hip
@@ -290,11 +290,27 @@
 };
 __global__ __launch_bounds__(1024) void build_span_tables_kernel(SpanArg sp, int B, int S, const int64_t* __restrict__ targets, long ignore,
                                                                  int32_t* __restrict__ rows, int32_t* __restrict__ span_dev,
-                                                                 int64_t* __restrict__ targets_phys) {
+                                                                 int64_t* __restrict__ targets_phys, int H, int32_t* __restrict__ blk128,
+                                                                 int32_t* __restrict__ blk256) {
   __shared__ int cnt_act[OASR_ROWTAB + 1];
   __shared__ int rows_s[512 * OASR_ROWTAB];
   const int nch = S >> 6, tid = threadIdx.x;
   if (tid <= OASR_ROWTAB) cnt_act[tid] = 0;
+  if (blk128) {
+    for (int i = tid; i < B * H; i += 1024) {
+      const int b = i / H, h = i - b * H;
+      int pre128 = 0, pre256 = 0;
+      for (int bb = 0; bb < b; ++bb) {
+        const int s64 = ((int)sp.span[bb] + 63) & ~63;
+        pre128 += (s64 + 127) >> 7;
+        pre256 += (s64 + 255) >> 8;
+      }
+      const int s64 = ((int)sp.span[b] + 63) & ~63;
+      const int n1 = (s64 + 127) >> 7, n2 = (s64 + 255) >> 8;
+      for (int j = 0; j < n1; ++j) blk128[(pre128 * H + h * n1) + j] = attn_qblk_pack(b, h, j);
+      for (int j = 0; j < n2; ++j) blk256[(pre256 * H + h * n2) + j] = attn_qblk_pack(b, h, j);
+    }
+  }
   __syncthreads();
   if (tid < nch) {
     int n = 0;
@@ -326,20 +342,27 @@
 }
 }
 int launch_build_span_tables(const int32_t* span_host, int B, int S, const int64_t* targets, long ignore, int32_t* rows, int32_t* span_dev,
-                             int64_t* targets_phys, long* active_rows, hipStream_t s) {
+                             int64_t* targets_phys, long* active_rows, hipStream_t s, SpanBlockTables* blocks) {
   OASR_REQUIRE(span_host && targets && rows && span_dev && targets_phys && active_rows, "build_span_tables: null pointer");
+  OASR_REQUIRE(!blocks || (blocks->H > 0 && blocks->H < 4096 && blocks->blk128 && blocks->blk256), "build_span_tables: bad block tables");
   OASR_REQUIRE(B > 0 && B <= 512 && S > 0 && S % 64 == 0 && S <= 64 * OASR_ROWTAB, "build_span_tables: need B <= 512, S %% 64 == 0, S <= %d (B=%d S=%d)",
                64 * OASR_ROWTAB, B, S);
   SpanArg sp;
   long act = 0;
+  int n128 = 0, n256 = 0;
   for (int b = 0; b < B; ++b) {
     OASR_REQUIRE(span_host[b] >= 0 && span_host[b] <= S, "build_span_tables: span[%d] = %d outside [0, %d]", b, span_host[b], S);
     sp.span[b] = (uint16_t)span_host[b];
-    act += (span_host[b] + 63) / 64 * 64;
+    const int s64 = (span_host[b] + 63) / 64 * 64;
+    act += s64;
+    n128 += (s64 + 127) / 128;
+    n256 += (s64 + 255) / 256;
   }
   for (int b = B; b < 512; ++b) sp.span[b] = 0;
   *active_rows = act;
-  hipLaunchKernelGGL(build_span_tables_kernel, dim3(1), dim3(1024), 0, s, sp, B, S, targets, ignore, rows, span_dev, targets_phys);
+  if (blocks) blocks->n128 = n128, blocks->n256 = n256;
+  hipLaunchKernelGGL(build_span_tables_kernel, dim3(1), dim3(1024), 0, s, sp, B, S, targets, ignore, rows, span_dev, targets_phys,
+                     blocks ? blocks->H : 0, blocks ? blocks->blk128 : nullptr, blocks ? blocks->blk256 : nullptr);
   OASR_LAUNCH_CHECK();
   return OASR_OK;
 }
diff --git a/olmoasr_amd/csrc/engine_run.h b/olmoasr_amd/csrc/engine_run.h
--- a/olmoasr_amd/csrc/engine_run.h
+++ b/olmoasr_amd/csrc/engine_run.h
@@ -38,6 +38,7 @@
   float *delta, *tmp_w1p, *tmp_w2p, *cs_scratch, *gemm_cs_scratch;
   int32_t* qtile_flags;
   int32_t *rows, *span_dev;
+  int32_t *blk128, *blk256;
   int64_t* targets_phys;
   float *lora_dw, *lora_part;
 };
@@ -140,7 +141,14 @@
     p.delta = A.f32((long)B * c->H * (stage == STAGE_DEC ? S : c->Te));
     p.cs_scratch = A.f32(stage == STAGE_DEC ? attn_colsum_scratch_floats(B, c->H, S, S > c->Te ? S : c->Te)
                                             : attn_colsum_scratch_floats(B, c->H, c->Te, c->Te));
-    if (dec) p.qtile_flags = (int32_t*)A.f32((size_t)B * c->H * ((S + 63) / 64) + 16);
+    if (dec) {
+      const size_t n_flags = (size_t)B * c->H * ((S + 63) / 64) + 16, n128 = span_block_entries(B, S, c->H, 128);
+      p.qtile_flags = (int32_t*)A.f32(n_flags);
+      if (n128 + span_block_entries(B, S, c->H, 256) <= n_flags) {
+        p.blk128 = p.qtile_flags;
+        p.blk256 = p.qtile_flags + n128;
+      }
+    }
     p.gemm_cs_scratch = A.f32((size_t)2 * cdiv(Mmax, 256) * 4 * d + 64);
     if (enc) {
       p.tmp_w1p = A.f32((long)d * 256);
@@ -167,6 +175,8 @@
   const int32_t* dec_rows = nullptr;
   const int32_t* dec_span = nullptr;
   long dec_rows_bwd = 0;
+  const int32_t *dec_blk128 = nullptr, *dec_blk256 = nullptr;
+  int dec_n128 = 0, dec_n256 = 0;
   long dec_rows_fwd = 0;
   const float* mel_clip_max = nullptr;
   float* lora_dw = nullptr;
@@ -364,6 +374,10 @@
       a.q_rows = dec_rows;
       a.k_rows = cross ? nullptr : dec_rows;
       if (dec_rows_fwd) a.q_span = dec_span;
+      a.qblk128 = dec_blk128;
+      a.qblk256 = dec_blk256;
+      a.n128 = dec_n128;
+      a.n256 = dec_n256;
     }
     return OASR_OK;
   }
diff --git a/olmoasr_amd/csrc/engine_step.hip b/olmoasr_amd/csrc/engine_step.hip
--- a/olmoasr_amd/csrc/engine_step.hip
+++ b/olmoasr_amd/csrc/engine_step.hip
@@ -121,10 +121,15 @@
   long ce_rows = Md;
   if (chunked) {
     long R = 0;
-    RC(launch_build_span_tables(a.span_host, B, S, a.targets, PAD_ID, p.rows, p.span_dev, p.targets_phys, &R, st));
+    SpanBlockTables blk{c->H, p.blk128, p.blk256, 0, 0};
+    RC(launch_build_span_tables(a.span_host, B, S, a.targets, PAD_ID, p.rows, p.span_dev, p.targets_phys, &R, st, p.blk128 ? &blk : nullptr));
     OASR_REQUIRE(R > 0, "oasr_train_step: no position of the micro-batch carries gradient (every span is 0)");
     r.dec_rows = p.rows;
     r.dec_span = p.span_dev;
+    r.dec_blk128 = p.blk128;
+    r.dec_blk256 = p.blk256;
+    r.dec_n128 = blk.n128;
+    r.dec_n256 = blk.n256;
     r.dec_rows_bwd = R;
     r.dec_rows_fwd = a.span_forward == OASR_SPAN_FORWARD_ACTIVE ? R : 0;
     if (const int mode = span_side_streams()) RC(r.side_begin(mode));
diff --git a/olmoasr_amd/csrc/fp32ref.hip b/olmoasr_amd/csrc/fp32ref.hip
--- a/olmoasr_amd/csrc/fp32ref.hip
+++ b/olmoasr_amd/csrc/fp32ref.hip
@@ -532,7 +532,7 @@
 int launch_colsum_accum(const float* x, long ld, long M, int ncols, float* out, hipStream_t s) {
   OASR_REQUIRE(x && out && ncols > 0, "colsum(f32): bad args");
   if (M <= 0) return OASR_OK;
-  long gy = M < 256 ? M : 256;
+  long gy = M <= 64 ? 1 : (M < 256 ? M : 256);
   hipLaunchKernelGGL(colsum_f32_kernel, dim3(cdiv(ncols, 256), (unsigned)gy), dim3(256), 0, s, x, ld, M, ncols, out);
   OASR_LAUNCH_CHECK();
   return OASR_OK;
diff --git a/olmoasr_amd/csrc/kernels.h b/olmoasr_amd/csrc/kernels.h
--- a/olmoasr_amd/csrc/kernels.h
+++ b/olmoasr_amd/csrc/kernels.h
@@ -98,7 +98,10 @@
   int32_t* qtile_flags;
   const int32_t *q_rows, *k_rows;
   const int32_t* q_span;
-};
+  const int32_t *qblk128, *qblk256;
+  int n128, n256;
+};
+__host__ __device__ static inline int32_t attn_qblk_pack(int b, int h, int blk) { return (int32_t)((b << 16) | (h << 4) | blk); }
 #ifndef OASR_ROWTAB
 #define OASR_ROWTAB 16
 #endif
@@ -111,6 +114,7 @@
 int launch_attention_bwd(const AttnArgs& a, hipStream_t s);
 int launch_attention_scores(const AttnArgs& a, float* out, hipStream_t s);
 void attention_set_pingpong(int on);
+void attention_set_span_grid(int on);
 int launch_attention_fwd(const AttnArgsF& a, hipStream_t s);
 int launch_attention_bwd(const AttnArgsF& a, hipStream_t s);
 int launch_attention_scores(const AttnArgsF& a, float* out, hipStream_t s);
@@ -155,8 +159,14 @@
                          hipStream_t s, const int32_t* rows = nullptr);
 int launch_embedding_bwd(const int64_t* tok, const bf16_t* dx, float* dE, float* dpos, int B, int S, int d, long pad_id, long n_embed,
                          hipStream_t s, const int32_t* rows = nullptr, const int32_t* span = nullptr);
+struct SpanBlockTables {
+  int H;
+  int32_t *blk128, *blk256;
+  int n128, n256;
+};
+static inline size_t span_block_entries(int B, int S, int H, int gran) { return (size_t)B * ((S + gran - 1) / gran) * H; }
 int launch_build_span_tables(const int32_t* span_host, int B, int S, const int64_t* targets, long ignore, int32_t* rows, int32_t* span_dev,
-                             int64_t* targets_phys, long* active_rows, hipStream_t s);
+                             int64_t* targets_phys, long* active_rows, hipStream_t s, SpanBlockTables* blocks = nullptr);
 int launch_colsum_accum(const bf16_t* x, long ld, long M, int ncols, float* out, hipStream_t s);
 int launch_conv2_col2im_dgelu(const bf16_t* dA , const bf16_t* u1 , bf16_t* dpre1, int B, int T1,
                               int d, hipStream_t s);
diff --git a/olmoasr_amd/ops.py b/olmoasr_amd/ops.py
--- a/olmoasr_amd/ops.py
+++ b/olmoasr_amd/ops.py
@@ -164,6 +164,28 @@
     return out
 
 
+def span_block_tables(span, B, S, H, device="cuda", with_rows=False):
+    span = torch.as_tensor(span, dtype=torch.int32).cpu().contiguous()
+    assert span.numel() == B
+    blk128 = torch.full((B * ((S + 127) // 128) * H,), -1, dtype=torch.int32, device=device)
+    blk256 = torch.full((B * ((S + 255) // 256) * H,), -1, dtype=torch.int32, device=device)
+    targets = torch.full((B, S), 51864, dtype=torch.int64, device=device)
+    rows = torch.empty(B, N.ROWTAB, dtype=torch.int32, device=device)
+    span_d = torch.empty(B, dtype=torch.int32, device=device)
+    tphys = torch.empty(B * S, dtype=torch.int64, device=device)
+    counts = (C.c_int32 * 2)()
+    N.check(N.lib().oasr_test_span_block_tables(C.c_void_p(span.data_ptr()), B, S, H, N.ptr(targets), N.ptr(rows), N.ptr(span_d), N.ptr(tphys),
+                                                N.ptr(blk128), N.ptr(blk256), counts, N.stream_ptr(device)), "span_block_tables")
+    blocks = (blk128, blk256, int(counts[0]), int(counts[1]))
+    return (blocks, rows, span_d) if with_rows else blocks
+
+
+def _set_blocks(a, q_blocks):
+    if q_blocks is not None:
+        blk128, blk256, n128, n256 = q_blocks
+        a.qblk128, a.qblk256, a.n128, a.n256 = blk128.data_ptr(), blk256.data_ptr(), n128, n256
+
+
 def _attn_args_rows(qc, kc, vc, oc, lse, B, H, Tq, Tk, q_rows, k_rows, kv_len, causal):
     a = N.AttnArgs()
     a.q, a.k, a.v, a.o = qc.data_ptr(), kc.data_ptr(), vc.data_ptr(), oc.data_ptr()
@@ -180,18 +202,25 @@
     return a
 
 
-def attention_fwd_rows(qc, kc, vc, B, H, Tq, Tk, q_rows, k_rows=None, kv_len=None, causal=False, want_o_lo=False):
+def attention_fwd_rows(qc, kc, vc, B, H, Tq, Tk, q_rows, k_rows=None, kv_len=None, causal=False, want_o_lo=False, q_span=None, q_blocks=None,
+                       fill=None):
     oc = torch.empty(B * Tq, H * 64, device=qc.device, dtype=BF)
     lse = torch.empty(B, H, Tq, device=qc.device, dtype=torch.float32)
+    o_lo = torch.empty_like(oc) if want_o_lo else None
+    if fill is not None:
+        for t in (oc, lse, o_lo):
+            if t is not None:
+                t.fill_(fill)
     a = _attn_args_rows(qc, kc, vc, oc.view(B * Tq, H, 64), lse, B, H, Tq, Tk, q_rows, k_rows, kv_len, causal)
-    o_lo = torch.empty_like(oc) if want_o_lo else None
     a.o_lo = o_lo.data_ptr() if want_o_lo else None
+    a.q_span = q_span.data_ptr() if q_span is not None else None
+    _set_blocks(a, q_blocks)
     N.check(N.lib().oasr_attention_fwd(C.byref(a), N.stream_ptr()), "attention_fwd(rows)")
     return (oc, lse, o_lo) if want_o_lo else (oc, lse)
 
 
 def attention_bwd_rows(qc, kc, vc, oc, lse, doc, B, H, Tq, Tk, q_rows, k_rows=None, q_span=None, kv_len=None, causal=False, o_lo=None,
-                       dq_colsum=None, dv_colsum=None, fill=None):
+                       dq_colsum=None, dv_colsum=None, fill=None, q_blocks=None, scratch_fill=None):
     def like(t):
         g = torch.empty_strided(t.shape, t.stride(), device=t.device, dtype=t.dtype)
         if fill is not None:
@@ -209,7 +238,10 @@
     scratch = None
     if dq_colsum is not None or dv_colsum is not None:
         scratch = torch.empty(B * ((Tq + 127) // 128 + (Tk + 127) // 128) * H * 64, device=qc.device, dtype=torch.float32)
+        if scratch_fill is not None:
+            scratch.fill_(scratch_fill)
         a.colsum_scratch = scratch.data_ptr()
+    _set_blocks(a, q_blocks)
     N.check(N.lib().oasr_attention_bwd(C.byref(a), N.stream_ptr()), "attention_bwd(rows)")
     return dq, dk, dv
 
```

After: 6115, median of 6. 2.3% higher.
